# hong-chen/er3t

Measured on AMD Instinct MI355X. Metric: photons/sec, higher is better.
Workload: dtype f32; 1 GPU; les480: 480x480x100-voxel LES cloud domain (Atm_nz=116), nadir radiance, HG g=0.85 + Rayleigh, Lambert 0.03; views=1, target=radiance, local_estimate=column-table (exact for nadir), parallelism=single GPU

## Files before the change

### er3t_amd/csrc/mi3d_api.hip

```cpp
#include <hip/hip_runtime.h>

#include <cmath>
#include <cstdarg>
#include <cstdio>
#include <cstdlib>
#include <cstring>
#include <string>
#include <utility>
#include <vector>

#include "mi3d_kernels.hip"
#include "mi3d_kernel_lean.hip"
#include "mi3d_kernel_rays.hip"
#include "mi3d_kernel_flux.hip"

using namespace mi3d;

#include <algorithm>

static constexpr size_t kTabLdsBudget = 24 * 1024;
constexpr int kEvSlots = 4;

namespace {

// ... 46 lines not shown

}

struct mi3d_solver {
    int device = 0;
    int num_cu = 256;
    hipStream_t stream = nullptr;
    hipStream_t own_stream = nullptr;
    bool use_own_stream = false;

    int nz = 0, np1d = 0;
    std::vector<double> zgrd;
    std::vector<float> ext1d, omg1d, apf1d, abs1d;
    int nx = 1, ny = 1, nz3 = 0, iz3l = 1, np3d = 0;
    double dx = 1.0e4, dy = 1.0e4;
    bool has_abst = false;
    int nang = 0, npf = 0;
    std::vector<float> ang, pha;
    int sfc_mtype = MI3D_SFC_LAMBERT, nxb = 0, nyb = 0;
    bool sfc_lambert_only = true;
    float sfc_param[5] = {0, 0, 0, 0, 0};
    std::vector<float> sfc2d_host;
    double src_flx = 1.0, src_qmax = 0.0, src_the = 180.0, src_phi = 0.0;
    int src_mtype = 1;
    double th_wlen = 0.0, th_ptot = 0.0, th_ms = 0.0;
    double src_fsol = -1.0, th_psol = 0.0;
    bool thermal() const { return src_mtype == 3 || src_mtype == 2; }
    std::vector<float> th_tlev;
    size_t th_ntmpa = 0, th_ntmps = 0;
    size_t th_ncell = 0;
    DevBuf<float> d_th_tlev, d_th_tmpa, d_th_tmps;
    DevBuf<double> d_th_cdf, d_th_bsum;
    DevBuf<DevThermal> d_th;
    bool dirty_thermal = false;
    int nview = 0, nxr = 1, nyr = 1;
    double view_the[MI3D_MAX_VIEW], view_phi[MI3D_MAX_VIEW], view_zloc[MI3D_MAX_VIEW], zref = 0.0;
    int rad_kind = 2;
    double cam_psi[MI3D_MAX_VIEW], cam_xpos[MI3D_MAX_VIEW], cam_ypos[MI3D_MAX_VIEW], cam_qmax[MI3D_MAX_VIEW], cam_umax[MI3D_MAX_VIEW],
           cam_vmax[MI3D_MAX_VIEW], cam_apsize[MI3D_MAX_VIEW];
    DevBuf<CamRec> d_cams;
    int cam_mpmap = 1, cam_mrproj = 0;
    DevBuf<double> d_camdir, d_zgrd;
    bool dirty_camdir = true;
    bool camdir_ok = false;
    int target = MI3D_TARGET_FLUX, solver = MI3D_SOLVER_3D, column_le = 1, counting = 0;
    double wmin = 0.2, wfac = 1.0, le_tau1 = 0.0, le_cmin = 0.0;
    std::vector<LayerRec> lay_host;
    std::vector<double> dir_level;
    int kdir = 0;
    DevBuf<double> d_dir_level;

    DevBuf<float> d_abst, d_extp, d_omgp, d_apfp;
    DevBuf<LayerRec> d_lay;
    DevBuf<ViewRec> d_views;
    DevBuf<DevCold> d_cold;
    DevBuf<float> d_bt1d, d_dz, d_bmin, d_bmax;
    DevBuf<float4> d_vrec;
    DevBuf<float> d_bext3;
    double z_cloud = -1.0;
    int tally_window = 1;
    unsigned vcol_f4 = 0, vrow_f4 = 0;
    int vpad_col = 0, vpad_row = 0;
    DevBuf<float> d_tcol0, d_tmu, d_tp, d_tcdf, d_sfc2d;
    DevBuf<uint16_t> d_tmuidx, d_tcdfidx;
    int nmarch = 0, n_step3d = 0, col0 = 0;
    int tab3d_lo = 1 << 30, tab3d_hi = -1;
    bool hg3d = true;
    int tab_lo = 0, tab_n = 0;
    DevBuf<int> d_tabrange;
    DevBuf<float2> d_csca;
    DevBuf<tally_t> d_rad_own, d_flux_own;
    DevBuf<tally_t> d_rad_acc;
    int rad_row_pad = -1;
    int rad_spread = -1;
    tally_t *rad_ext = nullptr, *flux_ext = nullptr;
    DevBuf<double> d_heat_own;
    double *heat_ext = nullptr;
    int heat_estimator = 0;
    size_t heat_elems() const { return (size_t)nz * nx * ny; }
    double *heat_ptr() { return heat_ext ? heat_ext : d_heat_own.p; }
    DevBuf<unsigned long long> d_counters, d_next;
    DevBuf<uint32_t> d_hist;
    DevBuf<uint16_t> d_tile;
    struct PreSet {
        DevBuf<uint32_t> order, cursor;
        DevBuf<float4> entry;
        hipEvent_t done = nullptr, loop = nullptr; bool used = false;
        void release() { order.release(); entry.release(); }
    };
    PreSet pre[2];
    hipStream_t pre_stream = nullptr;
    hipEvent_t pre_main = nullptr;
    bool pre_main_used = false;
    uint64_t pre_no = 0;
    int pre_last = 0;
    int overlap_pre = 1;
    int cam_images = -1;
    bool cam_warned = false;
    bool general_warned = false;
    int entry_records = 1;
    struct EvSet {
        DevBuf<float4> events;
        DevBuf<unsigned long long> evctr, hvlist;
        hipEvent_t emit = nullptr, rays = nullptr; bool used = false;
        void release() { events.release(); hvlist.release(); }
    };
    EvSet ev[2];
    DevCold cold_host2;
    hipStream_t rays_stream = nullptr;
    int overlap_rays = 0;
    int rays_wg = 0, emit_wg = 0;
    double ev_per_photon = 0.0;
    int n_xcd = 8;
    unsigned long long *h_evctr = nullptr;
    struct EvSlot { hipEvent_t done = nullptr; uint64_t nb = 0, cap = 0; unsigned epoch = 0; bool busy = false, cleared = false; };
    EvSlot ev_slot[kEvSlots];
    unsigned ev_epoch = 0;
    int ev_cap_log2 = 28;
    struct PendingSum { bool on = false; TallyList TL; double *flux = nullptr; unsigned nflux = 0; double *heat = nullptr; unsigned nheat = 0; int split = 1; };
    struct TlSet {
        DevBuf<uint2> rec, binned;
        DevBuf<uint32_t> words;
        DevBuf<unsigned long long> cursor;
        DevBuf<float4> runs;
        hipEvent_t filled = nullptr, sorted = nullptr, scattered = nullptr; bool used = false;
        PendingSum pend;
        void release() { rec.release(); binned.release(); words.release(); runs.release(); }
    };
    TlSet tl[2];
    DevBuf<unsigned long long> d_tl_stats;
    hipStream_t tl_stream = nullptr;
    unsigned runs_unread = 0;
    bool tl_unjoined = false;
    uint64_t tl_launch_no = 0;
    int overlap_sort = 1;
    int tl_split = 4;
    double tl_per_photon = 0.0;
    double tl_total_pp = 0.0, tl_runs_pp = 0.0;
    int tally_runs = 1;
    int tl_cap_log2 = 31;
    int tally_lists = 1;
    int lds_max = 65536;
    unsigned long long *h_tlctr = nullptr;
    DevBuf<char> d_tldesc;
    char *h_tldesc = nullptr;
    hipEvent_t tldesc_ev[64] = {};
    bool tldesc_used[64] = {};
    struct TlSlot { hipEvent_t done = nullptr; uint64_t nb = 0, cap = 0, bcap = 0, rcap = 0; bool busy = false; };
    TlSlot tl_slot[kEvSlots];
    int kernel_choice = 0;
    int tile_cols = -1;
    uint64_t batch = (uint64_t)1 << 30;
    DevCold cold_host;

    bool dirty_grid = true, dirty_phase = true, dirty_sfc = true, dirty_tally = true, dirty_views = true;
    bool have_1d = false;

    DevBuf<float> d_run_own[2], d_stat_out;
    DevBuf<float> d_get_out;
    DevBuf<double> d_get_add;
    float *run_ext[2] = {nullptr, nullptr};
    DevBuf<double> d_sum[2], d_sumsq[2];
    DevBuf<float> d_factor[2];
    bool stats_on = false, stats_joined = false;
    hipEvent_t stats_ev = nullptr;
    int stats_nrun = 0;
    double analytic_share = 1.0;
    float *run_ptr(int w) { return run_ext[w] ? run_ext[w] : d_run_own[w].p; }
    size_t stat_elems(int w) const { return w == 0 ? (size_t)nview * nxr * nyr : flux_elems(); }

    std::vector<std::pair<hipEvent_t, hipEvent_t>> pending;
    double kernel_ms = 0.0;
    uint64_t launches = 0;
    std::string last_kernel;

    size_t rad_elems() const { return (size_t)(nview > 0 ? nview : 1) * nxr * nyr; }
    size_t flux_elems() const { return (size_t)3 * (nz + 1) * nx * ny; }
    tally_t *rad_ptr() { return rad_ext ? rad_ext : d_rad_own.p; }
    tally_t *flux_ptr() { return flux_ext ? flux_ext : d_flux_own.p; }
};

namespace {

// ... 382 lines not shown
    hipLaunchKernelGGL(k_scan_top, dim3(1), dim3(1024), 0, h->stream, h->d_th_bsum.p, (unsigned long)nblk);
    HIPCHK(hipGetLastError());
    hipLaunchKernelGGL(k_scan_add, dim3((unsigned)nblk), dim3(256), 0, h->stream, h->d_th_cdf.p, (unsigned long)ncell, (const double *)h->d_th_bsum.p);
    HIPCHK(hipGetLastError());
    HIPCHK(hipEventRecord(e1, h->stream));
    double ptot = 0.0;
    HIPCHK(hipMemcpyAsync(&ptot, h->d_th_cdf.p + (ncell - 1), sizeof(double), hipMemcpyDeviceToHost, h->stream));
    HIPCHK(hipStreamSynchronize(h->stream));
    float ms = 0.0f;
    HIPCHK(hipEventElapsedTime(&ms, e0, e1));
    (void)hipEventDestroy(e0); (void)hipEventDestroy(e1);
    h->th_ms = ms;
    if (!(ptot >= 0.0) || !std::isfinite(ptot)) return fail(MI3D_EINVAL, "thermal source: total emitted power %g", ptot);
    h->th_ptot = ptot;
    h->th_ncell = ncell;
    h->th_psol = 0.0;
    if (h->src_mtype == 2)
        h->th_psol = h->src_fsol * std::fabs(std::cos(h->src_the * 3.14159265358979323846 / 180.0)) * (h->dx * h->nx) * (h->dy * h->ny);
    DevThermal T;
    T.cdf = h->d_th_cdf.p; T.ptot = ptot; T.psol = h->th_psol; T.ncell = (unsigned)ncell; T.nvox = (unsigned)nvox;
    T.nxb = sfc2d ? h->nxb : 1; T.nyb = sfc2d ? h->nyb : 1;
    if ((rc = h->d_th.upload(&T, 1))) return rc;
    return MI3D_OK;
}

constexpr double kCamDirMaxCells = 1048576.0;
int build_camdir(mi3d_solver *h) {
    const size_t n = (size_t)h->nview * h->nxr * h->nyr;
    HIPCHK(sync_streams(h));
    int rc;
    if ((rc = h->d_camdir.alloc(n)) || (rc = h->d_zgrd.upload(h->zgrd.data(), h->zgrd.size()))) return rc;
    HIPCHK(hipMemsetAsync(h->d_camdir.p, 0, n * sizeof(double), h->stream));
    h->camdir_ok = true;
    if (h->src_mtype == 1) {
        const double pi = 3.14159265358979323846;
        const double th = h->src_the * pi / 180.0, ph = h->src_phi * pi / 180.0;
        const int k3lo = h->nz3 > 0 ? h->iz3l - 1 : 0;
        if (h->nz3 > 0) {
            const double h3 = h->zgrd[k3lo + h->nz3] - h->zgrd[k3lo], sz = -std::cos(th);
            const double cells = h->nz3 + 2.0 + h3 / sz * (std::fabs(std::sin(th) * std::cos(ph)) / h->dx + std::fabs(std::sin(th) * std::sin(ph)) / h->dy);
            if (!(cells <= kCamDirMaxCells)) { h->camdir_ok = false; return MI3D_OK; }
        }
        hipLaunchKernelGGL(k_cam_direct, dim3((unsigned)((h->nview + 63) / 64)), dim3(64), 0, h->stream, h->nview, h->nxr, h->nyr,
                           (const CamRec *)h->d_cams.p, (const ViewRec *)h->d_views.p, (const double *)h->d_zgrd.p, (const LayerRec *)h->d_lay.p,
                           h->nz, h->nx, h->ny, h->nz3, k3lo, h->dx, h->dy, (const float *)(h->nz3 > 0 ? h->d_bext3.p : nullptr),
                           -std::sin(th) * std::cos(ph), -std::sin(th) * std::sin(ph), -std::cos(th), h->d_camdir.p);
        HIPCHK(hipGetLastError());
    }
    return MI3D_OK;
}

}

extern "C" {

int mi3d_version(void) { return MI3D_VERSION; }

const char *mi3d_last_error(void) { return g_err.c_str(); }

int mi3d_device_count(void) {
    int n = 0;
    if (hipGetDeviceCount(&n) != hipSuccess) return 0;
    return n;
}

int mi3d_create(int device, mi3d_solver **out) {
    if (!out) return fail(MI3D_EINVAL, "out is NULL");
    *out = nullptr;
    int n = 0;
    hipError_t e = hipGetDeviceCount(&n);
    if (e != hipSuccess || n <= 0)
        return fail(MI3D_EDEVICE, "no HIP device available (%s); this solver has no CPU fallback",
                    e == hipSuccess ? "device count is 0" : hipGetErrorString(e));
    if (device < 0 || device >= n) return fail(MI3D_EINVAL, "device %d out of range [0,%d)", device, n);
    HIPCHK(hipSetDevice(device));
    mi3d_solver *h = new mi3d_solver();
    h->device = device;
    hipDeviceProp_t prop;
    if (hipGetDeviceProperties(&prop, device) == hipSuccess && prop.multiProcessorCount > 0)
        h->num_cu = prop.multiProcessorCount;
    { int v = 0; if (hipDeviceGetAttribute(&v, hipDeviceAttributeMaxSharedMemoryPerBlock, device) == hipSuccess && v >= 32768) h->lds_max = v; else (void)hipGetLastError(); }
    int rc;
    if ((rc = h->d_counters.alloc(MI3D_NCOUNTER)) || (rc = h->d_next.alloc(8 * kCtrStride)) ||
        (rc = h->d_hist.alloc(kMaxTiles)) || (rc = h->pre[0].cursor.alloc(kMaxTiles))) { delete h; return rc; }
    HIPCHK(hipMemset(h->d_counters.p, 0, MI3D_NCOUNTER * sizeof(unsigned long long)));
    HIPCHK(hipMemset(h->d_next.p, 0, 8 * kCtrStride * sizeof(unsigned long long)));
    {
        DevBuf<unsigned> fl;
        unsigned host[8] = {0, 0, 0, 0, 0, 0, 0, 0};
        if (fl.alloc(8) == MI3D_OK && hipMemset(fl.p, 0, sizeof(host)) == hipSuccess) {
            hipLaunchKernelGGL(k_xcc_census, dim3(4096), dim3(64), 0, nullptr, fl.p);
            if (hipMemcpy(host, fl.p, sizeof(host), hipMemcpyDeviceToHost) == hipSuccess) {
                int n = 0;
                for (unsigned f : host) n += f ? 1 : 0;
                if (n >= 1) h->n_xcd = n;
            }
        }
        (void)hipGetLastError();
        fl.release();
    }
    if (const char *e = getenv("MI3D_TILE_COLS")) h->tile_cols = atoi(e);
    if (const char *e = getenv("MI3D_RAD_SPREAD")) h->rad_spread = atoi(e);
    if (const char *e = getenv("MI3D_RAD_ROW_PAD")) h->rad_row_pad = atoi(e);
    if (const char *e = getenv("MI3D_TALLY_WINDOW")) h->tally_window = atoi(e) ? 1 : 0;
    if (const char *e = getenv("MI3D_TALLY_LISTS")) h->tally_lists = atoi(e) ? 1 : 0;
    if (const char *e = getenv("MI3D_TALLY_RUNS")) h->tally_runs = atoi(e) ? 1 : 0;
    if (const char *e = getenv("MI3D_ENTRY_RECORDS")) h->entry_records = atoi(e) ? 1 : 0;
    if (const char *e = getenv("MI3D_OVERLAP_RAYS")) h->overlap_rays = atoi(e) ? 1 : 0;
    if (const char *e = getenv("MI3D_OVERLAP_SORT")) h->overlap_sort = std::max(0, std::min(2, atoi(e)));
    if (const char *e = getenv("MI3D_OVERLAP_PRE")) h->overlap_pre = std::max(0, std::min(2, atoi(e)));
    if (const char *e = getenv("MI3D_TL_SPLIT")) h->tl_split = std::max(1, std::min(64, atoi(e)));
    if (const char *e = getenv("MI3D_RAYS_WG")) h->rays_wg = std::max(0, std::min(8, atoi(e)));
    if (const char *e = getenv("MI3D_EMIT_WG")) h->emit_wg = std::max(0, std::min(8, atoi(e)));
    if (const char *e = getenv("MI3D_VPAD_COL")) h->vpad_col = std::max(0, atoi(e));
    if (const char *e = getenv("MI3D_VPAD_ROW")) h->vpad_row = std::max(0, atoi(e));
    if (const char *e = getenv("MI3D_KERNEL")) h->kernel_choice = std::strcmp(e, "generic") == 0 ? 1 : 0;
    if (const char *e = getenv("MI3D_EVCAP_LOG2")) { const int b = atoi(e); if (b >= 12 && b <= 28) h->ev_cap_log2 = b; }
    if (const char *e = getenv("MI3D_BATCH_LOG2")) { const int b = atoi(e); if (b >= 8 && b <= 30) h->batch = (uint64_t)1 << b; }
    *out = h;
    return MI3D_OK;
}

int mi3d_destroy(mi3d_solver *h) {
    if (!h) return MI3D_OK;
    (void)hipSetDevice(h->device);
    (void)hipDeviceSynchronize();
    auto destroy_event = [](hipEvent_t e) { if (e) (void)hipEventDestroy(e); };
    for (auto &pr : h->pending) { (void)hipEventDestroy(pr.first); (void)hipEventDestroy(pr.second); }
    destroy_event(h->stats_ev);
    for (auto &S : h->ev_slot) destroy_event(S.done);
    for (auto &S : h->tl_slot) destroy_event(S.done);
    for (hipEvent_t e : h->tldesc_ev) destroy_event(e);
    destroy_event(h->pre_main);
    for (auto &P : h->pre) { destroy_event(P.done); destroy_event(P.loop); P.release(); P.cursor.release(); }
    for (auto &E : h->ev) { destroy_event(E.emit); destroy_event(E.rays); E.release(); E.evctr.release(); }
    for (auto &T : h->tl) { destroy_event(T.filled); destroy_event(T.sorted); destroy_event(T.scattered); T.release(); T.cursor.release(); }
    for (hipStream_t st : {h->own_stream, h->rays_stream, h->tl_stream, h->pre_stream}) if (st) (void)hipStreamDestroy(st);
    for (void *p : {(void *)h->h_evctr, (void *)h->h_tlctr, (void *)h->h_tldesc}) if (p) (void)hipHostFree(p);
    h->d_abst.release(); h->d_extp.release(); h->d_omgp.release(); h->d_apfp.release();
    h->d_lay.release(); h->d_vrec.release(); h->d_bext3.release(); h->d_tcol0.release(); h->d_tmu.release(); h->d_tp.release();
    h->d_tcdf.release(); h->d_tmuidx.release(); h->d_tcdfidx.release(); h->d_sfc2d.release(); h->d_csca.release(); h->d_rad_own.release();
    h->d_flux_own.release(); h->d_heat_own.release(); h->d_counters.release(); h->d_next.release();
    h->d_rad_acc.release(); h->d_cams.release(); h->d_camdir.release(); h->d_zgrd.release();
    h->d_hist.release(); h->d_tile.release(); h->d_tldesc.release(); h->d_tl_stats.release();
    for (int w = 0; w < 2; ++w) { h->d_run_own[w].release(); h->d_sum[w].release(); h->d_sumsq[w].release(); h->d_factor[w].release(); }
    h->d_stat_out.release(); h->d_dir_level.release(); h->d_get_out.release(); h->d_get_add.release();
    h->d_th_tlev.release(); h->d_th_tmpa.release(); h->d_th_tmps.release(); h->d_th_cdf.release(); h->d_th_bsum.release(); h->d_th.release();
    h->d_views.release(); h->d_cold.release(); h->d_tabrange.release(); h->d_bt1d.release(); h->d_dz.release(); h->d_bmin.release(); h->d_bmax.release();
    delete h;
    return MI3D_OK;
}

int mi3d_set_atm1d(mi3d_solver *h, int nz, const double *zgrd, int np1d, const float *ext, const float *omg,
                   const float *apf, const float *abs) {
    int rc = check_handle(h);
    if (rc) return rc;
    if (nz < 1 || nz > kMaxLayers) return fail(MI3D_EINVAL, "Atm_nz=%d outside [1,%d]", nz, kMaxLayers);
    if (np1d < 1 || np1d > MI3D_MAX_NP1D) return fail(MI3D_EINVAL, "Atm_np1d=%d outside [1,%d]", np1d, MI3D_MAX_NP1D);
    if (!zgrd || !ext || !omg || !apf) return fail(MI3D_EINVAL, "NULL 1-D profile");
    for (int k = 0; k < nz; ++k)
        if (!(zgrd[k + 1] > zgrd[k])) return fail(MI3D_EINVAL, "Atm_zgrd0 must ascend strictly (level %d)", k + 1);
    const size_t n = (size_t)nz * np1d;
    for (size_t i = 0; i < n; ++i)
        if (!(ext[i] >= 0.0f) || !(omg[i] >= 0.0f)) return fail(MI3D_EINVAL, "negative or NaN 1-D extinction / albedo");
    if (h->nz != nz) h->dirty_tally = true;
    h->nz = nz; h->np1d = np1d;
    h->zgrd.assign(zgrd, zgrd + nz + 1);
    h->ext1d.assign(ext, ext + n); h->omg1d.assign(omg, omg + n); h->apf1d.assign(apf, apf + n);
    if (abs) h->abs1d.assign(abs, abs + nz); else h->abs1d.assign(nz, 0.0f);
    h->have_1d = true;
    h->dirty_grid = true;
    return MI3D_OK;
}

int mi3d_set_atm3d(mi3d_solver *h, int nx, int ny, int nz3, int iz3l, int np3d, double dx, double dy,
                   const float *abst, const float *extp, const float *omgp, const float *apfp) {
    int rc = check_handle(h);
    if (rc) return rc;
    if (nx < 1 || ny < 1 || nz3 < 0) return fail(MI3D_EINVAL, "bad grid %d x %d x %d", nx, ny, nz3);
    if (!(dx > 0.0) || !(dy > 0.0)) return fail(MI3D_EINVAL, "Atm_dx / Atm_dy must be positive");
    if (nz3 > 0) {
        if (np3d < 1 || np3d > MI3D_MAX_NP3D) return fail(MI3D_EINVAL, "Atm_np3d=%d outside [1,%d]", np3d, MI3D_MAX_NP3D);
        if (!extp || !omgp || !apfp) return fail(MI3D_EINVAL, "NULL 3-D array");
        if (iz3l < 1) return fail(MI3D_EINVAL, "Atm_iz3l=%d must be >= 1", iz3l);
    }
    if (h->nx != nx || h->ny != ny) h->dirty_tally = true;
    h->nx = nx; h->ny = ny; h->nz3 = nz3; h->iz3l = nz3 > 0 ? iz3l : 1; h->np3d = nz3 > 0 ? np3d : 0;
    h->dx = dx; h->dy = dy;
    h->has_abst = false;
    if (nz3 > 0) {
// ... 310 lines not shown
            h->tab3d_lo = init[0]; h->tab3d_hi = init[1]; h->hg3d = (init[2] == 0) && (init[1] < 0);
            HIPCHK(hipMemcpy(bmin.data(), h->d_bmin.p, h->nz3 * sizeof(float), hipMemcpyDeviceToHost));
            HIPCHK(hipMemcpy(bmax.data(), h->d_bmax.p, h->nz3 * sizeof(float), hipMemcpyDeviceToHost));
            double wsum = 0.0, wz = 0.0;
            for (int k3 = 0; k3 < h->nz3; ++k3) {
                uniform3d[k3] = (bmin[k3] == bmax[k3]) ? 1 : 0;
                bt3d[k3] = bmin[k3];
                const double wgt = (double)bmax[k3] - (double)bmin[k3];
                wsum += wgt; wz += wgt * 0.5 * (h->zgrd[k3lo + k3] + h->zgrd[k3lo + k3 + 1]);
            }
            h->z_cloud = wsum > 0.0 ? wz / wsum : -1.0;
        }
        std::vector<LayerRec> lay;
        if ((rc = build_layers(h, uniform3d, bt3d, lay))) return rc;
        if ((rc = h->d_lay.upload(lay.data(), lay.size()))) return rc;
        h->lay_host = lay;
        h->dirty_grid = false;
        h->dirty_thermal = true;
        h->dirty_views = true;
        ev_forget(h);
        for (auto &S : h->tl_slot) S.busy = false;
    }
    if (h->dirty_views) {
        if ((rc = build_views(h))) return rc;
        h->dirty_views = false;
        h->dirty_camdir = true;
    }
    if (h->dirty_phase) {
        if ((rc = build_tables(h))) return rc;
        h->dirty_phase = false;
    }
    if (h->npf <= 0 && needs_tables(h))
        return fail(MI3D_ESTATE, "a 1-D component selects a tabulated phase function (apf >= 1) but no table is loaded");
    if (h->dirty_sfc) {
        if (!h->sfc2d_host.empty())
            if ((rc = h->d_sfc2d.upload(h->sfc2d_host.data(), h->sfc2d_host.size()))) return rc;
        h->dirty_sfc = false;
    }
    if (h->dirty_tally) {
        if (!h->rad_ext) {
            if ((rc = h->d_rad_own.alloc(h->rad_elems()))) return rc;
            HIPCHK(hipMemsetAsync(h->d_rad_own.p, 0, h->rad_elems() * sizeof(tally_t), h->stream));
        }
        if (!h->flux_ext) {
            if ((rc = h->d_flux_own.alloc(h->flux_elems()))) return rc;
            HIPCHK(hipMemsetAsync(h->d_flux_own.p, 0, h->flux_elems() * sizeof(tally_t), h->stream));
        }
        if ((h->target & MI3D_TARGET_HEAT) && !h->heat_ext) {
            if ((rc = h->d_heat_own.alloc(h->heat_elems()))) return rc;
            HIPCHK(hipMemsetAsync(h->d_heat_own.p, 0, h->heat_elems() * sizeof(double), h->stream));
        }
        h->dirty_tally = false;
    }
    if (h->thermal() && h->dirty_thermal) {
        if ((rc = build_thermal(h))) return rc;
        h->dirty_thermal = false;
    }
    if (h->rad_kind == 1 && h->nview > 0 && h->dirty_camdir) {
        if ((rc = build_camdir(h))) return rc;
        h->dirty_camdir = false;
    }
    return MI3D_OK;
}

int mi3d_reset(mi3d_solver *h) {
    int rc = check_handle(h);
    if (rc) return rc;
    if ((rc = mi3d_prepare(h))) return rc;
    for (const auto &E : h->ev) if (E.used && E.rays) HIPCHK(hipStreamWaitEvent(h->stream, E.rays, 0));
    HIPCHK(tl_join(h));
    HIPCHK(hipMemsetAsync(h->rad_ptr(), 0, h->rad_elems() * sizeof(tally_t), h->stream));
    HIPCHK(hipMemsetAsync(h->flux_ptr(), 0, h->flux_elems() * sizeof(tally_t), h->stream));
    if ((h->target & MI3D_TARGET_HEAT) && h->heat_ptr()) HIPCHK(hipMemsetAsync(h->heat_ptr(), 0, h->heat_elems() * sizeof(double), h->stream));
    HIPCHK(hipMemsetAsync(h->d_counters.p, 0, MI3D_NCOUNTER * sizeof(unsigned long long), h->stream));
    if (h->d_rad_acc.p) HIPCHK(hipMemsetAsync(h->d_rad_acc.p, 0, h->d_rad_acc.cap * sizeof(tally_t), h->stream));
    if ((rc = drain_events(h))) return rc;
    for (auto &S : h->ev_slot) if (S.busy) S.cleared = true;
    h->kernel_ms = 0.0;
    h->launches = 0;
    return MI3D_OK;
}

static hipError_t launch_bins(mi3d_solver *h, hipStream_t st, const BinGeom &G, int ntile, uint64_t seed, uint64_t off, uint64_t nb, uint32_t *order, uint32_t *cursor) {
    hipError_t err = hipMemsetAsync(h->d_hist.p, 0, kMaxTiles * sizeof(uint32_t), st);
    if (err != hipSuccess) return err;
    const unsigned nblk = (unsigned)std::min<uint64_t>((nb + 4095) / 4096, 4096);
    hipLaunchKernelGGL(k_bin_count, dim3(nblk), dim3(256), 0, st, G, seed, off, (uint32_t)nb, h->d_tile.p, h->d_hist.p);
    hipLaunchKernelGGL(k_bin_scan, dim3(1), dim3(256), 0, st, ntile, h->d_hist.p, cursor);
    const uint32_t slab = (uint32_t)((nb + nblk - 1) / nblk);
    hipLaunchKernelGGL(k_bin_scatter, dim3(nblk), dim3(256), 0, st, ntile, (uint32_t)nb, slab, h->d_tile.p, cursor, order);
    return hipGetLastError();
}

static hipError_t launch_entry(mi3d_solver *h, hipStream_t st, const DevScene &S, uint64_t nb, uint64_t seed, uint64_t off, const uint32_t *order, float4 *entry) {
    const DevCold &C = h->cold_host;
    EntryArgs A;
    A.lay = C.lay;
    A.Lx = C.Lx; A.Ly = C.Ly; A.dx = S.dx; A.dy = S.dy; A.inv_dx = C.inv_dx; A.inv_dy = C.inv_dy; A.inv_nx = C.inv_nx; A.inv_ny = C.inv_ny;
    A.sdx = C.sdx; A.sdy = C.sdy; A.sdz = C.sdz; A.cos_cone = C.cos_cone;
    A.nx = S.nx; A.ny = S.ny; A.nz = S.nz; A.solver = S.solver; A.target = S.target; A.kdir = S.kdir;
    hipLaunchKernelGGL(k_entry, dim3((unsigned)((nb + 255) / 256)), dim3(256), 0, st, A, nb, seed, off, order, entry);
    return hipGetLastError();
}

static hipError_t launch_lean(mi3d_solver *h, hipStream_t st, const DevScene &S, bool emit, int mix, int nt, unsigned grid, size_t lds, uint64_t nb, uint64_t seed, uint64_t off) {
    const int v = (h->counting ? 4 : 0) + (h->solver == MI3D_SOLVER_P3D ? 2 : 0) + (emit ? 1 : 0);
#define MI3D_LEAN_LAUNCH(C, P, M)                                                                                                        \
    do {                                                                                                                                 \
        if (mix == 3 && nt == 512) {                                                                                                     \
            if (lds > 65536) (void)hipFuncSetAttribute(reinterpret_cast<const void *>(k_transport_lean<C, P, 0, 3, 512>), hipFuncAttributeMaxDynamicSharedMemorySize, (int)lds); \
            hipLaunchKernelGGL((k_transport_lean<C, P, 0, 3, 512>), dim3(grid), dim3(512), lds, st, S, nb, seed, off);                    \
        } else if (mix == 3) {                                                                                                           \
            if (lds > 65536) (void)hipFuncSetAttribute(reinterpret_cast<const void *>(k_transport_lean<C, P, 0, 3>), hipFuncAttributeMaxDynamicSharedMemorySize, (int)lds); \
            hipLaunchKernelGGL((k_transport_lean<C, P, 0, 3>), dim3(grid), dim3(256), lds, st, S, nb, seed, off);                         \
        } else if (mix == 2 && nt == 512 && (M) == 0) {                                                                                  \
            if (lds > 65536) (void)hipFuncSetAttribute(reinterpret_cast<const void *>(k_transport_lean<C, P, 0, 2, 512>), hipFuncAttributeMaxDynamicSharedMemorySize, (int)lds); \
            hipLaunchKernelGGL((k_transport_lean<C, P, 0, 2, 512>), dim3(grid), dim3(512), lds, st, S, nb, seed, off);                    \
        } else if (mix == 2) {                                                                                                           \
            if (lds > 65536) (void)hipFuncSetAttribute(reinterpret_cast<const void *>(k_transport_lean<C, P, M, 2>), hipFuncAttributeMaxDynamicSharedMemorySize, (int)lds); \
            hipLaunchKernelGGL((k_transport_lean<C, P, M, 2>), dim3(grid), dim3(256), lds, st, S, nb, seed, off);                         \
        } else if (mix == 1) hipLaunchKernelGGL((k_transport_lean<C, P, M, 1>), dim3(grid), dim3(256), lds, st, S, nb, seed, off);        \
        else hipLaunchKernelGGL((k_transport_lean<C, P, M, 0>), dim3(grid), dim3(256), lds, st, S, nb, seed, off);                        \
    } while (0)
    switch (v) {
        case 0: MI3D_LEAN_LAUNCH(false, false, 0); break;
        case 1: MI3D_LEAN_LAUNCH(false, false, 2); break;
        case 2: MI3D_LEAN_LAUNCH(false, true, 0); break;
        case 3: MI3D_LEAN_LAUNCH(false, true, 2); break;
        case 4: MI3D_LEAN_LAUNCH(true, false, 0); break;
        case 5: MI3D_LEAN_LAUNCH(true, false, 2); break;
        case 6: MI3D_LEAN_LAUNCH(true, true, 0); break;
        default: MI3D_LEAN_LAUNCH(true, true, 2); break;
    }
#undef MI3D_LEAN_LAUNCH
    return hipGetLastError();
}

static hipError_t launch_rays(mi3d_solver *h, hipStream_t st, const DevScene &S, bool heavy, size_t lds, uint64_t seed) {
    if (h->rad_kind == 1) {
        const unsigned gridc = (unsigned)h->num_cu * 4u;
        if (h->src_mtype == 3) {
            if (lds > 65536) {
                (void)hipFuncSetAttribute(reinterpret_cast<const void *>(k_rays<true, false, false, true, false, true>), hipFuncAttributeMaxDynamicSharedMemorySize, (int)lds);
                (void)hipFuncSetAttribute(reinterpret_cast<const void *>(k_rays<false, false, false, true, false, true>), hipFuncAttributeMaxDynamicSharedMemorySize, (int)lds);
            }
            if (h->counting) hipLaunchKernelGGL((k_rays<true, false, false, true, false, true>), dim3(gridc), dim3(256), lds, st, S, seed);
            else hipLaunchKernelGGL((k_rays<false, false, false, true, false, true>), dim3(gridc), dim3(256), lds, st, S, seed);
            return hipGetLastError();
        }
        if (lds > 65536) {
            (void)hipFuncSetAttribute(reinterpret_cast<const void *>(k_rays<true, false, false, true>), hipFuncAttributeMaxDynamicSharedMemorySize, (int)lds);
            (void)hipFuncSetAttribute(reinterpret_cast<const void *>(k_rays<false, false, false, true>), hipFuncAttributeMaxDynamicSharedMemorySize, (int)lds);
        }
        if (h->counting) hipLaunchKernelGGL((k_rays<true, false, false, true>), dim3(gridc), dim3(256), lds, st, S, seed);
        else hipLaunchKernelGGL((k_rays<false, false, false, true>), dim3(gridc), dim3(256), lds, st, S, seed);
        return hipGetLastError();
    }
    const unsigned grid = (unsigned)h->num_cu * (unsigned)((h->rays_wg > 0 && !heavy) ? std::min(h->rays_wg, MI3D_RAYS_WAVES(h->counting != 0, heavy)) : MI3D_RAYS_WAVES(h->counting != 0, heavy));
    const bool p3d = h->solver == MI3D_SOLVER_P3D;
    const bool plain = (S.target & kTargetPlainPhase) != 0 && !heavy;
#define MI3D_LAUNCH_RAYS(C, P, X)                                                                                                    \
    do {                                                                                                                             \
        if (plain) {                                                                                                                 \
            if (lds > 65536) (void)hipFuncSetAttribute(reinterpret_cast<const void *>(k_rays<C, P, false, false, true>), hipFuncAttributeMaxDynamicSharedMemorySize, (int)lds); \
            hipLaunchKernelGGL((k_rays<C, P, false, false, true>), dim3(grid), dim3(256), lds, st, S, seed);                          \
        } else {                                                                                                                     \
            if (lds > 65536) (void)hipFuncSetAttribute(reinterpret_cast<const void *>(k_rays<C, P, X, false, false>), hipFuncAttributeMaxDynamicSharedMemorySize, (int)lds); \
            hipLaunchKernelGGL((k_rays<C, P, X, false, false>), dim3(grid), dim3(256), lds, st, S, seed);                             \
        }                                                                                                                            \
    } while (0)
    switch ((h->counting ? 4 : 0) | (p3d ? 2 : 0) | (heavy ? 1 : 0)) {
        case 0: MI3D_LAUNCH_RAYS(false, false, false); break;
        case 1: MI3D_LAUNCH_RAYS(false, false, true); break;
        case 2: MI3D_LAUNCH_RAYS(false, true, false); break;
        case 3: MI3D_LAUNCH_RAYS(false, true, true); break;
        case 4: MI3D_LAUNCH_RAYS(true, false, false); break;
        case 5: MI3D_LAUNCH_RAYS(true, false, true); break;
        case 6: MI3D_LAUNCH_RAYS(true, true, false); break;
        default: MI3D_LAUNCH_RAYS(true, true, true); break;
    }
#undef MI3D_LAUNCH_RAYS
    return hipGetLastError();
}

#ifndef MI3D_BLOCKS_PER_CU
#define MI3D_BLOCKS_PER_CU(MARCH, COUNT) MI3D_WAVES(MARCH, COUNT)
#endif

static hipError_t launch_general(mi3d_solver *h, const DevScene &S, bool march, bool flux, unsigned grid, uint64_t nb, uint64_t seed, uint64_t off, bool emit = false) {
    const int tb = 256;
    const size_t lds = (size_t)h->nz * sizeof(LayerRec) + MI3D_MAX_VIEW * sizeof(ViewRec) + sizeof(DevCold) + (size_t)9 * tb * sizeof(float) +
                       (size_t)(h->tab_n > 0 ? (1 + 2 * h->tab_n) * h->nang * sizeof(float) : 0);
    const int src = h->src_mtype == 3 ? 1 : h->src_mtype == 2 ? 2 : 0;
    const DevThermal *th = src ? h->d_th.p : nullptr;
    if (emit) {
        if (h->counting) hipLaunchKernelGGL((k_transport<true, 2, false, false, 1>), dim3(grid), dim3(tb), lds, h->stream, S, nb, seed, off, th);
        else hipLaunchKernelGGL((k_transport<false, 2, false, false, 1>), dim3(grid), dim3(tb), lds, h->stream, S, nb, seed, off, th);
        return hipGetLastError();
    }
#define MI3D_LAUNCH_T(C, M, F, T)                                                                                                      \
    do { if (h->solver == MI3D_SOLVER_P3D) hipLaunchKernelGGL((k_transport<C, M, F, true, T>), dim3(grid), dim3(tb), lds, h->stream, S, nb, seed, off, th); \
         else hipLaunchKernelGGL((k_transport<C, M, F, false, T>), dim3(grid), dim3(tb), lds, h->stream, S, nb, seed, off, th); } while (0)
#define MI3D_LAUNCH(C, M, F) do { if (src == 2) MI3D_LAUNCH_T(C, M, F, 2); else if (src == 1) MI3D_LAUNCH_T(C, M, F, 1); else MI3D_LAUNCH_T(C, M, F, 0); } while (0)
    switch ((h->counting ? 4 : 0) | (march ? 2 : 0) | (flux ? 1 : 0)) {
// ... 347 lines not shown
        if (have > 0 && (double)have >= (double)c) c = have;
        else if (have > 0 && (double)have >= 0.7 * (double)c && (double)have * item_bytes >= 1.6e10) c = have;
        else if (c > have && have > 0) c = std::max<uint64_t>(c, have + have / 4);
        c = std::min<uint64_t>(c, lim);
        c = std::max<uint64_t>(c, std::min<uint64_t>(have, lim));
        return c / chunk * chunk;
    };
    const mi3d_solver::TlSet &S0 = h->tl[0];
    const uint64_t want_cap = cap_of(r.dpp, kTlChunk, S0.rec.cap, 8.0 * nset);
    const uint64_t want_bcap = cap_of(r.tpp, kTlChunk, S0.binned.cap, 8.0 * nset);
    const uint64_t want_rcap = runs ? std::max<uint64_t>(cap_of(r.rpp, kRunChunk, S0.runs.cap / 2, 32.0 * nset), 64 * kRunChunk) : 0;
    if (want_cap < 64 * kTlChunk) return 0;
    T.cap = (unsigned)want_cap; T.bcap = (unsigned)want_bcap; T.run_cap = (unsigned)want_rcap;
    T.nwave = (int)waves;
    T.wcap = (int)std::max<size_t>(64, 4 * (size_t)(want_cap / kTlChunk) / waves);
    T.run_wcap = runs ? (int)std::max<size_t>(64, 4 * (size_t)(want_rcap / kRunChunk) / waves) : 0;
    const size_t nrow = (size_t)tl_nrow(T);
    const size_t nwords = (size_t)(want_cap / kTlChunk) + waves * T.wcap + waves + 2 * nrow * T.nbins + 2 * (size_t)T.nbins + 1 +
                          (runs ? (size_t)(want_rcap / kRunChunk) + waves * T.run_wcap + waves : 0);
    bool moves = false;
    for (int q = 0; q < nset; ++q) moves = moves || want_cap > h->tl[q].rec.cap || want_bcap > h->tl[q].binned.cap || nwords > h->tl[q].words.cap || 2 * want_rcap > h->tl[q].runs.cap;
    if (moves && sync_streams(h) != hipSuccess) { (void)hipGetLastError(); return 0; }
    int rc = MI3D_OK;
    for (int q = 0; q < nset && !rc; ++q) {
        mi3d_solver::TlSet &S = h->tl[q];
        rc = S.rec.alloc(want_cap);
        if (!rc) rc = S.binned.alloc(want_bcap);
        if (!rc) rc = S.words.alloc(nwords);
        if (!rc) rc = S.cursor.alloc(kCtrStride);
        if (!rc && q == 0) rc = h->d_tl_stats.alloc(64 * 4);
        if (!rc && runs) rc = S.runs.alloc(2 * want_rcap);
    }
    if (!rc && !h->h_tlctr && hipHostMalloc((void **)&h->h_tlctr, (size_t)4 * kEvSlots * sizeof(unsigned long long)) != hipSuccess) rc = MI3D_EDEVICE;
    if (rc) {
        (void)hipGetLastError();
        for (auto &S : h->tl) S.release();
        fprintf(stderr, "Warning [mi3d_run]: no device memory for the tally-record lists of this flux job (%.1f GB free); an atomic per level crossing instead (same results, slower).\n", (double)free_b / 1.0e9);
        return 0;
    }
    tl_compact_hist(h, T);
    for (int q = 0; q < 2; ++q) { TL[q] = T; tl_lay_out(TL[q], h->tl[q < nset ? q : 0]); }
    return want_cap;
}

static uint64_t size_ev_lists(mi3d_solver *h, uint64_t nphoton, bool two_sets) {
    const double per_rec = (double)kEvBlockF4 * 16.0 / 64.0 + (h->sfc_lambert_only ? 0.0 : 8.0);
    size_t free_b = free_bytes((size_t)8 << 30);
    for (const auto &E : h->ev) free_b += E.events.cap * sizeof(float4) + E.hvlist.cap * sizeof(unsigned long long);
    const int nset = two_sets ? 2 : 1;
    const uint64_t cap_mem = (uint64_t)(0.25 * (double)free_b / (8.0 * per_rec * nset));
    const uint64_t cap_max = (uint64_t)1 << h->ev_cap_log2;
    uint64_t want_cap = std::min<uint64_t>(cap_max, 64 * nphoton + 65536);
    if (h->ev_per_photon > 0.0)
        want_cap = std::min<uint64_t>(want_cap, std::max<uint64_t>((uint64_t)(4.0 * h->ev_per_photon * (double)nphoton / h->n_xcd), 65536));
    else want_cap = std::min<uint64_t>(want_cap, (uint64_t)1 << 22);
    want_cap = std::max<uint64_t>(want_cap, std::min<uint64_t>(h->ev[0].events.cap / ((size_t)8 * kEvBlockF4) * 64, cap_max));
    want_cap = std::min<uint64_t>(want_cap, cap_mem);
    want_cap &= ~(uint64_t)63;
    int r = MI3D_OK;
    for (;;) {
        r = want_cap < 65536 ? fail(MI3D_EDEVICE, "no memory for event lists") : MI3D_OK;
        for (int q = 0; q < nset && !r; ++q) {
            mi3d_solver::EvSet &E = h->ev[q];
            r = E.events.alloc((size_t)8 * ev_list_f4(want_cap));
            if (!r) r = E.evctr.alloc(kCtrWords * kCtrStride);
            if (!r && !h->sfc_lambert_only) r = E.hvlist.alloc((size_t)8 * want_cap);
        }
        if (!r && !h->h_evctr && hipHostMalloc((void **)&h->h_evctr, (size_t)kEvSlots * 9 * kCtrStride * sizeof(unsigned long long)) != hipSuccess) r = MI3D_EDEVICE;
        if (!r || want_cap < 65536) break;
        (void)hipGetLastError();
        for (auto &E : h->ev) E.release();
        want_cap = (want_cap / 2) & ~(uint64_t)63;
    }
    if (r) {
        (void)hipGetLastError();
        fprintf(stderr, "Warning [mi3d_run]: no device memory for the event lists of the marched views (%.1f GB free); the general kernel marches them inside its photon loop (same results, slower).\n", (double)free_b / 1.0e9);
        return 0;
    }
    h->cold_host.ev_list = h->ev[0].events.p; h->cold_host.ev_ctr = h->ev[0].evctr.p; h->cold_host.ev_cap = (int)want_cap;
    h->cold_host.hv_list = h->sfc_lambert_only ? nullptr : h->ev[0].hvlist.p;
    return want_cap;
}

static bool use_entry_records(mi3d_solver *h, const RunPlan &plan, uint64_t nphoton) {
#if MI3D_LEAN_FAST
    if ((h->target & MI3D_TARGET_HEAT) && h->heat_estimator == 1) return false;
    if (plan.loop == Loop::General || plan.thermal || !h->entry_records || h->nx >= 65536 || h->ny >= 65536 || h->nz >= 32768) return false;
    DevBuf<float4> &E = h->pre[0].entry;
    const size_t need = entry_f4((size_t)std::min<uint64_t>(nphoton, h->batch));
    size_t free_b = free_bytes((size_t)8 << 30);
    free_b += E.cap * sizeof(float4);
    if (need > E.cap && need * sizeof(float4) > free_b / 2) return false;
    if (E.alloc(need) == MI3D_OK) { h->cold_host.entry = E.p; return true; }
    (void)hipGetLastError();
#endif
    return false;
}

static bool pre_second_set(mi3d_solver *h, const RunPlan &plan, bool use_entry, bool two_sets, uint64_t nphoton) {
    mi3d_solver::PreSet &P0 = h->pre[0], &P1 = h->pre[1];
    bool two = h->overlap_pre && !two_sets && (plan.sorted || use_entry) && (plan.loop == Loop::Flux || plan.loop == Loop::ColumnRays) &&
               (h->overlap_pre > 1 || nphoton >= ((uint64_t)1 << 22) || h->runs_unread > 0);
    if (two && !h->pre_stream && hipStreamCreateWithFlags(&h->pre_stream, hipStreamNonBlocking) != hipSuccess) { (void)hipGetLastError(); two = false; }
    for (auto &S : h->pre) two = two && new_event(S.done) && new_event(S.loop);
    if (two && plan.sorted && (P1.order.alloc(P0.order.cap) != MI3D_OK || P1.cursor.alloc(kMaxTiles) != MI3D_OK)) { (void)hipGetLastError(); two = false; }
    if (two && use_entry && P1.entry.cap < P0.entry.cap) {
        const size_t free_b = free_bytes(0) + P1.entry.cap * sizeof(float4);
        if (P0.entry.cap * sizeof(float4) > free_b / 2 || P1.entry.alloc(P0.entry.cap) != MI3D_OK) { (void)hipGetLastError(); two = false; }
    }
    if (!two && (P1.entry.cap * sizeof(float4) + P1.order.cap * sizeof(uint32_t)) > ((size_t)256 << 20)) P1.release();
    return two;
}

static void set_tally_window(mi3d_solver *h, const RunPlan &plan) {
    DevCold &C = h->cold_host;
    C.tile_end = nullptr; C.win_tc = 0; C.win_ntx = 0; C.win_ntile = 0; C.win_off = 0u;
    if (!(plan.loop == Loop::Column || plan.loop == Loop::ColumnRays) || !window_wanted(h) || !plan.sorted || h->nx >= 32768 || h->ny >= 32768 ||
        h->nx < kWin || h->ny < kWin || !(h->z_cloud >= 0.0) || !(C.sdz < 0.0f))
        return;
    const double ztoa = h->zgrd[h->nz];
    const double way = h->solver == MI3D_SOLVER_IPA ? 0.0 : (ztoa - h->z_cloud) / std::fabs((double)C.sdz);
    const int tcols = plan.G.tcols;
    const int margin = (kWin - std::min(tcols, kWin)) / 2 - std::max(0, tcols - kWin) / 2;
    auto wrap = [](long v, int n) { v %= n; if (v < 0) v += n; return (unsigned)v; };
    const unsigned ox = wrap(std::lround(C.sdx * way / h->dx) - margin, h->nx);
    const unsigned oy = wrap(std::lround(C.sdy * way / h->dy) - margin, h->ny);
    C.tile_end = h->pre[0].cursor.p;
    C.win_tc = tcols; C.win_ntx = plan.G.ntx; C.win_ntile = plan.ntile;
    C.win_off = ox | (oy << 16);
}

static int rad_acc_image(mi3d_solver *h, const RunPlan &plan, DevScene &S, int &rad_row) {
    rad_row = 0;
    const int row = h->rad_row_pad >= 0 ? h->nxr + h->rad_row_pad : 32 * (((h->nxr + 31) / 32) | 1);
    const size_t acc_elems = (size_t)h->nview * h->nyr * row;
    const bool few_pixels = plan.thermal && h->rad_kind == 1 && (size_t)h->nview * h->nyr * h->nxr <= 1024;
    const bool spread = (h->target & MI3D_TARGET_RADIANCE) && h->nview > 0 && h->rad_spread != 0 && !(h->rad_spread < 0 && plan.loop == Loop::ColumnRays && !few_pixels) &&
                        (double)acc_elems * kRadLine * sizeof(tally_t) <= 1.0e9 && (double)acc_elems * kRadLine < 2147483647.0;
    if (!spread) return MI3D_OK;
    const size_t need = acc_elems * kRadLine;
    if (h->d_rad_acc.cap < need || !h->d_rad_acc.p) {
        int rc = h->d_rad_acc.alloc(need);
        if (rc) return rc;
        HIPCHK(hipMemsetAsync(h->d_rad_acc.p, 0, need * sizeof(tally_t), h->stream));
    }
    S.rad = h->d_rad_acc.p; S.rad_stride = kRadLine; S.rad_row = row;
    rad_row = row;
    return MI3D_OK;
}

static int launch_photons(mi3d_solver *h, const RunPlan &plan, uint64_t ev_cap, const TallyList &TL, bool tl_two, uint64_t nphoton, uint64_t done, uint64_t &per) {
    const uint64_t left = nphoton - done;
    int rc;
    if (plan.loop == Loop::ColumnRays) {
        if ((rc = ev_collect(h, false))) return rc;
        const uint64_t room = photons_that_fit(ev_cap, h->ev_per_photon, h->n_xcd);
        const uint64_t want_n = std::max<uint64_t>(std::min<uint64_t>(room, h->batch), 64);
        const uint64_t nl = (left + want_n - 1) / want_n;
        per = (left + nl - 1) / nl;
    }
    if (TL.cap) {
        if ((rc = tl_collect(h, false))) return rc;
        const uint64_t waves = (uint64_t)h->num_cu * MI3D_FLUX_WAVES(h->counting != 0) * 4;
        auto room_of = [waves](uint64_t cap_, uint64_t chunk, double pp_) -> uint64_t {
            return (uint64_t)((double)(cap_ > 2 * waves * chunk ? cap_ - waves * chunk : cap_ / 2) / pp_);
        };
        const TlRates r = tl_rates(h, TL.run_cap != 0);
        uint64_t room = std::min(room_of(TL.cap, kTlChunk, r.dpp), room_of(TL.bcap, kTlChunk, r.tpp));
        if (TL.run_cap) room = std::min(room, room_of(TL.run_cap, kRunChunk, r.rpp));
        const uint64_t want_n = std::max<uint64_t>(std::min<uint64_t>(room, h->batch), 4096);
        uint64_t nl = (left + want_n - 1) / want_n;
        if (tl_two && done == 0) nl = std::max<uint64_t>(nl, std::min<uint64_t>((uint64_t)h->tl_split, nphoton >> 23));
        else if (tl_two) nl = std::max<uint64_t>(nl, std::min<uint64_t>((left + per - 1) / std::max<uint64_t>(per, 1), (uint64_t)h->tl_split));
        nl = std::max<uint64_t>(nl, 1);
        per = (left + nl - 1) / nl;
    }
    return MI3D_OK;
}

static hipError_t launch_column(mi3d_solver *h, const RunPlan &plan, const DevScene &Sl, int set, bool two_sets, hipStream_t rs, unsigned grid, uint64_t nb, uint64_t seed, uint64_t off) {
    const bool split = plan.loop == Loop::ColumnRays;
    mi3d_solver::EvSet &E = h->ev[set];
    const size_t lds_col = (size_t)(h->nz + 2) * sizeof(LayerRec) + MI3D_MAX_VIEW * sizeof(ViewRec) + sizeof(DevCold);
    const int emit_wg = h->counting ? 4 : (h->emit_wg > 0 ? std::min(h->emit_wg, MI3D_LEAN_EMIT_GRID) : MI3D_LEAN_EMIT_GRID);
    const unsigned gridp = split ? (unsigned)std::min<uint64_t>((nb + 255) / 256, (uint64_t)h->num_cu * emit_wg) : grid;
    DevScene Sx = Sl;
    if (set) Sx.cold = h->d_cold.p + 1;
    hipError_t err = hipSuccess;
    if (two_sets && E.used) err = hipStreamWaitEvent(h->stream, E.rays, 0);
    if (err == hipSuccess && split) err = hipMemsetAsync(E.evctr.p, 0, kCtrWords * kCtrStride * sizeof(unsigned long long), h->stream);
    if (err == hipSuccess && plan.thermal) err = launch_general(h, Sx, false, false, gridp, nb, seed, off, true);
    else if (err == hipSuccess) {
        const size_t lds_lean = lds_col + (h->cold_host.tile_end ? kWinLds : 0) + plan.lds_tab;
        const bool wide = plan.mix >= 2 && !split && !h->counting && lds_lean * 3 <= (size_t)160 * 1024 && lds_lean * 6 > (size_t)160 * 1024;
        unsigned gridw = wide ? (unsigned)std::min<uint64_t>((nb + 511) / 512, (uint64_t)h->num_cu * 3) : gridp;
        if (plan.mix >= 2 && !wide && !split && !h->counting) gridw = std::min<unsigned>(gridw, (unsigned)h->num_cu * (unsigned)std::max<size_t>(1, std::min<size_t>(MI3D_GEN_NARROW_WAVES, ((size_t)160 * 1024) / lds_lean)));
        err = launch_lean(h, h->stream, Sx, split, plan.mix_lean, wide ? 512 : 256, gridw, lds_lean, nb, seed, off);
    }
    if (err != hipSuccess || !split) return err;
    if (two_sets) {
        err = hipEventRecord(E.emit, h->stream);
        if (err == hipSuccess) err = hipStreamWaitEvent(rs, E.emit, 0);
    }
    const bool plain_scene = (Sl.target & kTargetPlainPhase) != 0 && h->rad_kind != 1;
    if (err == hipSuccess) err = launch_rays(h, rs, Sx, false, lds_col + rays_lds_extra(h->nz, h->rad_kind == 1) + (plain_scene ? 0 : plan.lds_tab), seed);
    if (err == hipSuccess && !h->sfc_lambert_only && h->rad_kind != 1)
        err = launch_rays(h, rs, Sx, true, lds_col + rays_lds_extra(h->nz) + plan.lds_tab, seed);
    return err;
}

static int flux_lists(mi3d_solver *h, const RunPlan &plan, uint64_t nphoton, TallyList TL[2], bool &tl_two, size_t &lds_fl) {
    int rc;
    if ((rc = h->d_tldesc.alloc((size_t)64 * sizeof(TallyList)))) return rc;
    if (!h->h_tldesc && hipHostMalloc((void **)&h->h_tldesc, (size_t)64 * sizeof(TallyList)) != hipSuccess) return fail(MI3D_EDEVICE, "no pinned memory for the tally-list descriptions");
    tl_two = h->overlap_sort != 0 && (h->overlap_sort == 2 || nphoton >= ((uint64_t)1 << 25) || h->runs_unread > 0);
    if (tl_two && !h->tl_stream && hipStreamCreateWithFlags(&h->tl_stream, hipStreamNonBlocking) != hipSuccess) { (void)hipGetLastError(); tl_two = false; }
    for (auto &T : h->tl) tl_two = tl_two && new_event(T.filled) && new_event(T.sorted) && new_event(T.scattered);
    const bool tl_pilot = !(h->tl_total_pp > 0.0) && nphoton > ((uint64_t)1 << 21);
    lds_fl = (size_t)(h->nz + 2) * sizeof(LayerRec) + sizeof(DevCold);
    if (h->tally_lists && nphoton >= 4096 && size_tally_lists(h, tl_pilot ? (uint64_t)1 << 21 : std::min<uint64_t>(nphoton, h->batch), tl_two ? 2 : 1, TL))
        lds_fl += TL[0].hist_wg ? ((size_t)TL[0].ncb + 3) / 4 * 16 : (size_t)TL[0].nbins * 16;
    lds_fl += (size_t)4 * 128 * sizeof(float4) + (size_t)4 * kTlStage * sizeof(uint2);
    lds_fl += plan.lds_tab;
    if (!TL[0].cap) tl_two = false;
    if (!tl_two && TL[0].cap) HIPCHK(tl_join(h));
    return MI3D_OK;
}

static int event_lists(mi3d_solver *h, RunPlan &plan, uint64_t nphoton, uint64_t &ev_cap, bool &two_sets) {
    if (plan.loop == Loop::ColumnRays) {
        two_sets = h->overlap_rays != 0;
        if (two_sets && !h->rays_stream && hipStreamCreateWithFlags(&h->rays_stream, hipStreamNonBlocking) != hipSuccess) { (void)hipGetLastError(); two_sets = false; }
        for (auto &E : h->ev) two_sets = two_sets && new_event(E.emit) && new_event(E.rays);
        if (!(ev_cap = size_ev_lists(h, nphoton, two_sets))) {
            for (auto &E : h->ev) E.release();
            plan.loop = Loop::General; plan.why = "no device memory for its event lists"; two_sets = false;
            if (h->rad_kind == 1) {
                if (h->cam_images > 0) return fail(MI3D_EDEVICE, "no device memory for the event lists of a camera job with cam_images=%d (the general kernel serves the nearest image only)", h->cam_images);
                return cam_fallback(h, plan.why);
            }
        }
    } else if (h->ev[0].events.p) {
        HIPCHK(sync_streams(h));
        for (auto &E : h->ev) E.release();
    }
    return MI3D_OK;
}

static hipError_t launch_pre(mi3d_solver *h, const RunPlan &plan, int pset, bool pre_two, bool pre_track, bool use_entry, const DevScene &S, uint64_t nb, uint64_t seed, uint64_t off) {
    mi3d_solver::PreSet &PS = h->pre[pset];
    hipStream_t const ps = pre_two ? h->pre_stream : h->stream;
    hipError_t eb = hipSuccess;
    if (pre_two && PS.used) eb = hipStreamWaitEvent(ps, PS.loop, 0);
    if (eb == hipSuccess && pre_two && h->pre_main_used) { eb = hipStreamWaitEvent(ps, h->pre_main, 0); h->pre_main_used = false; }
    if (eb == hipSuccess && plan.sorted) eb = launch_bins(h, ps, plan.G, plan.ntile, seed, off, nb, PS.order.p, PS.cursor.p);
    if (eb == hipSuccess && use_entry)
        eb = launch_entry(h, ps, S, nb, seed, off, plan.sorted ? (const uint32_t *)PS.order.p : (const uint32_t *)nullptr, PS.entry.p);
    if (eb == hipSuccess && pre_two) eb = hipEventRecord(PS.done, ps);
    if (eb == hipSuccess && pre_track && !pre_two) {
        if (!h->pre_main) eb = hipEventCreateWithFlags(&h->pre_main, hipEventDisableTiming);
        if (eb == hipSuccess) { eb = hipEventRecord(h->pre_main, h->stream); h->pre_main_used = true; }
    }
    if (eb == hipSuccess && pre_two) eb = hipStreamWaitEvent(h->stream, PS.done, 0);
    return eb;
}

int mi3d_run(mi3d_solver *h, uint64_t nphoton, uint64_t seed, uint64_t photon_offset) {
    int rc = check_handle(h);
    if (rc) return rc;
    if ((rc = mi3d_prepare(h))) return rc;
    if ((h->target & MI3D_TARGET_RADIANCE) && h->nview == 0)
        return fail(MI3D_ESTATE, "radiance requested but no view is set (mi3d_set_views)");
    if ((h->target & MI3D_TARGET_RADIANCE) && h->rad_kind == 1 && h->solver != MI3D_SOLVER_3D)
        return fail(MI3D_EUNSUP, "cameras (Rad_mrkind=1) need the 3-D solver");
    const bool thermal = h->thermal();
    if (h->src_mtype == 2 && (h->target & MI3D_TARGET_RADIANCE) && h->rad_kind == 1)
        return fail(MI3D_EUNSUP, "solar+thermal source (Src_mtype=2): all-sky cameras (Rad_mrkind=1) are not supported");
    if (nphoton == 0) return MI3D_OK;
    if (thermal && !(h->th_ptot + h->th_psol > 0.0)) {
        h->last_kernel = h->src_mtype == 2 ? "k_transport [solar+thermal: nothing emits, no sunlight]" : "k_transport [thermal: nothing emits]";
        return MI3D_OK;
    }
    {
        const double lim = 2147483647.0;
        const double nvox = (double)h->nx * h->ny * (h->nz3 + 1) * (h->np3d > 0 ? h->np3d : 1);
        if (nvox > lim || (double)h->flux_elems() > lim || (double)h->rad_elems() > lim || (double)h->heat_elems() > lim)
            return fail(MI3D_EUNSUP, "grid too large for the 32-bit table indices of the transport kernel");
    }
    DevScene S;
    if ((rc = fill_scene(h, S))) return rc;
    RunPlan plan = plan_run(h, nphoton);
    if (plan.sorted) {
        const size_t cap = (size_t)std::min<uint64_t>(nphoton, h->batch);
        if ((rc = h->pre[0].order.alloc(cap)) || (rc = h->d_tile.alloc(cap))) return rc;
    }
    h->cold_host.order = plan.sorted ? h->pre[0].order.p : nullptr;

    TallyList TL[2] = {};
    bool tl_two = false, two_sets = false;
    size_t lds_fl = 0;
    uint64_t ev_cap = 0;
    if (plan.loop == Loop::Flux && (rc = flux_lists(h, plan, nphoton, TL, tl_two, lds_fl))) return rc;
    if (h->rad_kind == 1 && plan.loop != Loop::ColumnRays && (rc = cam_fallback(h, plan.why))) return rc;
    if ((rc = event_lists(h, plan, nphoton, ev_cap, two_sets))) return rc;
    name_route(h, plan, TL[0].cap != 0, nphoton);
    const uint64_t cap = (uint64_t)h->num_cu * (plan.loop == Loop::Flux ? MI3D_FLUX_WAVES(h->counting != 0)
                                                : plan.loop == Loop::General ? MI3D_BLOCKS_PER_CU(plan.march, h->counting != 0)
                                                                             : MI3D_LEAN_WAVES(h->counting != 0, plan.march));
    const bool use_entry = use_entry_records(h, plan, nphoton);
    const bool pre_two = pre_second_set(h, plan, use_entry, two_sets, nphoton);
    const bool pre_track = h->overlap_pre && (plan.sorted || use_entry);
    h->runs_unread++;
    set_tally_window(h, plan);
    int rad_row = 0;
    if ((rc = rad_acc_image(h, plan, S, rad_row))) return rc;
    h->cold_host.cam_images = (unsigned)(plan.loop == Loop::ColumnRays ? (h->cam_images < 0 ? 2 : h->cam_images) : 0);
    HIPCHK(upload_cold(h, two_sets, pre_two));

    hipEvent_t run_e0 = nullptr;
    struct RunGuard { hipEvent_t &e; mi3d_solver *h; ~RunGuard() { if (e) { (void)hipEventDestroy(e); e = nullptr; (void)sync_streams(h); } } } run_guard{run_e0, h};
    const bool run_timed = two_sets || tl_two;
    if (run_timed) { HIPCHK(hipEventCreate(&run_e0)); HIPCHK(hipEventRecord(run_e0, h->stream)); }
    uint64_t ilaunch = 0;
    const uint64_t nlaunch = (nphoton + h->batch - 1) / h->batch;
    uint64_t per = (nphoton + nlaunch - 1) / nlaunch;
    for (uint64_t done = 0; done < nphoton; done += per) {
        if ((rc = launch_photons(h, plan, ev_cap, TL[0], tl_two, nphoton, done, per))) return rc;
        const uint64_t nb = std::min<uint64_t>(per, nphoton - done), off = photon_offset + done;
        if (h->pending.size() >= 64 && (rc = drain_events(h))) return rc;
        HIPCHK(hipMemsetAsync(h->d_next.p, 0, 8 * kCtrStride * sizeof(unsigned long long), h->stream));
        const int pset = pre_two ? (int)(h->pre_no & 1) : 0;
        mi3d_solver::PreSet &PS = h->pre[pset];
        const hipError_t eb = launch_pre(h, plan, pset, pre_two, pre_track, use_entry, S, nb, seed, off);
        if (eb != hipSuccess) { (void)sync_streams(h); return fail(MI3D_EDEVICE, "photon order / entry records: %s", hipGetErrorString(eb)); }
        DevScene Sl = S;
        if (pset) Sl.cold = h->d_cold.p + 1;
        const uint64_t want = (nb + 255) / 256;
        const unsigned grid = (unsigned)(want < cap ? want : cap);
        hipEvent_t e0 = nullptr, e1 = nullptr;
        hipError_t err = run_timed ? hipSuccess : hipEventCreate(&e0);
        if (err == hipSuccess && !run_timed && (err = hipEventCreate(&e1)) == hipSuccess) err = hipEventRecord(e0, h->stream);
        const int set = two_sets ? (int)(ilaunch & 1) : 0;
        const int tset = tl_two ? (int)(h->tl_launch_no & 1) : 0;
        hipStream_t const rs = two_sets ? h->rays_stream : h->stream;
        if (err == hipSuccess && plan.loop == Loop::Flux) {
            err = launch_flux(h, tset, tl_two, Sl, TL[tset], plan.mix, grid, lds_fl, nb, seed, off);
            if (err == hipSuccess && tl_two) { err = hipEventRecord(h->tl[tset].sorted, h->tl_stream); h->tl[tset].used = true; h->tl_unjoined = true; }
        } else if (err == hipSuccess && plan.loop == Loop::General) err = launch_general(h, Sl, plan.march, plan.flux, grid, nb, seed, off);
        else if (err == hipSuccess) err = launch_column(h, plan, Sl, set, two_sets, rs, grid, nb, seed, off);
        if (err == hipSuccess && !run_timed) err = hipEventRecord(e1, h->stream);
        h->pre_last = pset;
        if (err == hipSuccess && (pre_two || pre_track)) {
            if (!PS.loop) err = hipEventCreateWithFlags(&PS.loop, hipEventDisableTiming);
            if (err == hipSuccess) err = hipEventRecord(PS.loop, h->stream);
            PS.used = true;
            if (pre_two) h->pre_no++;
        }
        if (err != hipSuccess) {
            if (e0) (void)hipEventDestroy(e0);
            if (e1) (void)hipEventDestroy(e1);
            (void)sync_streams(h);
            return fail(MI3D_EDEVICE, "transport launch failed: %s", hipGetErrorString(err));
        }
        if (!run_timed) h->pending.emplace_back(e0, e1);
        h->launches++; ilaunch++;
        if (TL[0].cap) {
            const bool first = !(h->tl_total_pp > 0.0);
            if ((rc = tl_note(h, TL[0].cap, TL[0].bcap, TL[0].run_cap, nb, h->d_tl_stats.p + 4 * ((h->launches - 1) % 64), tl_two ? h->tl_stream : h->stream))) return rc;
            h->tl_launch_no++;
            if (first && done + nb < nphoton) {
                if ((rc = tl_collect(h, true))) return rc;
                HIPCHK(sync_streams(h));
                if (!size_tally_lists(h, std::min<uint64_t>(nphoton - done - nb, h->batch), tl_two ? 2 : 1, TL)) return fail(MI3D_EDEVICE, "no device memory to grow the tally-record lists after the pilot launch");
            }
        }
        if (plan.loop == Loop::ColumnRays) {
            mi3d_solver::EvSet &E = h->ev[set];
            rc = ev_note(h, ev_cap, nb, rs, E.evctr.p);
            if (!rc && two_sets) {
                if (hipEventRecord(E.rays, rs) != hipSuccess) rc = fail(MI3D_EDEVICE, "event record failed");
                E.used = true;
            }
            if (rc) { (void)sync_streams(h); return rc; }
            if (!(h->ev_per_photon > 0.0)) {
                if ((rc = ev_collect(h, true))) return rc;
                if (done + nb < nphoton) {
                    HIPCHK(sync_streams(h));
                    if (!(ev_cap = size_ev_lists(h, nphoton, two_sets))) return fail(MI3D_EDEVICE, "no device memory to grow the event lists of the marched views after the pilot launch");
                    HIPCHK(upload_cold(h, two_sets, pre_two));
                }
            }
        }
    }
    const bool tl_lazy = h->overlap_sort == 2 && tl_two && !two_sets && !h->flux_ext && !h->heat_ext && !h->rad_ext && (h->stream == nullptr || h->stream == h->own_stream);
    if (run_timed) {
        if (tl_two && !tl_lazy) HIPCHK(tl_join(h));
        for (const auto &E : h->ev) if (two_sets && E.used) HIPCHK(hipStreamWaitEvent(h->stream, E.rays, 0));
        hipEvent_t run_e1 = nullptr;
        HIPCHK(hipEventCreate(&run_e1)); HIPCHK(hipEventRecord(run_e1, tl_two && tl_lazy ? h->tl_stream : h->stream));
        h->pending.emplace_back(run_e0, run_e1);
        run_e0 = nullptr;
    }
    if (plan.loop == Loop::ColumnRays && (rc = ev_collect(h, false))) { (void)sync_streams(h); return rc; }
    if (TL[0].cap && (rc = tl_collect(h, false))) return rc;
    if (rad_row) {
        const int n = (int)h->rad_elems();
        hipLaunchKernelGGL(k_fold_rad, dim3((unsigned)((n + 255) / 256)), dim3(256), 0, h->stream, h->d_rad_acc.p, h->rad_ptr(), kRadLine, n, h->nxr, rad_row);
        HIPCHK(hipGetLastError());
    }
    return MI3D_OK;
}

int mi3d_sync(mi3d_solver *h) {
    int rc = check_handle(h);
    if (rc) return rc;
    HIPCHK(sync_main(h));
    return ev_settle(h);
}

int mi3d_set_kernel(mi3d_solver *h, int choice) {
    int rc = check_handle(h);
    if (rc) return rc;
    if (choice < 0 || choice > 1) return fail(MI3D_EINVAL, "kernel choice %d (0: the lean kernels where they apply, 1: always the general one; choice 2, the lean loop with the rays of marched views inside it, was retired in round 5)", choice);
    HIPCHK(tl_join(h));
    h->kernel_choice = choice;
    return MI3D_OK;
}

int mi3d_set_tuning(mi3d_solver *h, const char *key, int value) {
    int rc = check_handle(h);
    if (rc) return rc;
    if (!key) return fail(MI3D_EINVAL, "NULL key");
    const std::string k(key);
    if (k == "tile_cols") { if (value < -1 || value > 4096) return fail(MI3D_EINVAL, "tile_cols=%d", value); h->tile_cols = value; }
    else if (k == "batch_log2") { if (value < 8 || value > 30) return fail(MI3D_EINVAL, "batch_log2=%d outside [8,30]", value); h->batch = (uint64_t)1 << value; }
    else if (k == "evcap_log2") {
        if (value < 10 || value > 28) return fail(MI3D_EINVAL, "evcap_log2=%d outside [10,28]", value);
        HIPCHK(sync_streams(h));
        h->ev_cap_log2 = value; ev_forget(h);
        for (auto &E : h->ev) E.release();
    }
    else if (k == "rad_spread") h->rad_spread = value < 0 ? -1 : (value ? 1 : 0);
    else if (k == "tally_window") h->tally_window = value ? 1 : 0;
    else if (k == "rad_row_pad") { if (value < -1 || value > 4096) return fail(MI3D_EINVAL, "rad_row_pad=%d outside [-1,4096]", value); h->rad_row_pad = value; }
    else if (k == "tlcap_log2") {
        if (value < 16 || value > 31) return fail(MI3D_EINVAL, "tlcap_log2=%d outside [16,31]", value);
        HIPCHK(sync_main(h));
        h->tl_cap_log2 = value; h->tl_per_photon = 0.0; h->tl_total_pp = 0.0; h->tl_runs_pp = 0.0;
        for (auto &S : h->tl_slot) S.busy = false;
        for (auto &T : h->tl) T.release();
    }
    else if (k == "vpad_col" || k == "vpad_row") {
        if (value < 0 || value > 4096) return fail(MI3D_EINVAL, "%s=%d outside [0,4096]", key, value);
        (k == "vpad_col" ? h->vpad_col : h->vpad_row) = value;
        h->dirty_grid = true;
    }
    else if (k == "overlap_rays") { HIPCHK(sync_streams(h)); h->overlap_rays = value ? 1 : 0; }
    else if (k == "overlap_pre") { if (value < 0 || value > 2) return fail(MI3D_EINVAL, "overlap_pre=%d outside [0,2]", value); HIPCHK(sync_streams(h)); h->overlap_pre = value; if (!value) { h->pre[1].release(); h->pre_last = 0; } }
    else if (k == "overlap_sort") { if (value < 0 || value > 2) return fail(MI3D_EINVAL, "overlap_sort=%d outside [0,2]", value); HIPCHK(sync_streams(h)); h->overlap_sort = value; if (!value) h->tl[1].release(); }
    else if (k == "tl_split") { if (value < 1 || value > 64) return fail(MI3D_EINVAL, "tl_split=%d outside [1,64]", value); h->tl_split = value; }
    else if (k == "rays_wg" || k == "emit_wg") { if (value < 0 || value > 8) return fail(MI3D_EINVAL, "%s=%d outside [0,8]", key, value); (k == "rays_wg" ? h->rays_wg : h->emit_wg) = value; }
    else if (k == "cam_images") { if (value < -1 || value > 8) return fail(MI3D_EINVAL, "cam_images=%d outside [-1,8]", value); h->cam_images = value; }
    else if (k == "entry_records") { HIPCHK(sync_main(h)); h->entry_records = value ? 1 : 0; if (!value) h->pre[0].entry.release(); }
    else if (k == "tally_runs") { HIPCHK(sync_main(h)); h->tally_runs = value ? 1 : 0; h->tl_per_photon = 0.0; h->tl_total_pp = 0.0; h->tl_runs_pp = 0.0; if (!value) for (auto &T : h->tl) T.runs.release(); }
    else if (k == "tally_lists") { HIPCHK(sync_main(h)); h->tally_lists = value ? 1 : 0; if (!value) for (auto &T : h->tl) T.release(); }
    else if (k == "own_stream") {
        HIPCHK(sync_main(h));
        const bool was_default = (h->stream == nullptr) || (h->stream == h->own_stream);
        if (value && !h->own_stream && hipStreamCreateWithFlags(&h->own_stream, hipStreamNonBlocking) != hipSuccess)
            return fail(MI3D_EDEVICE, "cannot create a stream");
        h->use_own_stream = value != 0;
        if (was_default) h->stream = h->use_own_stream ? h->own_stream : nullptr;
    }
    else return fail(MI3D_EINVAL, "unknown tuning key '%s'", key);
    return MI3D_OK;
}

const char *mi3d_last_kernel(mi3d_solver *h) { return h ? h->last_kernel.c_str() : ""; }

int mi3d_get_timing(mi3d_solver *h, double *kernel_ms, uint64_t *launches) {
    int rc = check_handle(h);
    if (rc) return rc;
    if ((rc = drain_events(h))) return rc;
    if (kernel_ms) *kernel_ms = h->kernel_ms;
    if (launches) *launches = h->launches;
    return MI3D_OK;
}

int mi3d_get_radiance(mi3d_solver *h, uint64_t nphoton_total, float *out) {
    int rc = check_handle(h);
    if (rc) return rc;
    if (!out || nphoton_total == 0) return fail(MI3D_EINVAL, "bad arguments to mi3d_get_radiance");
    if (!h->rad_ptr()) return fail(MI3D_ESTATE, "no radiance tally (nothing has run)");
    HIPCHK(sync_main(h));
    if ((rc = ev_settle(h))) return rc;
    const size_t n = (size_t)h->nview * h->nxr * h->nyr;
    const double amp = src_amp(h);
    const double fac = h->rad_kind == 1 ? amp * (h->dx * h->nx) * (h->dy * h->ny) / (double)nphoton_total
                                        : amp * (double)h->nxr * (double)h->nyr / (double)nphoton_total;
    if (n == 0) return MI3D_OK;
    if ((rc = h->d_get_out.alloc(n))) return rc;
    hipLaunchKernelGGL(k_get_field, dim3((unsigned)((n + 255) / 256)), dim3(256), 0, h->stream, (const tally_t *)h->rad_ptr(), h->d_get_out.p, fac,
                       1u, 1u, -1L, (const double *)nullptr, n);
    HIPCHK(hipGetLastError());
    HIPCHK(hipMemcpyAsync(out, h->d_get_out.p, n * sizeof(float), hipMemcpyDeviceToHost, h->stream));
    HIPCHK(hipStreamSynchronize(h->stream));
    return MI3D_OK;
}

int mi3d_get_flux(mi3d_solver *h, uint64_t nphoton_total, float *out) {
    int rc = check_handle(h);
    if (rc) return rc;
    if (!out || nphoton_total == 0) return fail(MI3D_EINVAL, "bad arguments to mi3d_get_flux");
    if (!h->flux_ptr()) return fail(MI3D_ESTATE, "no flux tally (nothing has run)");
    HIPCHK(sync_main(h));
    const size_t n = h->flux_elems();
    const double amp = src_amp(h);
    const double fac = amp * (double)h->nx * (double)h->ny / (double)nphoton_total;
    const double *add = nullptr;
    if (!h->dir_level.empty()) {
        std::vector<double> a(h->dir_level);
        for (double &x : a) x = amp * x;
        if ((rc = h->d_get_add.upload(a.data(), a.size()))) return rc;
        add = h->d_get_add.p;
    }
    if (n == 0) return MI3D_OK;
    if ((rc = h->d_get_out.alloc(n))) return rc;
    hipLaunchKernelGGL(k_get_field, dim3((unsigned)((n + 255) / 256)), dim3(256), 0, h->stream, h->flux_ptr(), h->d_get_out.p, fac,
                       (unsigned)((size_t)h->nx * h->ny), (unsigned)(h->nz + 1), (long)(n / 3), add, n);
    HIPCHK(hipGetLastError());
    HIPCHK(hipMemcpyAsync(out, h->d_get_out.p, n * sizeof(float), hipMemcpyDeviceToHost, h->stream));
    HIPCHK(hipStreamSynchronize(h->stream));
    return MI3D_OK;
}

int mi3d_get_direct_levels(mi3d_solver *h, double *out) {
    int rc = check_handle(h);
    if (rc) return rc;
    if (!out) return fail(MI3D_EINVAL, "out is NULL");
    if ((int)h->dir_level.size() != h->nz + 1) return fail(MI3D_ESTATE, "no job has run on this handle since its grid was set");
    const double amp = src_amp(h);
    for (int L = 0; L <= h->nz; ++L) out[L] = amp * h->dir_level[L];
    return MI3D_OK;
}

int mi3d_get_camera_direct(mi3d_solver *h, double *out) {
// ... 171 lines not shown
                           h->d_sum[w].p, h->d_sumsq[w].p, (int)n);
        HIPCHK(hipGetLastError());
    }
    h->stats_nrun++;
    return stats_mark(h);
}

int mi3d_stats_join(mi3d_solver *h, mi3d_solver *owner) {
    int rc = check_handle(h);
    if (rc) return rc;
    if (!owner || owner == h || !owner->stats_on || owner->stats_joined) return fail(MI3D_ESTATE, "mi3d_stats_join: the owner has not begun statistics of its own");
    if (owner->device != h->device) return fail(MI3D_EINVAL, "mi3d_stats_join: the two handles are on different devices");
    if ((rc = mi3d_prepare(h))) return rc;
    if (h->target != owner->target) return fail(MI3D_EINVAL, "mi3d_stats_join: the two handles have different targets");
    for (int w = 0; w < 2; ++w) {
        h->run_ext[w] = nullptr;
        if (!(h->target & (w == 0 ? MI3D_TARGET_RADIANCE : MI3D_TARGET_FLUX))) continue;
        if (h->stat_elems(w) != owner->stat_elems(w)) return fail(MI3D_EINVAL, "mi3d_stats_join: the two scenes have different result shapes");
        h->run_ext[w] = owner->run_ptr(w);
    }
    h->stats_on = true;
    h->stats_joined = true;
    h->stats_nrun = 0;
    return MI3D_OK;
}

int mi3d_stats_chain(mi3d_solver *h, mi3d_solver *after) {
    int rc = check_handle(h);
    if (rc) return rc;
    if (!after || after == h) return MI3D_OK;
    if (after->device != h->device) return fail(MI3D_EINVAL, "mi3d_stats_chain: the two handles are on different devices");
    if (after->stats_ev) HIPCHK(hipStreamWaitEvent(h->stream, after->stats_ev, 0));
    return MI3D_OK;
}

int mi3d_stats_get(mi3d_solver *h, int which, float *mean, float *sdev, int *nrun) {
    int rc = check_handle(h);
    if (rc) return rc;
    if (!h->stats_on) return fail(MI3D_ESTATE, "mi3d_stats_begin has not been called");
    if (which != MI3D_TARGET_RADIANCE && which != MI3D_TARGET_FLUX) return fail(MI3D_EINVAL, "which=%d", which);
    if (nrun) *nrun = h->stats_nrun;
    if (!mean && !sdev) return MI3D_OK;
    if (!(h->target & which)) return fail(MI3D_ESTATE, "no statistics of that kind were gathered");
    if (h->stats_nrun == 0) return fail(MI3D_ESTATE, "no run has been closed (mi3d_stats_end_run)");
    const int w = which == MI3D_TARGET_RADIANCE ? 0 : 1;
    const size_t n = h->stat_elems(w);
    if ((rc = h->d_stat_out.alloc(2 * n))) return rc;
    hipLaunchKernelGGL(k_stats_final, dim3((unsigned)((n + 255) / 256)), dim3(256), 0, h->stream, h->d_sum[w].p,
                       h->d_sumsq[w].p, h->d_stat_out.p, h->d_stat_out.p + n, 1.0 / (double)h->stats_nrun, (int)n);
    HIPCHK(hipGetLastError());
    HIPCHK(sync_main(h));
    if ((rc = ev_settle(h))) return rc;
    if (mean) HIPCHK(hipMemcpy(mean, h->d_stat_out.p, n * sizeof(float), hipMemcpyDeviceToHost));
    if (sdev) HIPCHK(hipMemcpy(sdev, h->d_stat_out.p + n, n * sizeof(float), hipMemcpyDeviceToHost));
    return MI3D_OK;
}

int mi3d_debug_philox(mi3d_solver *h, uint64_t seed, uint64_t id0, uint32_t draw, int n, uint32_t *out) {
    int rc = check_handle(h);
    if (rc) return rc;
    if (n <= 0 || !out) return fail(MI3D_EINVAL, "bad arguments to mi3d_debug_philox");
    DevBuf<uint32_t> d;
    if ((rc = d.alloc((size_t)4 * n))) return rc;
    hipLaunchKernelGGL(k_philox, dim3((n + 255) / 256), dim3(256), 0, h->stream, seed, id0, draw, n, d.p);
    HIPCHK(hipGetLastError());
    HIPCHK(sync_main(h));
    HIPCHK(hipMemcpy(out, d.p, (size_t)4 * n * sizeof(uint32_t), hipMemcpyDeviceToHost));
    d.release();
    return MI3D_OK;
}

int mi3d_debug_order(mi3d_solver *h, uint64_t n, uint32_t *order_out, uint32_t *tile_end_out, int ntile_max) {
    int rc = check_handle(h);
    if (rc) return rc;
    if (n == 0 || !order_out) return fail(MI3D_EINVAL, "bad arguments to mi3d_debug_order");
    if (!h->pre[0].order.p || h->pre[0].order.cap < n) return fail(MI3D_ESTATE, "no photon order of that length (the last launch ran in id order, or was shorter)");
    HIPCHK(sync_main(h));
    HIPCHK(hipMemcpy(order_out, h->pre[h->pre_last].order.p, (size_t)n * sizeof(uint32_t), hipMemcpyDeviceToHost));
    if (tile_end_out && ntile_max > 0)
        HIPCHK(hipMemcpy(tile_end_out, h->pre[h->pre_last].cursor.p, (size_t)std::min(ntile_max, kMaxTiles) * sizeof(uint32_t), hipMemcpyDeviceToHost));
    return MI3D_OK;
}

int mi3d_debug_thermal(mi3d_solver *h, double *ptot, double *cdf_out, uint64_t n) {
    int rc = check_handle(h);
    if (rc) return rc;
    if (!h->thermal()) return fail(MI3D_ESTATE, "mi3d_debug_thermal: the job is not thermal (Src_mtype=%d)", h->src_mtype);
    if (h->dirty_thermal || !h->d_th_cdf.p) return fail(MI3D_ESTATE, "mi3d_debug_thermal: the thermal source is not built (call mi3d_prepare)");
    if (cdf_out && n != h->th_ncell)
        return fail(MI3D_EINVAL, "mi3d_debug_thermal: the CDF has %zu cells, not %llu", h->th_ncell, (unsigned long long)n);
    HIPCHK(sync_main(h));
    if (ptot) *ptot = h->th_ptot;
    if (cdf_out) HIPCHK(hipMemcpy(cdf_out, h->d_th_cdf.p, (size_t)n * sizeof(double), hipMemcpyDeviceToHost));
    return MI3D_OK;
}

static_assert(MI3D_TAB_IDX_N == kTabIdxN, "include/mi3d.h states the length of a bucket index");

int mi3d_debug_phase_tables(mi3d_solver *h, int nang, int npf, float *mu, float *p, float *cdf, uint16_t *mu_idx, uint16_t *cdf_idx) {
    int rc = check_handle(h);
    if (rc) return rc;
    if (h->npf <= 0 || h->dirty_phase || !h->d_tmu.p) return fail(MI3D_ESTATE, "mi3d_debug_phase_tables: no phase table is built (mi3d_set_phase, mi3d_prepare)");
    if (nang != h->nang || npf != h->npf) return fail(MI3D_EINVAL, "mi3d_debug_phase_tables: the tables are %d x %d, not %d x %d", h->npf, h->nang, npf, nang);
    HIPCHK(sync_main(h));
    const size_t n = (size_t)nang, nt = n * (size_t)npf;
    if (mu) HIPCHK(hipMemcpy(mu, h->d_tmu.p, n * sizeof(float), hipMemcpyDeviceToHost));
    if (p) HIPCHK(hipMemcpy(p, h->d_tp.p, nt * sizeof(float), hipMemcpyDeviceToHost));
    if (cdf) HIPCHK(hipMemcpy(cdf, h->d_tcdf.p, nt * sizeof(float), hipMemcpyDeviceToHost));
    if (mu_idx) HIPCHK(hipMemcpy(mu_idx, h->d_tmuidx.p, (size_t)kTabIdxN * sizeof(uint16_t), hipMemcpyDeviceToHost));
    if (cdf_idx) HIPCHK(hipMemcpy(cdf_idx, h->d_tcdfidx.p, (size_t)npf * kTabIdxN * sizeof(uint16_t), hipMemcpyDeviceToHost));
    return MI3D_OK;
}

int mi3d_debug_phase(mi3d_solver *h, int path, int tab_lo, int tab_n, int n, const float *apf, const float *x, const float *usel,
                     float *p_out, float *mu_out) {
    int rc = check_handle(h);
    if (rc) return rc;
    if (path < 0 || path > 3 || n <= 0 || !apf || !x || !usel || !p_out || !mu_out) return fail(MI3D_EINVAL, "bad arguments to mi3d_debug_phase");
    const bool tables = h->npf > 0;
    if (tables && (h->dirty_phase || !h->d_tmu.p)) return fail(MI3D_ESTATE, "mi3d_debug_phase: the phase tables are not built (call mi3d_prepare)");
    const bool staged = tables && (path == 1 || path == 2);
    size_t lds = sizeof(DevCold);
    if (staged) {
        if (tab_lo < 0 || tab_n < 1 || tab_n > h->npf - tab_lo)
            return fail(MI3D_EINVAL, "mi3d_debug_phase: tables %d .. %d are not among the %d loaded", tab_lo, tab_lo + tab_n - 1, h->npf);
        lds += lean_tab_floats(h->nang, tab_n) * sizeof(float);
        if (lds > 64 * 1024) return fail(MI3D_EINVAL, "mi3d_debug_phase: %d tables of %d angles do not fit the LDS (%zu bytes)", tab_n, h->nang, lds);
    }
    for (int i = 0; i < n; ++i) {
        if (path == 3 && !(apf[i] < 1.0f)) return fail(MI3D_EINVAL, "mi3d_debug_phase: path 3 takes analytic selectors only (apf[%d] = %g)", i, (double)apf[i]);
        if (staged && apf[i] >= 1.0f) {
            const float t = apf[i] - 1.0f;
            int i0 = (int)std::floor(t), i1 = t > (float)i0 ? i0 + 1 : i0;
            if (i0 >= h->npf - 1) i0 = i1 = h->npf - 1;
            if (i0 < tab_lo || i1 > tab_lo + tab_n - 1)
                return fail(MI3D_EINVAL, "mi3d_debug_phase: apf[%d] = %g refers to a table outside the staged %d .. %d", i, (double)apf[i], tab_lo, tab_lo + tab_n - 1);
        }
    }
    DevCold C;
    memset(&C, 0, sizeof(C));
    if (tables) {
        C.nang = h->nang; C.npf = h->npf; C.tmu = h->d_tmu.p; C.tp = h->d_tp.p; C.tcdf = h->d_tcdf.p;
        C.tmu_idx = h->d_tmuidx.p; C.tcdf_idx = h->d_tcdfidx.p;
        if (staged) { C.tab_lo = tab_lo; C.tab_n = tab_n; }
    }
    DevBuf<DevCold> d_cold;
    DevBuf<float> d_in, d_out;
    const size_t m = (size_t)n;
    auto done = [&](int code) { d_cold.release(); d_in.release(); d_out.release(); return code; };
    if ((rc = d_cold.upload(&C, 1)) || (rc = d_in.alloc(3 * m)) || (rc = d_out.alloc(2 * m))) return done(rc);
    if (hipMemcpy(d_in.p, apf, m * sizeof(float), hipMemcpyHostToDevice) != hipSuccess || hipMemcpy(d_in.p + m, x, m * sizeof(float), hipMemcpyHostToDevice) != hipSuccess ||
        hipMemcpy(d_in.p + 2 * m, usel, m * sizeof(float), hipMemcpyHostToDevice) != hipSuccess)
        return done(fail(MI3D_EDEVICE, "mi3d_debug_phase: copy to the device failed"));
    const unsigned nblk = (unsigned)std::min<size_t>((m + 255) / 256, 1024);
    hipLaunchKernelGGL(k_debug_phase, dim3(nblk), dim3(256), lds, h->stream, d_cold.p, path, n, d_in.p, d_in.p + m, d_in.p + 2 * m, d_out.p, d_out.p + m);
    hipError_t e = hipGetLastError();
    if (e == hipSuccess) e = sync_main(h);
    if (e == hipSuccess) e = hipMemcpy(p_out, d_out.p, m * sizeof(float), hipMemcpyDeviceToHost);
    if (e == hipSuccess) e = hipMemcpy(mu_out, d_out.p + m, m * sizeof(float), hipMemcpyDeviceToHost);
    if (e != hipSuccess) return done(fail(MI3D_EDEVICE, "mi3d_debug_phase: %s", hipGetErrorString(e)));
    return done(MI3D_OK);
}

}
```

### er3t_amd/csrc/mi3d_device.h

```cpp
#pragma once

#include <hip/hip_runtime.h>
#include <stdint.h>

#include "../../include/mi3d.h"
#include "mi3d_diag.h"

namespace mi3d {

constexpr float kPi = 3.14159265358979323846f;
constexpr int kLayStride = 16;
constexpr int kMaxLayers = 512;
constexpr float kTauCut = 16.0f;

constexpr int kTargetPlainPhase = 0x100;
constexpr int kTargetRayleigh1d = 0x200;
constexpr int kTargetHeatPath = 0x400;
constexpr int kLayIn3d = 1;
constexpr int kLayStep3d = 2;

struct LayerRec {
    float dz;
    float bt;
    float zlo;
    int flags;
    float ks1d[MI3D_MAX_NP1D];
    float apf1d[MI3D_MAX_NP1D];
    float tabove;
    float tauz;
    int run_lo, run_hi;
};
static_assert(sizeof(LayerRec) == kLayStride * sizeof(float), "LayerRec layout");

struct ViewRec {
    float vx, vy, vz;
    float zs;
    int column;
    int roulette;
    float zreg;
    int point;
};
static_assert(sizeof(ViewRec) == 32, "ViewRec layout");

struct CamRec {
    float cx, cy, cz;
    float r2min;
    float zx, zy, zz;
    float cos_half;
    float xx, xy, xz;
    float inv_du;
    float yx, yy, yz;
    float inv_dv;
};
static_assert(sizeof(CamRec) == 64, "CamRec layout");
constexpr int kCamPoint = 1, kCamRect = 2, kCamCos = 4, kCamWrap = 8;

struct DevCold {
    float ztoa, zref, inv_Lx, inv_Ly;
    int nang, npf;
    const float *tmu, *tp, *tcdf;
    int tab_lo, tab_n;
    int sfc_mtype, nxb, nyb;
    float sfc_p0, sfc_p1, sfc_p2, sfc_sx, sfc_sy;
    const float *sfc2d;
    const LayerRec *lay;
    const ViewRec *views;
    unsigned long long *counters;
    float Lx, Ly;
    float inv_nx, inv_ny;
    float inv_dx, inv_dy;
    float sdx, sdy, sdz, cos_cone;
    const float2 *csca;
    const float *tcol0;
    unsigned long long *next_photon;
    float le_tau1;
    float sfc_p3;
    const uint32_t *order;
    float sfc_p4;
    int ev_cap;
    const CamRec *cams;
    float4 *ev_list;
    unsigned long long *ev_ctr;
    unsigned long long *hv_list;
    double *heat;
    float le_cmin;
    unsigned cam_images;
    const float4 *entry;
    const uint32_t *tile_end;
    int win_tc, win_ntx;
    int win_ntile;
    unsigned win_off;
    const uint16_t *tmu_idx;
    const uint16_t *tcdf_idx;
};
static_assert(sizeof(DevCold) == 304, "DevCold is staged in LDS as 19 float4");
constexpr int kTabNB = 512;
constexpr int kTabIdxN = kTabNB + 2;
__host__ __device__ inline int tab_bucket_mu(float mu) { const int b = (int)(fmaf(mu, 0.5f, 0.5f) * (float)kTabNB); return b < 0 ? 0 : (b > kTabNB - 1 ? kTabNB - 1 : b); }
__host__ __device__ inline int tab_bucket_u(float u) { const int b = (int)(u * (float)kTabNB); return b < 0 ? 0 : (b > kTabNB - 1 ? kTabNB - 1 : b); }
constexpr int kWin = 64;
constexpr int kEntryF4 = 3;
__host__ __device__ inline size_t entry_f4(size_t n) { return ((n + 63) / 64) * 64 * (size_t)kEntryF4; }
__host__ __device__ inline unsigned entry_index(unsigned pos) { return (pos >> 6) * (64u * (unsigned)kEntryF4) + (pos & 63u); }
constexpr int kEvStride = 64;
constexpr int kEvBlockF4 = 3 * 64 + 16;
__host__ __device__ inline size_t ev_list_f4(size_t cap) { return (cap / 64) * kEvBlockF4; }
__host__ __device__ inline unsigned ev_index(unsigned slot) { return (slot >> 6) * (unsigned)kEvBlockF4 + (slot & 63u); }
__host__ __device__ inline unsigned ev_word(unsigned slot) { return ((slot >> 6) * (unsigned)kEvBlockF4 + 192u) * 4u + (slot & 63u); }
constexpr unsigned kEvBlock = 512;
constexpr unsigned kCtrCursor = 9, kCtrHeavyFill = 17, kCtrHeavyCursor = 25, kCtrWords = 33;
constexpr int kCtrStride = 16;
constexpr int kColdF4 = sizeof(DevCold) / 16;

typedef double tally_t;
constexpr int kRadLine = 16;

struct DevScene {
    int nz, k3lo, nx, ny, nz3, np1d, np3d;
    int kdir;
    float dx, dy;
    float pix_sx, pix_sy;
    unsigned vcol_f4, vrow_f4;
    const float *bext3;
    const float4 *vrec;
    int nview, nmarch, nxr, nyr;
    int col0;
    int target, solver;
    float wmin, wfac;
    int rad_row;
    int rad_stride;
    tally_t *rad;
    tally_t *flux;
    const DevCold *cold;
};

typedef float vf4_t __attribute__((ext_vector_type(4)));
typedef unsigned vu2_t __attribute__((ext_vector_type(2)));
__device__ inline float4 nt_load(const float4 *p) { const vf4_t v = __builtin_nontemporal_load(reinterpret_cast<const vf4_t *>(p)); return make_float4(v.x, v.y, v.z, v.w); }
__device__ inline void nt_store(float4 *p, const float4 v) { __builtin_nontemporal_store((vf4_t){v.x, v.y, v.z, v.w}, reinterpret_cast<vf4_t *>(p)); }
__device__ inline uint2 nt_load(const uint2 *p) { const vu2_t v = __builtin_nontemporal_load(reinterpret_cast<const vu2_t *>(p)); return make_uint2(v.x, v.y); }
__device__ inline void nt_store(uint2 *p, const uint2 v) { __builtin_nontemporal_store((vu2_t){v.x, v.y}, reinterpret_cast<vu2_t *>(p)); }
#define MI3D_GLOBAL_AS __attribute__((address_space(1)))
template <class T> __device__ __forceinline__ const T *sgpr_ptr(const T *p) {
    const unsigned long long v = (unsigned long long)p;
    return reinterpret_cast<const T *>(((unsigned long long)(unsigned)__builtin_amdgcn_readfirstlane((int)(v >> 32)) << 32) | (unsigned)__builtin_amdgcn_readfirstlane((int)v));
}
__device__ __forceinline__ uint32_t glb_load_u32(const void *ubase, const unsigned byte_off) {
    return *reinterpret_cast<const MI3D_GLOBAL_AS uint32_t *>((const MI3D_GLOBAL_AS char *)ubase + byte_off);
}
template <bool NTL> __device__ __forceinline__ float4 glb_load_f4(const void *ubase, const unsigned byte_off) {
    const MI3D_GLOBAL_AS vf4_t *p = reinterpret_cast<const MI3D_GLOBAL_AS vf4_t *>((const MI3D_GLOBAL_AS char *)ubase + byte_off);
    const vf4_t v = NTL ? __builtin_nontemporal_load(p) : *p;
    return make_float4(v.x, v.y, v.z, v.w);
}
#ifndef MI3D_ENTRY_NT_LOAD
#define MI3D_ENTRY_NT_LOAD 1
#endif
#ifndef MI3D_TL_NT
#define MI3D_TL_NT 9
#endif

__device__ inline float frcp(float x) { return __builtin_amdgcn_rcpf(x); }
__device__ inline float fsqrt(float x) { return __builtin_amdgcn_sqrtf(x); }
__device__ inline float frsq(float x) { return __builtin_amdgcn_rsqf(x); }

__device__ inline uint32_t xor3_key(uint32_t a, uint32_t b, uint32_t k) {
    uint32_t r;
    asm("v_bitop3_b32 %0, %1, %2, %3 bitop3:0x96" : "=v"(r) : "v"(a), "v"(b), "s"(k));
    return r;
}

__device__ inline void philox4x32_10(uint32_t c0, uint32_t c1, uint32_t c2, uint32_t c3,
                                     uint32_t k0, uint32_t k1, uint32_t out[4]) {
#pragma unroll
    for (int r = 0; r < 10; ++r) {
        const uint64_t p0 = (uint64_t)0xD2511F53u * c0;
        const uint64_t p1 = (uint64_t)0xCD9E8D57u * c2;
        const uint32_t n0 = xor3_key((uint32_t)(p1 >> 32), c1, k0);
        const uint32_t n1 = (uint32_t)p1;
        const uint32_t n2 = xor3_key((uint32_t)(p0 >> 32), c3, k1);
        const uint32_t n3 = (uint32_t)p0;
        c0 = n0; c1 = n1; c2 = n2; c3 = n3;
        k0 += 0x9E3779B9u;
        k1 += 0xBB67AE85u;
    }
    out[0] = c0; out[1] = c1; out[2] = c2; out[3] = c3;
// ... 459 lines not shown
```

### er3t_amd/csrc/mi3d_kernel_lean.hip

```cpp
#include "mi3d_device.h"
#include "mi3d_diag.h"

namespace mi3d {

#ifndef MI3D_LEAN_THRESH
#define MI3D_LEAN_THRESH 16
#endif
#ifndef MI3D_LEAN_PASS
#define MI3D_LEAN_PASS 2
#endif
#ifndef MI3D_LEAN_EMIT4
#define MI3D_LEAN_EMIT4 1
#endif
#ifndef MI3D_LEAN_EMIT_GRID
#define MI3D_LEAN_EMIT_GRID 5
#endif
#ifndef MI3D_LEAN_FAST
#define MI3D_LEAN_FAST 1
#endif
#ifndef MI3D_LEAN_THRESH_EMIT
#define MI3D_LEAN_THRESH_EMIT 24
#endif
#ifndef MI3D_LEAN_FAST_PASS
#define MI3D_LEAN_FAST_PASS 8
#endif
#ifndef MI3D_LEAN_RARE_T
#define MI3D_LEAN_RARE_T 0
#endif
#ifndef MI3D_LEAN_WIN_EMIT
#define MI3D_LEAN_WIN_EMIT 0
#endif
#ifndef MI3D_LEAN_B4_DEFER
#define MI3D_LEAN_B4_DEFER 1
#endif
#ifndef MI3D_LEAN_PEND
#define MI3D_LEAN_PEND 1
#endif
constexpr unsigned kWinNone = 0xffffffffu;
constexpr int kWinCtl = 24;
constexpr size_t kWinLds = (size_t)kWin * kWin * sizeof(float) + kWinCtl * sizeof(unsigned);
#ifndef MI3D_LEAN_WAVES
#define MI3D_LEAN_WAVES(COUNT, MARCH) (((COUNT) || (MARCH)) ? 4 : 6)
#endif

constexpr int M_COLLU = 12;
constexpr int M_UNIFW = 13;
constexpr int M_SETUP = 14;
constexpr int M_DRAWR = 15;
constexpr int M_DRAWL = 16;
constexpr int M_ENTRY = 17;

template <bool COUNT, bool P3D, int MARCH, int MIX, int NT = 256>
#ifndef MI3D_LEAN_REG_WAVES
#define MI3D_LEAN_REG_WAVES(COUNT, MARCH) MI3D_LEAN_WAVES(COUNT, MARCH)
#endif
#ifndef MI3D_GEN_NARROW_WAVES
#define MI3D_GEN_NARROW_WAVES 6
#endif
__global__ void __launch_bounds__(NT, (MIX >= 2 && NT == 256 && MARCH == 0 && !COUNT) ? MI3D_GEN_NARROW_WAVES : MI3D_LEAN_REG_WAVES(COUNT, MARCH == 2 && MI3D_LEAN_EMIT4))
k_transport_lean(const DevScene S, const uint64_t nphoton, const uint64_t seed, const uint64_t offset) {
    static_assert(MARCH == 0 || MARCH == 2, "marched views go through event records and k_rays");
    static_assert(MIX >= 0 && MIX <= 3 && (NT == 256 || NT == 512), "builds");
    constexpr bool MIXED = (MARCH != 0), EMIT = (MARCH == 2), TWO = (MIX == 1), GEN = (MIX >= 2), RAY1 = (MIX == 3);
    constexpr unsigned NW = NT / 64;
    extern __shared__ float4 smem[];
    constexpr int kL4 = kLayStride / 4;
    const float4 *lay4 = smem + kL4;
    const LayerRec *lay = reinterpret_cast<const LayerRec *>(lay4);
    const int o_view = (S.nz + 2) * kL4;
    const ViewRec *views = reinterpret_cast<const ViewRec *>(smem + o_view);
    const DevCold *cold = reinterpret_cast<const DevCold *>(smem + o_view + MI3D_MAX_VIEW * 2);
    float *wbuf = reinterpret_cast<float *>(smem + o_view + MI3D_MAX_VIEW * 2 + kColdF4);
    unsigned *wctl = reinterpret_cast<unsigned *>(wbuf + kWin * kWin);
#define WLD(i_) __hip_atomic_load(wctl + (i_), __ATOMIC_SEQ_CST, __HIP_MEMORY_SCOPE_WORKGROUP)
#define WLDS(i_) ((unsigned)__builtin_amdgcn_readfirstlane((int)WLD(i_)))
#define WST(i_, v_) __hip_atomic_store(wctl + (i_), (unsigned)(v_), __ATOMIC_SEQ_CST, __HIP_MEMORY_SCOPE_WORKGROUP)
    const bool win_on = (!EMIT || MI3D_LEAN_WIN_EMIT) && S.cold->tile_end != nullptr;
    if (win_on) {
        for (int i = threadIdx.x; i < kWin * kWin; i += blockDim.x) wbuf[i] = 0.0f;
        if (threadIdx.x < kWinCtl) WST(threadIdx.x, (threadIdx.x < 2) ? kWinNone : 0u);
    }
    const float *ltab = nullptr;
    if (GEN && S.cold->tab_n > 0) {
        float *dst = win_on ? reinterpret_cast<float *>(wctl + kWinCtl) : wbuf;
        stage_tables(S.cold, dst);
        ltab = dst;
    }
    {
        const float4 *src = reinterpret_cast<const float4 *>(S.cold->lay);
        for (int i = threadIdx.x; i < S.nz * kL4; i += blockDim.x) smem[kL4 + i] = src[i];
        if (threadIdx.x < 2 * kL4) smem[threadIdx.x < kL4 ? threadIdx.x : (S.nz + 1) * kL4 + (threadIdx.x - kL4)] = make_float4(0.0f, 0.0f, 0.0f, 0.0f);
        const float4 *vsrc = reinterpret_cast<const float4 *>(S.cold->views);
        for (int i = threadIdx.x; i < S.nview * 2; i += blockDim.x) smem[o_view + i] = vsrc[i];
        const float4 *csrc = reinterpret_cast<const float4 *>(S.cold);
        if (threadIdx.x < kColdF4) smem[o_view + MI3D_MAX_VIEW * 2 + threadIdx.x] = csrc[threadIdx.x];
    }
    __syncthreads();

    const bool ipa_all = (S.solver == MI3D_SOLVER_IPA);
    const bool same_grid = (S.nxr == S.nx) && (S.nyr == S.ny);
    const bool plain = !GEN && (S.target & kTargetPlainPhase) != 0;
    const LeanTab T = GEN ? lean_tab(cold, ltab) : LeanTab{};
    const int np1d = (GEN && !RAY1) ? S.np1d : 1;
    const bool two3 = TWO || (GEN && !RAY1 && S.np3d > 1);
    const bool ray1 = RAY1 || (GEN && (S.target & kTargetRayleigh1d) != 0);
#define IPA_NOW() (ipa_all || (P3D && !direct))
    Counters cnt = {};
    const unsigned sx_b = S.vcol_f4 * 16u, sy_b = S.vrow_f4 * 16u;
    const char *vbase = reinterpret_cast<const char *>(S.vrec) - (long)S.k3lo * 16;
#define VREC(ix_, iy_, k_) (*reinterpret_cast<const float4 *>(vbase + ((unsigned)(iy_) * sy_b + (unsigned)(ix_) * sx_b + (unsigned)(k_) * 16u)))

    float px = 0, py = 0, pz = 0, ux = 0, uy = 0, uz = 1, iux = 1, iuy = 1, iuz = 1;
    float t = 0, tx = 0, ty = 0, tz = 0;
    int ix = 0, iy = 0, k = 0, stepx = 0, stepy = 0;
    int wrapx = 0, wrapy = 0;
    float rem = 0.0f;
    float w = 0.0f;
    float u1 = 0, u2 = 0, u3 = 0;
    uint32_t lid = 0;
#define PHOTON_ID() (offset + (uint64_t)lid)
    uint32_t draw = 0;
    int mode = M_NEED, kind = E_LAUNCH;
    bool direct = false;
    unsigned pool_next = 0, pool_left = 0;
    const unsigned xcc = __builtin_amdgcn_s_getreg((3 << 11) | 20) & 7u;
    unsigned victim = 0;
    unsigned nphot_wave = 0;
    int pend_pix = -1;
    float pend_val = 0.0f;
    const unsigned wave_w = (unsigned)__builtin_amdgcn_readfirstlane((int)(threadIdx.x >> 6));
    unsigned my_pass = 0;
    static_assert(kWin == 64, "the window's place arithmetic");
    unsigned worg = 0x80008000u, worg2 = 0x80008000u;
    const int jv_col = MIXED ? S.col0 : 0;
    typedef unsigned short us2_t __attribute__((ext_vector_type(2)));
#define RAD_TALLY(key_, val_)                                                                                                    \
    do {                                                                                                                         \
        MI3D_WIN_ANY(COUNT, cnt);                                                                                                    \
        const us2_t k2_ = __builtin_bit_cast(us2_t, (unsigned)(key_));                                                           \
        const us2_t d2_ = __builtin_elementwise_min(k2_ - __builtin_bit_cast(us2_t, worg), k2_ - __builtin_bit_cast(us2_t, worg2)); \
        const unsigned d_ = __builtin_bit_cast(unsigned, d2_);                                                                   \
        if ((d_ & ~((unsigned)(kWin - 1) * 0x10001u)) == 0u) {                                                                   \
            atomicAdd(&wbuf[(d_ >> (16 - 6)) | (d_ & (unsigned)(kWin - 1))], (val_));                                            \
            MI3D_WIN_HIT(COUNT, cnt);                                                                                                      \
        } else {                                                                                                                 \
            const int ir_ = (key_) & 0xffff, jr_ = (int)((unsigned)(key_) >> 16);                                                \
            RAD_ADD(&S.rad[(unsigned)((jv_col * S.nyr + jr_) * S.rad_row + ir_) * (unsigned)S.rad_stride], (val_));              \
        }                                                                                                                        \
    } while (0)
    auto win_flush = [&]() {
        const unsigned bo = WLD(1);
        if (bo == kWinNone) return;
        const int bx = (int)(bo & 0xffffu), by = (int)(bo >> 16);
        for (int i = threadIdx.x & 63; i < kWin * kWin; i += 64) {
            const float v = __hip_atomic_exchange(&wbuf[i], 0.0f, __ATOMIC_RELAXED, __HIP_MEMORY_SCOPE_WORKGROUP);
            if (v != 0.0f) {
                int ir = bx + (i & (kWin - 1)), jr = by + i / kWin;
                ir -= ir >= S.nxr ? S.nxr : 0; jr -= jr >= S.nyr ? S.nyr : 0;
                RAD_ADD(&S.rad[(unsigned)((jv_col * S.nyr + jr) * S.rad_row + ir) * (unsigned)S.rad_stride], v);
            }
        }
    };
    float4 rec = make_float4(0.0f, 0.0f, 0.0f, 0.0f);
    float &bt_ev = rec.x, &ev_tab = rec.y, &ev_ks0 = rec.z, &ev_apf0 = rec.w;
    float ev_ksb = 0.0f, ev_apfb = 0.0f;
    float &ev_sfc = ev_tab;
    bool emit = false;
    unsigned long long ev_lo = 0, ev_hi = 0;

#define MI3D_ENTRY_UNPACK()                                                                                          \
    do {                                                                                                             \
        const unsigned cell_ = (unsigned)ix, km_ = (unsigned)k;                                                      \
        ix = (int)(cell_ & 0xffffu); iy = (int)(cell_ >> 16);                                                        \
        k = (int)(km_ & 0xffffu);                                                                                    \
        mode = ((km_ >> 16) & 0x7fffu) == (unsigned)M_FLY ? M_SETUP : M_UNIF;                                        \
        if (COUNT && (km_ >> 31)) cnt.steps++;                  \
    } while (0)
#define MI3D_TICK(slot) MI3D_DIAG_TICK(COUNT, cnt, tick, slot)
#define MI3D_TICKC(slot, census_slot) MI3D_FPC_TICK(COUNT, cnt, tick, slot, census_slot)
    long long tick = COUNT ? clock64() : 0; (void)tick;
    unsigned pass_ctr = 0;
    for (;;) {
        if (win_on) {
            my_pass++;
            asm volatile("" ::: "memory");
            if ((threadIdx.x & 63) == 0) __hip_atomic_store(wctl + 8 + wave_w, my_pass, __ATOMIC_RELAXED, __HIP_MEMORY_SCOPE_WORKGROUP);
            asm volatile("" ::: "memory");
            const unsigned o_ = (unsigned)__builtin_amdgcn_readfirstlane((int)__hip_atomic_load(wctl, __ATOMIC_RELAXED, __HIP_MEMORY_SCOPE_WORKGROUP));
            asm volatile("" ::: "memory");
            worg = o_ == kWinNone ? 0x80008000u : o_;
            worg2 = o_ == kWinNone ? 0x80008000u : (((o_ & 0xffffu) - (unsigned)S.nxr) & 0xffffu) | (((o_ >> 16) - (unsigned)S.nyr) << 16);
        }
        MI3D_MARK("A");
        for (;;) {
            const bool flying = (mode == M_FLY);
            const int nfly = __popcll(__ballot(flying));
            if (nfly == 0) break;
            if (nfly < (EMIT ? MI3D_LEAN_THRESH_EMIT : MI3D_LEAN_THRESH) && __ballot(mode != M_FLY && mode != M_DONE) != 0ull) break;
            if (COUNT) { cnt.a_slots++; if (flying) cnt.a_lanes++; }
            if (flying) {
                const float tn = fminf(fminf(tx, ty), tz);
                const float dtau = rec.x * (tn - t);
                if (COUNT) { cnt.steps++; cnt.steps3d++; }
                MI3D_DIAG_CLEAR_STEP(COUNT, cnt, rec.z, dtau >= rem);
                if (dtau >= rem) mode = M_COLL;
                else {
                    rem -= dtau;
                    t = tn;
                    const bool zf = (tz == tn), xf = !zf && (tx == tn), yf = !zf && !xf;
                    const int cx = ix + stepx, cy = iy + stepy;
                    const int cxw = (unsigned)cx >= (unsigned)S.nx ? wrapx : cx, cyw = (unsigned)cy >= (unsigned)S.ny ? wrapy : cy;
                    ix = xf ? cxw : ix;
                    iy = yf ? cyw : iy;
                    const float txn = fmaf(S.dx, iux, tx), tyn = fmaf(S.dy, iuy, ty);
                    tx = xf ? txn : tx;
                    ty = yf ? tyn : ty;
                    if (zf) {
                        k += uz > 0.0f ? 1 : -1;
                        const float4 Ln = lay4[k * kL4];
                        tz = fmaf(Ln.x, iuz, tz);
                        if (!(__float_as_int(Ln.w) & kLayStep3d)) mode = M_UNIFW;
                    }
                    if (mode == M_FLY) rec = VREC(ix, iy, k);
                }
            }
        }

        MI3D_TICK(0);
        MI3D_MARK("BSCHED");
        if (COUNT) { cnt.b_slots++; if (mode != M_FLY && mode != M_DONE) cnt.b_lanes++; }
        bool full_ = MI3D_LEAN_FAST_PASS <= 1 || ((pass_ctr++ % (unsigned)(MI3D_LEAN_FAST_PASS)) == 0u) || __ballot(mode == M_COLL) == 0ull;
        if (MI3D_LEAN_RARE_T > 0 && !full_) full_ = __popcll(__ballot(mode != M_FLY && mode != M_DONE && mode != M_COLL)) >= MI3D_LEAN_RARE_T;
        const bool full = full_;
        MI3D_FPC(COUNT, cnt, 1, le_steps, !full && mode != M_FLY && mode != M_DONE && mode != M_COLL);
        MI3D_FPC(COUNT, cnt, 1, le_steps3d, full);

        MI3D_MARK("C");
        bool fastc = (mode == M_COLL);
        float c_kstot = 0.0f, c_ks1 = 0.0f;
        if (fastc) {
            const float4 L = lay4[k * kL4];
            const LayerRec &Lk = lay[k];
            const float ks1 = Lk.ks1d[0];
            const float ibt = frcp(rec.x);
            const float tc = fmaf(rem, ibt, t);
            const float ax = __builtin_amdgcn_fmed3f((tx - tc) * floor_abs(ux), 0.0f, S.dx);
            const float ay = __builtin_amdgcn_fmed3f((ty - tc) * floor_abs(uy), 0.0f, S.dy);
            const float az = __builtin_amdgcn_fmed3f((tz - tc) * floor_abs(uz), 0.0f, L.x);
            px = ux > 0.0f ? S.dx - ax : ax;
            py = uy > 0.0f ? S.dy - ay : ay;
            pz = uz > 0.0f ? L.x - az : az;
            if (COUNT) cnt.scatter++;
            const float ks3 = rec.z;
            float kstot = ks1 + ks3;
            if (GEN && !ray1) for (int ip = 1; ip < np1d; ++ip) kstot += Lk.ks1d[ip];
            if (two3) {
                const float2 cs = cold->csca[((unsigned)(iy * S.nx + ix) * (unsigned)S.nz3 + (unsigned)(k - S.k3lo)) * 2u + 1u];
// ... 281 lines not shown
            if (kind != E_LAUNCH) direct = false;
            if (!(w > 0.0f)) { if (COUNT) cnt.absorbed++; mode = M_NEED; }
            else {
                mode = M_DRAW;
                if (w < S.wmin) { if (COUNT) cnt.roulette++; mode = M_DRAWR; }
            }
        }

        MI3D_TICKC(4, 1);
        MI3D_MARK("B6");
        if (mode == M_DRAW || mode == M_DRAWR || mode == M_DRAWL) {
            float r0, r1, r2, r3;
            draw4_fast<!EMIT>(seed, PHOTON_ID(), draw++, r0, r1, r2, r3);
            if (mode == M_DRAW) {
                rem = -0.69314718f * __builtin_amdgcn_logf(r0);
                u1 = r1; u2 = r2; u3 = r3;
                mode = (lay[k].flags & kLayStep3d) ? M_SETUP : M_UNIF;
                MI3D_FPC(COUNT, cnt, 1, flux_tally, mode == M_UNIF);
            } else if (mode == M_DRAWR) {
                MI3D_FPC(COUNT, cnt, 1, flux_tally, r0 * S.wfac < w);
                if (r0 * S.wfac < w) { w = S.wfac; mode = M_DRAW; }
                else { if (COUNT) cnt.killed++; mode = M_NEED; }
            } else {
                float x = r0 * cold->Lx, y = r1 * cold->Ly;
                if (x >= cold->Lx) x = 0.0f;
                if (y >= cold->Ly) y = 0.0f;
                ix = min((int)(x * cold->inv_dx), S.nx - 1);
                iy = min((int)(y * cold->inv_dy), S.ny - 1);
                px = fminf(fmaxf(x - (float)ix * S.dx, 0.0f), S.dx);
                py = fminf(fmaxf(y - (float)iy * S.dy, 0.0f), S.dy);
                k = S.nz - 1;
                pz = lay[k].dz;
                ux = cold->sdx; uy = cold->sdy; uz = cold->sdz;
                u2 = 1.0f - r2 * (1.0f - cold->cos_cone);
                u3 = r3;
                w = 1.0f;
                direct = true;
                kind = E_LAUNCH;
                mode = M_FINISH;
            }
        }
        MI3D_TICKC(5, 1);

        MI3D_MARK("B4");
        MI3D_FPC(COUNT, cnt, 2, flux_tally, mode == M_NEED);
        const bool ended = mode == M_NEED && draw != 0;
        nphot_wave += (unsigned)__popcll(__ballot(ended));
        if (ended) draw = 0;
        bool took = false;
        for (;;) {
            const unsigned long long need = __ballot(mode == M_NEED);
            if (need == 0ull) break;
            if (pool_left == 0u) {
                const int leader = __ffsll((long long)need) - 1;
                bool got = false;
                while (victim < 8u) {
                    const unsigned x = (xcc + victim) & 7u;
                    const unsigned long long lo = (nphoton * x) >> 3, hi = (nphoton * (x + 1u)) >> 3;
                    const unsigned piece = (unsigned)(hi - lo);
                    unsigned long long b = 0;
                    if ((int)(threadIdx.x & 63) == leader) b = atomicAdd(cold->next_photon + x * kCtrStride, (unsigned long long)kChunk);
                    const unsigned b32 = (unsigned)__builtin_amdgcn_readlane((int)b, leader);
                    if (b32 < piece) {
                        pool_next = (unsigned)lo + b32;
                        pool_left = min(piece - b32, (unsigned)kChunk);
                        got = true;
                        break;
                    }
                    victim++;
                }
                if (!got) {
                    if (mode == M_NEED) mode = M_DONE;
                    break;
                }
            }
            const unsigned rank = __builtin_amdgcn_mbcnt_hi((unsigned)(need >> 32), __builtin_amdgcn_mbcnt_lo((unsigned)need, 0u));
            const unsigned take = min((unsigned)__popcll(need), pool_left);
            if (mode == M_NEED && rank < pool_left) {
                const uint32_t *order = sgpr_ptr(cold->order);
                const float4 *entry = sgpr_ptr(cold->entry);
                lid = order ? glb_load_u32(order + pool_next, rank * 4u) : pool_next + rank;
                if (entry) {
                    const unsigned j = (pool_next & 63u) + rank;
                    const float4 *eb = entry + (size_t)(pool_next >> 6) * (size_t)(64 * kEntryF4);
                    const unsigned eo = ((j >> 6) * (unsigned)(64 * kEntryF4) + (j & 63u)) * 16u;
                    const float4 q0 = glb_load_f4<MI3D_ENTRY_NT_LOAD != 0>(eb, eo), q1 = glb_load_f4<MI3D_ENTRY_NT_LOAD != 0>(eb, eo + 1024u), q2 = glb_load_f4<MI3D_ENTRY_NT_LOAD != 0>(eb, eo + 2048u);
                    px = q0.x; py = q0.y; pz = q0.z; rem = q0.w;
                    ux = q1.x; uy = q1.y; uz = q1.z; u1 = q1.w;
                    u2 = q2.x; u3 = q2.y;
                    ix = __float_as_int(q2.z); k = __float_as_int(q2.w);
                    mode = M_ENTRY;
                    w = 1.0f; direct = true; draw = 2;
                    kind = E_LAUNCH;
#if !MI3D_LEAN_B4_DEFER
                    MI3D_ENTRY_UNPACK();
#endif
                } else {
                    draw = 0;
                    mode = M_DRAWL;
                }
            }
            took = true;
            pool_next += take; pool_left -= take;
        }
        MI3D_TICKC(-1, 3);
        if (ended && pend_pix >= 0) { RAD_TALLY(pend_pix, pend_val); pend_pix = -1; }
        if (win_on) {
            const bool lane0 = (threadIdx.x & 63) == 0;
            if (WLDS(2) == wave_w + 1u) {
                bool clear = true;
                for (unsigned q = 0; q < NW; ++q) {
                    const unsigned c = WLDS(8 + q);
                    if (q != wave_w && !(c != WLDS(8 + NW + q) || c == kWinNone)) clear = false;
                }
                if (clear) {
                    win_flush();
                    const unsigned pos = WLDS(6);
                    const uint32_t *tend = sgpr_ptr(cold->tile_end);
                    const int ntile = __builtin_amdgcn_readfirstlane(cold->win_ntile);
                    int t = 0;
                    for (int j = 0; j < ntile; j += 64) {
                        const int q = j + (int)(threadIdx.x & 63);
                        t += __popcll(__ballot(q < ntile && tend[q] <= pos));
                    }
                    t = min(t, ntile - 1);
                    const unsigned lo = t > 0 ? tend[t - 1] : 0u, hi = tend[t];
                    const int ntx = cold->win_ntx, tc = cold->win_tc;
                    const int ty = t / ntx, tb = t - ty * ntx, tx = (ty & 1) ? ntx - 1 - tb : tb;
                    int ox = tx * tc + (int)(cold->win_off & 0xffffu), oy = ty * tc + (int)(cold->win_off >> 16);
                    while (ox >= S.nxr) ox -= S.nxr;
                    while (oy >= S.nyr) oy -= S.nyr;
                    if (lane0) {
                        WST(4, lo); WST(5, hi);
                        WST(1, (unsigned)ox | ((unsigned)oy << 16));
                        WST(0, (unsigned)ox | ((unsigned)oy << 16));
                        WST(2, 0u);
                    }
                }
            } else if (took) {
                const unsigned pos = pool_next - 1u;
                if ((pos < WLDS(4) || pos >= WLDS(5)) && WLDS(2) == 0u) {
                    unsigned won = 0u;
                    if (lane0) won = atomicCAS(wctl + 2, 0u, wave_w + 1u) == 0u ? 1u : 0u;
                    won = (unsigned)__builtin_amdgcn_readfirstlane((int)won);
                    if (won) {
                        if (lane0) {
                            WST(0, kWinNone);
                            for (unsigned q = 0; q < NW; ++q) WST(8 + NW + q, WLD(8 + q));
                            WST(6, pos);
                        }
                    }
                }
            }
        }
        if (mode == M_ENTRY) MI3D_ENTRY_UNPACK();
        MI3D_TICKC(3, 5);

        MI3D_MARK("B7");
        if (mode == M_SETUP) {
            const float4 L = lay4[k * kL4];
            iux = frcp(floor_abs(ux)); iuy = frcp(floor_abs(uy)); iuz = frcp(floor_abs(uz));
            tx = (ux > 0.0f ? S.dx - px : px) * iux;
            ty = (uy > 0.0f ? S.dy - py : py) * iuy;
            tz = (uz > 0.0f ? L.x - pz : pz) * iuz;
            t = 0.0f;
            const bool ipa = IPA_NOW();
            stepx = ipa ? 0 : (ux > 0.0f ? 1 : -1);
            stepy = ipa ? 0 : (uy > 0.0f ? 1 : -1);
            wrapx = ux > 0.0f ? 0 : S.nx - 1; wrapy = uy > 0.0f ? 0 : S.ny - 1;
            rec = VREC(ix, iy, k);
            mode = M_FLY;
        }
        MI3D_TICKC(5, 1);
        }

        MI3D_MARK("END");
        if (__ballot(mode != M_DONE) == 0ull) break;
    }
#undef MI3D_TICK
#undef MI3D_TICKC
#undef MI3D_ENTRY_UNPACK
    if (win_on) {
        unsigned nd = 0u;
        if ((threadIdx.x & 63) == 0) { WST(8 + wave_w, kWinNone); nd = atomicAdd(wctl + 3, 1u); }
        nd = (unsigned)__builtin_amdgcn_readfirstlane((int)nd);
        if (nd == NW - 1u) win_flush();
    }

    if (EMIT) {
        for (unsigned long long q = ev_lo + (threadIdx.x & 63); q < ev_hi; q += 64)
            if (q < (unsigned long long)S.cold->ev_cap) S.cold->ev_list[ev_list_f4(S.cold->ev_cap) * xcc + ev_index((unsigned)q)] = make_float4(0.0f, 0.0f, 0.0f, 0.0f);
    }
    {
        uint32_t vals[24] = {(threadIdx.x & 63) == 0 ? nphot_wave : 0u, cnt.steps, cnt.steps3d, cnt.scatter, cnt.surface, cnt.le_rays,
                             cnt.le_steps, cnt.le_steps3d, cnt.le_column, cnt.flux_tally, cnt.roulette,
                             cnt.killed, cnt.escaped, cnt.absorbed, cnt.a_lanes, cnt.a_slots, cnt.b_lanes, cnt.b_slots,
                             cnt.cyc[0], cnt.cyc[1], cnt.cyc[2], cnt.cyc[3], cnt.cyc[4], cnt.cyc[5]};
        const int ncnt = COUNT ? 24 : 1;
        for (int q = 0; q < ncnt; ++q) {
            unsigned long long v = vals[q];
            for (int off = 32; off > 0; off >>= 1) v += __shfl_down(v, off, 64);
            if ((threadIdx.x & 63) == 0 && v) atomicAdd(&S.cold->counters[q], v);
        }
    }
#undef IPA_NOW
#undef VREC
#undef PHOTON_ID
}

#ifdef MI3D_ONLY_HEADLINE
template __global__ void k_transport_lean<false, false, 0, 0>(const DevScene, const uint64_t, const uint64_t, const uint64_t);
#else
#define MI3D_LEAN_INST(C, P) template __global__ void k_transport_lean<C, P, 0, 0>(const DevScene, const uint64_t, const uint64_t, const uint64_t); \
                             template __global__ void k_transport_lean<C, P, 2, 0>(const DevScene, const uint64_t, const uint64_t, const uint64_t); \
                             template __global__ void k_transport_lean<C, P, 0, 1>(const DevScene, const uint64_t, const uint64_t, const uint64_t); \
                             template __global__ void k_transport_lean<C, P, 2, 1>(const DevScene, const uint64_t, const uint64_t, const uint64_t); \
                             template __global__ void k_transport_lean<C, P, 0, 2>(const DevScene, const uint64_t, const uint64_t, const uint64_t); \
                             template __global__ void k_transport_lean<C, P, 2, 2>(const DevScene, const uint64_t, const uint64_t, const uint64_t); \
                             template __global__ void k_transport_lean<C, P, 0, 2, 512>(const DevScene, const uint64_t, const uint64_t, const uint64_t); \
                             template __global__ void k_transport_lean<C, P, 0, 3>(const DevScene, const uint64_t, const uint64_t, const uint64_t); \
                             template __global__ void k_transport_lean<C, P, 0, 3, 512>(const DevScene, const uint64_t, const uint64_t, const uint64_t);
MI3D_LEAN_INST(false, false) MI3D_LEAN_INST(false, true) MI3D_LEAN_INST(true, false) MI3D_LEAN_INST(true, true)
#undef MI3D_LEAN_INST
#endif

struct EntryArgs {
    const LayerRec *lay;
    float Lx, Ly, dx, dy, inv_dx, inv_dy, inv_nx, inv_ny;
    float sdx, sdy, sdz, cos_cone;
    int nx, ny, nz, solver, target, kdir;
};

__global__ void __launch_bounds__(256)
k_entry(const EntryArgs A, const uint64_t nphoton, const uint64_t seed, const uint64_t offset, const uint32_t *__restrict__ order, float4 *__restrict__ entry) {
    const LayerRec *lay = A.lay;
    const bool ipa = (A.solver == MI3D_SOLVER_IPA);
    {
        const unsigned i = blockIdx.x * 256u + threadIdx.x;
        if (i >= (unsigned)nphoton) return;
        const uint64_t id = offset + (uint64_t)(order ? order[i] : i);
        float r0, r1, r2, r3;
        draw4_fast(seed, id, 0u, r0, r1, r2, r3);
        float x = r0 * A.Lx, y = r1 * A.Ly;
        if (x >= A.Lx) x = 0.0f;
        if (y >= A.Ly) y = 0.0f;
        int ix = min((int)(x * A.inv_dx), A.nx - 1);
        int iy = min((int)(y * A.inv_dy), A.ny - 1);
        float px = fminf(fmaxf(x - (float)ix * A.dx, 0.0f), A.dx);
        float py = fminf(fmaxf(y - (float)iy * A.dy, 0.0f), A.dy);
        int k = A.nz - 1;
        float pz = lay[k].dz;
        float ux = A.sdx, uy = A.sdy, uz = A.sdz;
        const float mu_cone = 1.0f - r2 * (1.0f - A.cos_cone);
        if (!(A.cos_cone >= 1.0f)) rotate_dir(ux, uy, uz, mu_cone, r3);
        draw4_fast(seed, id, 1u, r0, r1, r2, r3);
        float rem = -0.69314718f * __builtin_amdgcn_logf(r0);
        int mode = (lay[k].flags & kLayStep3d) ? M_FLY : M_UNIF;
        unsigned ran = 0u;
        if (mode == M_UNIF) {
            const bool up = uz > 0.0f;
            const LayerRec Lk = lay[k];
            const int kend = up ? Lk.run_hi : Lk.run_lo;
            const LayerRec Le = lay[kend];
            const float tv = up ? (Le.tauz + Le.bt * Le.dz - Lk.tauz) - Lk.bt * pz
                                : (Lk.tauz - Le.tauz) + Lk.bt * pz;
            const float hv = up ? (Le.zlo + Le.dz) - (Lk.zlo + pz) : (Lk.zlo + pz) - Le.zlo;
            const float iuzl = frcp(fmaxf(fabsf(uz), 1e-20f));
            const float tpath = tv * iuzl;
            const int knew = up ? kend + 1 : kend - 1;
            const bool no_tally = !(A.target & MI3D_TARGET_FLUX) || (!up && min(k, A.kdir - 1) < knew + 1);
            if (tpath < rem && knew >= 0 && knew < A.nz && no_tally) {
                rem -= tpath;
                const float s = hv * iuzl;
                px += ux * s; py += uy * s;
                k = knew;
                pz = up ? 0.0f : lay[knew].dz;
                fold_xy_raw(A.dx, A.dy, A.nx, A.ny, A.inv_dx, A.inv_dy, A.inv_nx, A.inv_ny, px, py, ix, iy, ipa);
                mode = M_FLY;
                ran = 1u;
            }
        }
        typedef float vf4 __attribute__((ext_vector_type(4)));
        vf4 *e = reinterpret_cast<vf4 *>(entry) + entry_index(i);
        __builtin_nontemporal_store((vf4){px, py, pz, rem}, e);
        __builtin_nontemporal_store((vf4){ux, uy, uz, r1}, e + 64);
        __builtin_nontemporal_store((vf4){r2, r3, __uint_as_float((unsigned)ix | ((unsigned)iy << 16)), __uint_as_float((unsigned)k | ((unsigned)mode << 16) | (ran << 31))}, e + 128);
    }
}

}
```

### er3t_amd/csrc/mi3d_kernels.hip

```cpp
#include "mi3d_device.h"
#include "mi3d_diag.h"

namespace mi3d {

__global__ void __launch_bounds__(256)
k_build_grid(int nx, int ny, int nz3, int k3lo, int np3d, const float *bt1d, const float *abst,
             const float *extp, const float *omgp, const float *apfp, float4 *vrec, float2 *csca, unsigned vcol_f4, unsigned vrow_f4, float *bext3) {
    const long nvox = (long)nx * ny * nz3;
    const long v = (long)blockIdx.x * blockDim.x + threadIdx.x;
    if (v >= nvox) return;
    const int ix = (int)(v % nx);
    const int iy = (int)((v / nx) % ny);
    const int k3 = (int)(v / ((long)nx * ny));
    float bt = bt1d[k3lo + k3];
    if (abst) bt += abst[v];
    const long o = ((long)iy * nx + ix) * nz3 + k3;
    float ks0 = 0.0f, apf0 = 0.0f;
    for (int ip = 0; ip < np3d; ++ip) {
        const float e = extp[ip * nvox + v];
        bt += e;
        float2 c = make_float2(omgp[ip * nvox + v] * e, apfp[ip * nvox + v]);
        if (!(c.x > 0.0f)) c.y = 0.0f;
        if (ip == 0) { ks0 = c.x; apf0 = c.y; }
        if (np3d > 1) csca[o * np3d + ip] = c;
// ... 187 lines not shown
__global__ void __launch_bounds__(256)
k_get_net_heating(const ThermalGrid G, const double *__restrict__ tally, double norm, double src_flx, float *__restrict__ out) {
#pragma clang fp contract(off)
    const size_t n = (size_t)G.nz * G.ny * G.nx;
    const size_t i = (size_t)blockIdx.x * blockDim.x + threadIdx.x;
    if (i >= n) return;
    const int k = (int)(i / ((size_t)G.ny * G.nx)), col = (int)(i % ((size_t)G.ny * G.nx)), iy = col / G.nx, ix = col % G.nx;
    const bool in3d = G.nz3 > 0 && k >= G.k3lo && k < G.k3lo + G.nz3;
    const double emit = src_flx * cell_emission(G, k, iy, ix, in3d).e;
    out[i] = tally ? (float)(tally[i] * norm / (double)G.lay[k].dz - emit) : (float)emit;
}

constexpr int kScanT = 256, kScanR = 8, kScanChunk = kScanT * kScanR;
__global__ void __launch_bounds__(256)
k_scan_chunk(double *a, unsigned long n, double *bsum) {
    __shared__ double s[kScanT];
    const unsigned t = threadIdx.x;
    const unsigned long base = (unsigned long)blockIdx.x * kScanChunk + (unsigned long)t * kScanR;
    double v[kScanR], run = 0.0;
#pragma unroll
    for (int r = 0; r < kScanR; ++r) { run += base + r < n ? a[base + r] : 0.0; v[r] = run; }
    s[t] = run;
    __syncthreads();
    for (unsigned off = 1; off < kScanT; off <<= 1) {
        const double x = t >= off ? s[t - off] : 0.0;
        __syncthreads();
        s[t] += x;
        __syncthreads();
    }
    const double before = t > 0 ? s[t - 1] : 0.0;
#pragma unroll
    for (int r = 0; r < kScanR; ++r) if (base + r < n) a[base + r] = v[r] + before;
    if (t == kScanT - 1) bsum[blockIdx.x] = s[kScanT - 1];
}
__global__ void __launch_bounds__(1024)
k_scan_top(double *bsum, unsigned long nb) {
    __shared__ double s[1024];
    const unsigned t = threadIdx.x;
    double carry = 0.0;
    for (unsigned long c0 = 0; c0 < nb; c0 += 1024) {
        const double x0 = c0 + t < nb ? bsum[c0 + t] : 0.0;
        s[t] = x0;
        __syncthreads();
        for (unsigned off = 1; off < 1024; off <<= 1) {
            const double x = t >= off ? s[t - off] : 0.0;
            __syncthreads();
            s[t] += x;
            __syncthreads();
        }
        if (c0 + t < nb) bsum[c0 + t] = carry + s[t] - x0;
        carry += s[1023];
        __syncthreads();
    }
}
__global__ void __launch_bounds__(256)
k_scan_add(double *a, unsigned long n, const double *bsum) {
    const double off = bsum[blockIdx.x];
    const unsigned long base = (unsigned long)blockIdx.x * kScanChunk;
    for (unsigned r = threadIdx.x; r < (unsigned)kScanChunk; r += blockDim.x)
        if (base + r < n) a[base + r] += off;
}

__device__ inline double u01_pair(uint32_t a, uint32_t b) {
    return ((double)(a >> 9) + ((double)(b >> 9) + 0.5) * (1.0 / 8388608.0)) * (1.0 / 8388608.0);
}

struct BinGeom {
    float Lx, Ly, inv_tx, inv_ty;
    int nx, ny;
    int tcols, ntx, nty;
};
constexpr int kMaxTiles = 1024;

__device__ inline int launch_tile(const BinGeom G, uint64_t seed, uint64_t id) {
    uint32_t w[4];
    philox4x32_10((uint32_t)id, (uint32_t)(id >> 32), 0u, 0u, (uint32_t)seed, (uint32_t)(seed >> 32), w);
    float x = u01(w[0]) * G.Lx, y = u01(w[1]) * G.Ly;
    if (x >= G.Lx) x = 0.0f;
    if (y >= G.Ly) y = 0.0f;
    const int tx = min((int)(x * G.inv_tx), G.ntx - 1), ty = min((int)(y * G.inv_ty), G.nty - 1);
    return ty * G.ntx + ((ty & 1) ? G.ntx - 1 - tx : tx);
}

__global__ void __launch_bounds__(256)
k_bin_count(const BinGeom G, uint64_t seed, uint64_t offset, uint32_t n, uint16_t *tile, uint32_t *hist) {
    __shared__ uint32_t lh[kMaxTiles];
    const int nt = G.ntx * G.nty;
    for (int i = threadIdx.x; i < nt; i += blockDim.x) lh[i] = 0u;
    __syncthreads();
    for (uint32_t i = blockIdx.x * blockDim.x + threadIdx.x; i < n; i += gridDim.x * blockDim.x) {
        const int t = launch_tile(G, seed, offset + i);
        tile[i] = (uint16_t)t;
        atomicAdd(&lh[t], 1u);
    }
    __syncthreads();
    for (int i = threadIdx.x; i < nt; i += blockDim.x)
        if (lh[i]) atomicAdd(&hist[i], lh[i]);
}

__global__ void __launch_bounds__(256)
k_bin_scan(int nt, const uint32_t *hist, uint32_t *cursor) {
    static_assert(kMaxTiles == 4 * 256, "four tiles per thread");
    __shared__ uint32_t s[256];
    const int t = threadIdx.x;
    uint32_t h[4], sum = 0u;
    for (int j = 0; j < 4; ++j) { h[j] = 4 * t + j < nt ? hist[4 * t + j] : 0u; sum += h[j]; }
    s[t] = sum;
    __syncthreads();
    for (int off = 1; off < 256; off <<= 1) {
        const uint32_t v = t >= off ? s[t - off] : 0u;
        __syncthreads();
        s[t] += v;
        __syncthreads();
    }
    uint32_t run = s[t] - sum;
    for (int j = 0; j < 4; ++j) { if (4 * t + j < nt) cursor[4 * t + j] = run; run += h[j]; }
}

constexpr int kScatterR = 16;
__global__ void __launch_bounds__(256)
k_bin_scatter(int nt, uint32_t n, uint32_t slab, const uint16_t *tile, uint32_t *cursor, uint32_t *order) {
    constexpr int NT = 256, CH = NT * kScatterR;
    __shared__ uint32_t lcount[kMaxTiles], lstart[kMaxTiles], gbase[kMaxTiles], part[NT / 64];
    __shared__ uint32_t sidx[CH];
    __shared__ uint16_t stile[CH];
    const unsigned tid = threadIdx.x;
    for (int i = tid; i < nt; i += NT) lcount[i] = 0u;
    __syncthreads();
    const uint32_t lo = blockIdx.x * slab, hi = min(n, lo + slab);
    for (uint32_t i = lo + tid; i < hi; i += NT) atomicAdd(&lcount[tile[i]], 1u);
    __syncthreads();
    for (int i = tid; i < nt; i += NT) gbase[i] = lcount[i] ? atomicAdd(&cursor[i], lcount[i]) : 0u;
    const int per = (nt + NT - 1) / NT;
    const int tlo = min((int)tid * per, nt), thi = min(tlo + per, nt);
    __syncthreads();
    for (uint32_t c0 = lo; c0 < hi; c0 += CH) {
        for (int i = tlo; i < thi; ++i) lcount[i] = 0u;
        __syncthreads();
        uint32_t t[kScatterR];
#pragma unroll
        for (int r = 0; r < kScatterR; ++r) {
            const uint32_t i = c0 + (uint32_t)(r * NT) + tid;
            t[r] = i < hi ? (uint32_t)tile[i] : 0xffffffffu;
            if (t[r] != 0xffffffffu) atomicAdd(&lcount[t[r]], 1u);
        }
        __syncthreads();
        uint32_t sum = 0;
        for (int i = tlo; i < thi; ++i) sum += lcount[i];
        uint32_t incl = sum;
        for (int off = 1; off < 64; off <<= 1) {
            const uint32_t x = __shfl_up(incl, off, 64);
            if ((tid & 63u) >= (unsigned)off) incl += x;
        }
        if ((tid & 63u) == 63u) part[tid >> 6] = incl;
        __syncthreads();
        uint32_t before = 0, total = 0;
        for (unsigned wv = 0; wv < (unsigned)(NT / 64); ++wv) { const uint32_t x = part[wv]; total += x; if (wv < (tid >> 6)) before += x; }
        uint32_t run = before + incl - sum;
        for (int i = tlo; i < thi; ++i) {
            const uint32_t c = lcount[i];
            lstart[i] = run; lcount[i] = run;
            run += c;
        }
        __syncthreads();
#pragma unroll
        for (int r = 0; r < kScatterR; ++r)
            if (t[r] != 0xffffffffu) {
                const uint32_t p = atomicAdd(&lcount[t[r]], 1u);
                sidx[p] = c0 + (uint32_t)(r * NT) + tid;
                stile[p] = (uint16_t)t[r];
            }
        __syncthreads();
        for (uint32_t j = tid; j < total; j += NT) {
            const uint32_t tt = stile[j];
            order[gbase[tt] + (j - lstart[tt])] = sidx[j];
        }
        __syncthreads();
        for (int i = tlo; i < thi; ++i) gbase[i] += lcount[i] - lstart[i];
    }
}

__global__ void __launch_bounds__(256)
k_fold_rad(tally_t *__restrict__ acc, tally_t *__restrict__ tally, int stride, int n, int nxr, int rad_row) {
    const int i = blockIdx.x * blockDim.x + threadIdx.x;
    if (i >= n) return;
    const size_t a = ((size_t)(i / nxr) * rad_row + (size_t)(i % nxr)) * stride;
    const tally_t v = acc[a];
    if (v != 0.0) { tally[i] += v; acc[a] = 0.0; }
}

__global__ void __launch_bounds__(256)
k_stats_add(const tally_t *__restrict__ tally, float *__restrict__ run_acc, const float *__restrict__ factor,
            double norm, int plane, int nlevel, int down_lo, const double *__restrict__ dir_level, int n,
            const double *__restrict__ add_px, double add_scale) {
#pragma clang fp contract(off)
    const int i = blockIdx.x * blockDim.x + threadIdx.x;
    if (i >= n) return;
    double t = tally[i];
    if (down_lo >= 0 && i >= down_lo && i < 2 * down_lo) t += tally[i - down_lo];
    const double a = add_px ? add_px[i] * add_scale : (dir_level && i < 2 * down_lo) ? dir_level[(i / plane) % nlevel] : 0.0;
    const float v = (float)(t * norm + a);
    const float f = factor[(i / plane) % nlevel];
    const float prod = v * f;
    run_acc[i] = run_acc[i] + prod;
}

__global__ void __launch_bounds__(256)
k_get_field(const tally_t *__restrict__ tally, float *__restrict__ out, double norm, unsigned plane, unsigned nlevel, long down_lo,
            const double *__restrict__ add, size_t n) {
#pragma clang fp contract(off)
    const size_t i = (size_t)blockIdx.x * blockDim.x + threadIdx.x;
    if (i >= n) return;
    double t = tally[i];
    const unsigned lev = (unsigned)((i / plane) % nlevel);
    if (down_lo >= 0) {
        if (i >= (size_t)down_lo && i < 2 * (size_t)down_lo) t += tally[i - (size_t)down_lo];
        const double a = (add && i < 2 * (size_t)down_lo) ? add[lev] : 0.0;
        out[i] = (float)(t * norm + a);
    } else if (add) out[i] = (float)(t * norm / add[lev]);
    else out[i] = (float)(t * norm);
}

constexpr double kCamDirTauMax = 100.0;
__global__ void __launch_bounds__(64)
k_cam_direct(int nview, int nxr, int nyr, const CamRec *__restrict__ cams, const ViewRec *__restrict__ views, const double *__restrict__ zgrd,
             const LayerRec *__restrict__ lay, int nz, int nx, int ny, int nz3, int k3lo, double dx, double dy, const float *__restrict__ bext3,
             double sx, double sy, double sz, double *__restrict__ out) {
    const int iv = blockIdx.x * blockDim.x + threadIdx.x;
    if (iv >= nview) return;
    const CamRec Cm = cams[iv];
    const float dxc = (float)sx * Cm.xx + (float)sy * Cm.xy + (float)sz * Cm.xz, dyc = (float)sx * Cm.yx + (float)sy * Cm.yy + (float)sz * Cm.yz;
    const float dzc = fminf((float)sx * Cm.zx + (float)sy * Cm.zy + (float)sz * Cm.zz, 1.0f);
    if (dzc < Cm.cos_half) return;
    int ir, jr;
    float val;
    if (!cam_pixel(Cm, views[iv].point, reinterpret_cast<const float *>(cams + nview) + iv * nxr, nxr, nyr, dxc, dyc, dzc, 1.0f, ir, jr, val)) return;
    double x = Cm.cx, y = Cm.cy, z = fmax((double)Cm.cz, zgrd[0]);
    double tau = 0.0;
    int k = 0;
    while (k < nz && zgrd[k + 1] <= z) ++k;
    for (; k < nz && tau <= kCamDirTauMax; ++k) {
        const double ztop = zgrd[k + 1];
        if (!(nz3 > 0 && k >= k3lo && k < k3lo + nz3)) {
            const double t = (ztop - z) / sz;
            tau += (double)lay[k].bt * t;
            x += sx * t; y += sy * t; z = ztop;
            continue;
        }
        long ixu = (long)floor(x / dx), iyu = (long)floor(y / dy);
        for (;;) {
            const double tz = (ztop - z) / sz;
            const double tx = sx > 0.0 ? ((double)(ixu + 1) * dx - x) / sx : sx < 0.0 ? ((double)ixu * dx - x) / sx : INFINITY;
            const double ty = sy > 0.0 ? ((double)(iyu + 1) * dy - y) / sy : sy < 0.0 ? ((double)iyu * dy - y) / sy : INFINITY;
            double t = tz;
            int axis = 2;
            if (tx < t) { t = tx; axis = 0; }
            if (ty < t) { t = ty; axis = 1; }
            t = fmax(t, 0.0);
            const long ix = ((ixu % nx) + nx) % nx, iy = ((iyu % ny) + ny) % ny;
            tau += (double)bext3[((size_t)iy * nx + ix) * nz3 + (k - k3lo)] * t;
            x += sx * t; y += sy * t; z += sz * t;
// ... 868 lines not shown
```

### er3t_amd/solver.py

```python

import ctypes as C
import os

import numpy as np

from .scene import Scene, TARGET_FLUX, TARGET_RADIANCE, TARGET_HEAT

__all__ = ['Mi3dSolver', 'load_library', 'library_path', 'COUNTER_NAMES']

MAX_VIEW = 16
NCOUNTER = 24
COUNTER_NAMES = ['photons', 'steps', 'steps3d', 'scatter', 'surface', 'le_rays', 'le_steps', 'le_steps3d',
                 'le_column', 'flux_tally', 'roulette', 'killed', 'escaped', 'absorbed',
                 'sched_a_lanes', 'sched_a_slots', 'sched_b_lanes', 'sched_b_slots',
                 'ticks_a', 'ticks_b0', 'ticks_b12', 'ticks_b34', 'ticks_b5', 'ticks_b6']

_fp  = C.POINTER(C.c_float)
_dp  = C.POINTER(C.c_double)
_u64 = C.c_uint64
_LIB = None

_SIGNATURES = [
    ('mi3d_version'            , C.c_int   , []),
    ('mi3d_last_error'         , C.c_char_p, []),
    ('mi3d_device_count'       , C.c_int   , []),
    ('mi3d_create'             , C.c_int   , [C.c_int, C.POINTER(C.c_void_p)]),
    ('mi3d_destroy'            , C.c_int   , [C.c_void_p]),
    ('mi3d_set_atm1d'          , C.c_int   , [C.c_void_p, C.c_int, _dp, C.c_int, _fp, _fp, _fp, _fp]),
    ('mi3d_set_atm3d'          , C.c_int   , [C.c_void_p, C.c_int, C.c_int, C.c_int, C.c_int, C.c_int, C.c_double, C.c_double, _fp, _fp, _fp, _fp]),
    ('mi3d_set_phase'          , C.c_int   , [C.c_void_p, C.c_int, C.c_int, _fp, _fp]),
    ('mi3d_set_surface'        , C.c_int   , [C.c_void_p, C.c_int, _fp]),
    ('mi3d_set_surface2d'      , C.c_int   , [C.c_void_p, C.c_int, C.c_int, _fp, _fp, _fp]),
    ('mi3d_set_source'         , C.c_int   , [C.c_void_p, C.c_double, C.c_double, C.c_double, C.c_double]),
    ('mi3d_set_thermal'        , C.c_int   , [C.c_void_p, C.c_int, C.c_double, C.c_int, _fp, _fp, _fp]),
    ('mi3d_set_solar_irradiance', C.c_int  , [C.c_void_p, C.c_double]),
    ('mi3d_get_source_power'   , C.c_int   , [C.c_void_p, _dp, _dp]),
    ('mi3d_set_views'          , C.c_int   , [C.c_void_p, C.c_int, _dp, _dp, _dp, C.c_double, C.c_int, C.c_int]),
    ('mi3d_set_cameras'        , C.c_int   , [C.c_void_p, C.c_int] + [_dp]*10 + [C.c_int, C.c_int]),
    ('mi3d_set_camera_map'     , C.c_int   , [C.c_void_p, C.c_int, C.c_int]),
    ('mi3d_set_options'        , C.c_int   , [C.c_void_p, C.c_int, C.c_int, C.c_double, C.c_double, C.c_int]),
    ('mi3d_set_le_roulette'    , C.c_int   , [C.c_void_p, C.c_double]),
    ('mi3d_set_le_weight_roulette', C.c_int, [C.c_void_p, C.c_double]),
    ('mi3d_set_counting'       , C.c_int   , [C.c_void_p, C.c_int]),
    ('mi3d_bind_device_buffers', C.c_int   , [C.c_void_p, C.c_void_p, C.c_void_p, C.c_void_p]),
    ('mi3d_bind_heating_buffer', C.c_int   , [C.c_void_p, C.c_void_p]),
    ('mi3d_set_heating_estimator', C.c_int , [C.c_void_p, C.c_int]),
    ('mi3d_prepare'            , C.c_int   , [C.c_void_p]),
    ('mi3d_reset'              , C.c_int   , [C.c_void_p]),
    ('mi3d_run'                , C.c_int   , [C.c_void_p, _u64, _u64, _u64]),
    ('mi3d_sync'               , C.c_int   , [C.c_void_p]),
    ('mi3d_last_kernel'        , C.c_char_p, [C.c_void_p]),
    ('mi3d_set_kernel'         , C.c_int   , [C.c_void_p, C.c_int]),
    ('mi3d_set_tuning'         , C.c_int   , [C.c_void_p, C.c_char_p, C.c_int]),
    ('mi3d_get_timing'         , C.c_int   , [C.c_void_p, _dp, C.POINTER(_u64)]),
    ('mi3d_get_radiance'       , C.c_int   , [C.c_void_p, _u64, _fp]),
    ('mi3d_get_flux'           , C.c_int   , [C.c_void_p, _u64, _fp]),
    ('mi3d_get_direct_levels'  , C.c_int   , [C.c_void_p, _dp]),
    ('mi3d_get_camera_direct'  , C.c_int   , [C.c_void_p, _dp]),
    ('mi3d_get_heating'        , C.c_int   , [C.c_void_p, _u64, _fp]),
    ('mi3d_get_emission'       , C.c_int   , [C.c_void_p, _fp]),
    ('mi3d_get_counters'       , C.c_int   , [C.c_void_p, C.POINTER(_u64)]),
    ('mi3d_stats_begin'        , C.c_int   , [C.c_void_p, C.c_void_p, C.c_void_p]),
    ('mi3d_stats_set_analytic_share', C.c_int, [C.c_void_p, C.c_double]),
    ('mi3d_stats_add'          , C.c_int   , [C.c_void_p, _u64, _fp, _fp]),
    ('mi3d_stats_join'         , C.c_int   , [C.c_void_p, C.c_void_p]),
    ('mi3d_stats_chain'        , C.c_int   , [C.c_void_p, C.c_void_p]),
    ('mi3d_stats_end_run'      , C.c_int   , [C.c_void_p, _fp, _fp]),
    ('mi3d_stats_get'          , C.c_int   , [C.c_void_p, C.c_int, _fp, _fp, C.POINTER(C.c_int)]),
    ('mi3d_debug_philox'       , C.c_int   , [C.c_void_p, _u64, _u64, C.c_uint32, C.c_int, C.POINTER(C.c_uint32)]),
    ('mi3d_debug_order'        , C.c_int   , [C.c_void_p, _u64, C.POINTER(C.c_uint32), C.POINTER(C.c_uint32), C.c_int]),
    ('mi3d_debug_thermal'      , C.c_int   , [C.c_void_p, C.POINTER(C.c_double), C.POINTER(C.c_double), _u64]),
    ('mi3d_debug_phase_tables' , C.c_int   , [C.c_void_p, C.c_int, C.c_int, _fp, _fp, _fp, C.POINTER(C.c_uint16), C.POINTER(C.c_uint16)]),
    ('mi3d_debug_phase'        , C.c_int   , [C.c_void_p, C.c_int, C.c_int, C.c_int, C.c_int, _fp, _fp, _fp, _fp, _fp]),
]

TAB_IDX_N = 514


def library_path():
    return os.environ.get('MI3D_LIBRARY') or os.path.join(os.path.dirname(os.path.abspath(__file__)), 'libmi3drt.so')


def load_library():


    global _LIB
    if _LIB is None:
        path = library_path()
        if not os.path.exists(path):
            msg = 'Error [Mi3dSolver]: Cannot find <%s>. Build it with `python -c "import __graft_entry__ as g; g.build()"`.' % path
            raise OSError(msg)
        lib = C.CDLL(path)
        for name, restype, argtypes in _SIGNATURES:
            try:
                fn = getattr(lib, name)
            except AttributeError:
                if os.environ.get('MI3D_LIBRARY'):
                    setattr(lib, name, _stale(name, path))
                    continue
                msg = 'Error [Mi3dSolver]: <%s> is stale: it lacks <%s>. Rebuild it with `make -C er3t_amd/csrc`.' % (path, name)
                raise OSError(msg)
            fn.restype  = restype
            fn.argtypes = argtypes
        _LIB = lib
    return _LIB


def _stale(name, path):
    def missing(*args):
        msg = 'Error [Mi3dSolver]: library is stale: <%s> missing from <%s>.' % (name, path)
        raise OSError(msg)
    return missing


def _ptr(a, typ=_fp):
    return None if a is None else a.ctypes.data_as(typ)


class Mi3dSolver:


    def __init__(self, device=0):
        self.lib = load_library()
        self._h  = C.c_void_p()
        self._chk(self.lib.mi3d_create(int(device), C.byref(self._h)))
        self.device = device
        self.scene  = None

    def _chk(self, rc):
        if rc != 0:
            msg = 'Error [Mi3dSolver]: %s (code %d).' % (self.lib.mi3d_last_error().decode('utf-8', 'replace'), rc)
            raise OSError(msg)

    def close(self):
        if getattr(self, '_h', None) is not None and self._h.value:
            self.lib.mi3d_destroy(self._h)
            self._h = C.c_void_p()

    def __del__(self):
        try:
            self.close()
        except Exception:
            pass

    def set_atm1d(self, zgrd, ext1d, omg1d, apf1d, abs1d):
        zgrd  = np.ascontiguousarray(zgrd, dtype=np.float64)
        ext1d = np.ascontiguousarray(np.atleast_2d(ext1d), dtype=np.float32)
        omg1d = np.ascontiguousarray(np.atleast_2d(omg1d), dtype=np.float32)
        apf1d = np.ascontiguousarray(np.atleast_2d(apf1d), dtype=np.float32)
        abs1d = np.ascontiguousarray(abs1d, dtype=np.float32)
        nz = zgrd.size - 1
        if ext1d.shape[1] != nz or omg1d.shape != ext1d.shape or apf1d.shape != ext1d.shape or abs1d.size != nz:
            raise ValueError('Error [Mi3dSolver]: 1-D profiles do not match <zgrd>.')
# ... 163 lines not shown
    def radiance(self, nphoton_total):
        out = np.zeros(self._shape_rad, dtype=np.float32)
        if out.size:
            self._chk(self.lib.mi3d_get_radiance(self._h, int(nphoton_total), _ptr(out)))
        return out

    def flux(self, nphoton_total):
        out = np.zeros(self._shape_flux, dtype=np.float32)
        self._chk(self.lib.mi3d_get_flux(self._h, int(nphoton_total), _ptr(out)))
        return out

    def direct_levels(self):
        out = np.zeros(self.scene.nz+1, dtype=np.float64)
        self._chk(self.lib.mi3d_get_direct_levels(self._h, _ptr(out, _dp)))
        return out

    def camera_direct(self):
        out = np.zeros(self._shape_rad, dtype=np.float64)
        if out.size:
            self._chk(self.lib.mi3d_get_camera_direct(self._h, _ptr(out, _dp)))
        return out

    def heating(self, nphoton_total):
        s = self.scene
        out = np.zeros((s.nz, s.ny, s.nx), dtype=np.float32)
        self._chk(self.lib.mi3d_get_heating(self._h, int(nphoton_total), _ptr(out)))
        return out

    def emission(self):
        s = self.scene
        out = np.zeros((s.nz, s.ny, s.nx), dtype=np.float32)
        self._chk(self.lib.mi3d_get_emission(self._h, _ptr(out)))
        return out

    def stats_begin(self, rad_run_ptr=None, flux_run_ptr=None):
        self._chk(self.lib.mi3d_stats_begin(self._h, C.c_void_p(rad_run_ptr or 0), C.c_void_p(flux_run_ptr or 0)))

    def stats_join(self, owner):
        self._chk(self.lib.mi3d_stats_join(self._h, owner._h))

    def stats_chain(self, after):
        self._chk(self.lib.mi3d_stats_chain(self._h, after._h))

    def stats_set_analytic_share(self, share):
        self._chk(self.lib.mi3d_stats_set_analytic_share(self._h, float(share)))

    def stats_add(self, nphoton_total, factor_rad=None, factor_flux=None):
        s = self.scene
        fr = ff = None
        if factor_rad is not None:
            fr = np.ascontiguousarray(np.broadcast_to(np.asarray(factor_rad, dtype=np.float32), (s.nview,)))
        if factor_flux is not None:
            ff = np.ascontiguousarray(np.broadcast_to(np.asarray(factor_flux, dtype=np.float32), (s.nz+1,)))
        self._chk(self.lib.mi3d_stats_add(self._h, int(nphoton_total), _ptr(fr), _ptr(ff)))

    def stats_end_run(self, keep=False):
        s = self.scene
        rad = np.zeros(self._shape_rad, dtype=np.float32) if keep and (s.target & TARGET_RADIANCE) else None
        flux = np.zeros(self._shape_flux, dtype=np.float32) if keep and (s.target & TARGET_FLUX) else None
        self._chk(self.lib.mi3d_stats_end_run(self._h, _ptr(rad), _ptr(flux)))
        out = {}
        if rad is not None:
            out['rad'] = rad
        if flux is not None:
            out['flux'] = flux
        return out

    def stats_get(self, which):
        shape = self._shape_rad if which == TARGET_RADIANCE else self._shape_flux
        mean = np.zeros(shape, dtype=np.float32); sdev = np.zeros(shape, dtype=np.float32); n = C.c_int(0)
        self._chk(self.lib.mi3d_stats_get(self._h, int(which), _ptr(mean), _ptr(sdev), C.byref(n)))
        return mean, sdev, int(n.value)

    def counters(self):
        out = np.zeros(NCOUNTER, dtype=np.uint64)
        self._chk(self.lib.mi3d_get_counters(self._h, out.ctypes.data_as(C.POINTER(_u64))))
        return dict(zip(COUNTER_NAMES, (int(v) for v in out)))

    def debug_order(self, n, ntile_max=1024):
        order = np.zeros(n, dtype=np.uint32); tend = np.zeros(ntile_max, dtype=np.uint32)
        self._chk(self.lib.mi3d_debug_order(self._h, int(n), order.ctypes.data_as(C.POINTER(C.c_uint32)), tend.ctypes.data_as(C.POINTER(C.c_uint32)), int(ntile_max)))
        return order, tend

    def debug_thermal(self, ncell):
        ptot = C.c_double(0.0); cdf = np.zeros(int(ncell), dtype=np.float64)
        self._chk(self.lib.mi3d_debug_thermal(self._h, C.byref(ptot), cdf.ctypes.data_as(C.POINTER(C.c_double)), int(ncell)))
        return float(ptot.value), cdf

    def debug_phase_tables(self, nang, npf):
        mu = np.zeros(nang, dtype=np.float32); p = np.zeros((npf, nang), dtype=np.float32); cdf = np.zeros((npf, nang), dtype=np.float32)
        mi = np.zeros(TAB_IDX_N, dtype=np.uint16); ci = np.zeros((npf, TAB_IDX_N), dtype=np.uint16)
        u16 = C.POINTER(C.c_uint16)
        self._chk(self.lib.mi3d_debug_phase_tables(self._h, int(nang), int(npf), _ptr(mu), _ptr(p), _ptr(cdf), _ptr(mi, u16), _ptr(ci, u16)))
        return mu, p, cdf, mi, ci

    def debug_phase(self, path, apf, x, usel=None, tab_lo=0, tab_n=0):
        x = np.ascontiguousarray(np.ravel(x), dtype=np.float32)
        apf = np.ascontiguousarray(np.broadcast_to(np.asarray(apf, dtype=np.float32), x.shape))
        usel = np.ascontiguousarray(np.broadcast_to(np.asarray(0.0 if usel is None else usel, dtype=np.float32), x.shape))
        p = np.zeros(x.size, dtype=np.float32); m = np.zeros(x.size, dtype=np.float32)
        self._chk(self.lib.mi3d_debug_phase(self._h, int(path), int(tab_lo), int(tab_n), x.size, _ptr(apf), _ptr(x), _ptr(usel), _ptr(p), _ptr(m)))
        return p, m

    def philox(self, seed, id0, draw, n):
        out = np.zeros((n, 4), dtype=np.uint32)
        self._chk(self.lib.mi3d_debug_philox(self._h, int(seed), int(id0), int(draw), int(n), out.ctypes.data_as(C.POINTER(C.c_uint32))))
        return out
```

### include/mi3d.h

```cpp
#ifndef MI3D_H
#define MI3D_H

#include <stdint.h>

#ifdef __cplusplus
extern "C" {
#endif

#define MI3D_VERSION 100

#define MI3D_OK 0
#define MI3D_EINVAL (-1)
#define MI3D_ESTATE (-2)
#define MI3D_EDEVICE (-3)
#define MI3D_EUNSUP (-4)

#define MI3D_MAX_NP1D 4
#define MI3D_MAX_NP3D 4
#define MI3D_MAX_VIEW 16
#define MI3D_NCOUNTER 24

#define MI3D_TARGET_FLUX 1
#define MI3D_TARGET_RADIANCE 2
#define MI3D_TARGET_HEAT 4
// ... 35 lines not shown

int mi3d_version(void);
const char *mi3d_last_error(void);

int mi3d_device_count(void);

int mi3d_create(int device, mi3d_solver **out);
int mi3d_destroy(mi3d_solver *h);

int mi3d_set_atm1d(mi3d_solver *h, int nz, const double *zgrd, int np1d, const float *ext,
                   const float *omg, const float *apf, const float *abs);

int mi3d_set_atm3d(mi3d_solver *h, int nx, int ny, int nz3, int iz3l, int np3d, double dx,
                   double dy, const float *abst, const float *extp, const float *omgp,
                   const float *apfp);

int mi3d_set_phase(mi3d_solver *h, int nang, int npf, const float *ang, const float *pha);

int mi3d_set_surface(mi3d_solver *h, int mtype, const float param[5]);

int mi3d_set_surface2d(mi3d_solver *h, int nxb, int nyb, const float *tmps, const float *jsfc,
                       const float *psfc);

int mi3d_set_source(mi3d_solver *h, double flx, double qmax_deg, double the_deg, double phi_deg);

int mi3d_set_thermal(mi3d_solver *h, int mtype, double wlen_um, int nlev, const float *tmp1d, const float *tmpa3d,
                     const float *tmps2d);

int mi3d_set_solar_irradiance(mi3d_solver *h, double fsol);
int mi3d_get_source_power(mi3d_solver *h, double *ptot, double *psol);

int mi3d_set_views(mi3d_solver *h, int nview, const double *the_deg, const double *phi_deg,
                   const double *zloc, double zref, int nxr, int nyr);

int mi3d_set_cameras(mi3d_solver *h, int ncam, const double *the_deg, const double *phi_deg, const double *psi_deg,
                     const double *xpos, const double *ypos, const double *zloc, const double *qmax_deg,
                     const double *umax_deg, const double *vmax_deg, const double *apsize, int nxr, int nyr);
int mi3d_set_camera_map(mi3d_solver *h, int mpmap, int mrproj);

int mi3d_set_options(mi3d_solver *h, int target, int solver, double wmin, double wfac, int column_le);

int mi3d_set_le_roulette(mi3d_solver *h, double tau1);
int mi3d_set_le_weight_roulette(mi3d_solver *h, double cmin);

int mi3d_set_counting(mi3d_solver *h, int on);

int mi3d_bind_device_buffers(mi3d_solver *h, void *rad_sum, void *flux_sum, void *stream);
int mi3d_bind_heating_buffer(mi3d_solver *h, void *heat_sum);

int mi3d_set_heating_estimator(mi3d_solver *h, int estimator);

int mi3d_prepare(mi3d_solver *h);

int mi3d_reset(mi3d_solver *h);

int mi3d_run(mi3d_solver *h, uint64_t nphoton, uint64_t seed, uint64_t photon_offset);

int mi3d_sync(mi3d_solver *h);
const char *mi3d_last_kernel(mi3d_solver *h);
int mi3d_set_kernel(mi3d_solver *h, int choice);
int mi3d_set_tuning(mi3d_solver *h, const char *key, int value);

int mi3d_get_timing(mi3d_solver *h, double *kernel_ms, uint64_t *launches);

int mi3d_get_radiance(mi3d_solver *h, uint64_t nphoton_total, float *out);
int mi3d_get_flux(mi3d_solver *h, uint64_t nphoton_total, float *out);
int mi3d_get_direct_levels(mi3d_solver *h, double *out);
int mi3d_get_camera_direct(mi3d_solver *h, double *out);
int mi3d_get_heating(mi3d_solver *h, uint64_t nphoton_total, float *out);
int mi3d_get_emission(mi3d_solver *h, float *out);
int mi3d_get_counters(mi3d_solver *h, uint64_t out[MI3D_NCOUNTER]);

int mi3d_stats_begin(mi3d_solver *h, void *rad_run, void *flux_run);
int mi3d_stats_join(mi3d_solver *h, mi3d_solver *owner);
int mi3d_stats_chain(mi3d_solver *h, mi3d_solver *after);
int mi3d_stats_set_analytic_share(mi3d_solver *h, double share);
int mi3d_stats_add(mi3d_solver *h, uint64_t nphoton_total, const float *factor_rad, const float *factor_flux);
int mi3d_stats_end_run(mi3d_solver *h, float *rad_run_out, float *flux_run_out);
int mi3d_stats_get(mi3d_solver *h, int which, float *mean, float *sdev, int *nrun);

int mi3d_debug_philox(mi3d_solver *h, uint64_t seed, uint64_t id0, uint32_t draw, int n,
                      uint32_t *out);
int mi3d_debug_order(mi3d_solver *h, uint64_t n, uint32_t *order_out, uint32_t *tile_end_out, int ntile_max);
int mi3d_debug_thermal(mi3d_solver *h, double *ptot, double *cdf_out, uint64_t n);
#define MI3D_TAB_IDX_N 514
int mi3d_debug_phase_tables(mi3d_solver *h, int nang, int npf, float *mu, float *p, float *cdf, uint16_t *mu_idx, uint16_t *cdf_idx);
int mi3d_debug_phase(mi3d_solver *h, int path, int tab_lo, int tab_n, int n, const float *apf, const float *x, const float *usel,
                     float *p_out, float *mu_out);

#ifdef __cplusplus
}
#endif
#endif
```

Before: 2.899 billion photons/s.

## Shrink entry records for collimated sources and rebuild photon binning without global atomics

For a collimated solar beam with no thermal source, photon entry records drop from three float4 to two. The shared direction is read from the cold scene struct and the layer thickness is re-derived in the transport kernel, which cuts entry-record write and read bandwidth. The tile binning is rewritten as a deterministic per-block histogram, a per-tile scan across blocks, and an LDS-staged scatter using per-wave counters. This replaces global atomic cursors and the separate memset. The scatter needs more dynamic LDS, and a new debug entry-dump API is added.

```diff
diff --git a/er3t_amd/csrc/mi3d_api.hip b/er3t_amd/csrc/mi3d_api.hip
--- a/er3t_amd/csrc/mi3d_api.hip
+++ b/er3t_amd/csrc/mi3d_api.hip
@@ -152,6 +152,7 @@
     DevBuf<unsigned long long> d_counters, d_next;
     DevBuf<uint32_t> d_hist;
     DevBuf<uint16_t> d_tile;
+    size_t bin_lds_set = 0;
     struct PreSet {
         DevBuf<uint32_t> order, cursor;
         DevBuf<float4> entry;
@@ -169,6 +170,9 @@
     bool cam_warned = false;
     bool general_warned = false;
     int entry_records = 1;
+    int entry_form_run = 0;
+    int entry_form_last = 0;
+    uint64_t entry_n_last = 0;
     struct EvSet {
         DevBuf<float4> events;
         DevBuf<unsigned long long> evctr, hvlist;
@@ -717,7 +721,7 @@
     { int v = 0; if (hipDeviceGetAttribute(&v, hipDeviceAttributeMaxSharedMemoryPerBlock, device) == hipSuccess && v >= 32768) h->lds_max = v; else (void)hipGetLastError(); }
     int rc;
     if ((rc = h->d_counters.alloc(MI3D_NCOUNTER)) || (rc = h->d_next.alloc(8 * kCtrStride)) ||
-        (rc = h->d_hist.alloc(kMaxTiles)) || (rc = h->pre[0].cursor.alloc(kMaxTiles))) { delete h; return rc; }
+        (rc = h->pre[0].cursor.alloc(kMaxTiles))) { delete h; return rc; }
     HIPCHK(hipMemset(h->d_counters.p, 0, MI3D_NCOUNTER * sizeof(unsigned long long)));
     HIPCHK(hipMemset(h->d_next.p, 0, 8 * kCtrStride * sizeof(unsigned long long)));
     {
@@ -740,7 +744,7 @@
     if (const char *e = getenv("MI3D_TALLY_WINDOW")) h->tally_window = atoi(e) ? 1 : 0;
     if (const char *e = getenv("MI3D_TALLY_LISTS")) h->tally_lists = atoi(e) ? 1 : 0;
     if (const char *e = getenv("MI3D_TALLY_RUNS")) h->tally_runs = atoi(e) ? 1 : 0;
-    if (const char *e = getenv("MI3D_ENTRY_RECORDS")) h->entry_records = atoi(e) ? 1 : 0;
+    if (const char *e = getenv("MI3D_ENTRY_RECORDS")) { const int v = atoi(e); h->entry_records = v == 2 ? 2 : (v ? 1 : 0); }
     if (const char *e = getenv("MI3D_OVERLAP_RAYS")) h->overlap_rays = atoi(e) ? 1 : 0;
     if (const char *e = getenv("MI3D_OVERLAP_SORT")) h->overlap_sort = std::max(0, std::min(2, atoi(e)));
     if (const char *e = getenv("MI3D_OVERLAP_PRE")) h->overlap_pre = std::max(0, std::min(2, atoi(e)));
@@ -1217,28 +1221,36 @@
 }
 
 static hipError_t launch_bins(mi3d_solver *h, hipStream_t st, const BinGeom &G, int ntile, uint64_t seed, uint64_t off, uint64_t nb, uint32_t *order, uint32_t *cursor) {
-    hipError_t err = hipMemsetAsync(h->d_hist.p, 0, kMaxTiles * sizeof(uint32_t), st);
-    if (err != hipSuccess) return err;
     const unsigned nblk = (unsigned)std::min<uint64_t>((nb + 4095) / 4096, 4096);
-    hipLaunchKernelGGL(k_bin_count, dim3(nblk), dim3(256), 0, st, G, seed, off, (uint32_t)nb, h->d_tile.p, h->d_hist.p);
-    hipLaunchKernelGGL(k_bin_scan, dim3(1), dim3(256), 0, st, ntile, h->d_hist.p, cursor);
-    const uint32_t slab = (uint32_t)((nb + nblk - 1) / nblk);
-    hipLaunchKernelGGL(k_bin_scatter, dim3(nblk), dim3(256), 0, st, ntile, (uint32_t)nb, slab, h->d_tile.p, cursor, order);
+    const uint32_t slab = (uint32_t)(((nb + nblk - 1) / nblk + 7) / 8 * 8);
+    uint32_t *bhist = h->d_hist.p, *hist = h->d_hist.p + (size_t)ntile * nblk;
+    const size_t lds = bin_scatter_lds(ntile);
+    if (lds > 65536 && lds > h->bin_lds_set) {
+        if (hipFuncSetAttribute(reinterpret_cast<const void *>(k_bin_scatter), hipFuncAttributeMaxDynamicSharedMemorySize, (int)lds) != hipSuccess) return hipGetLastError();
+        h->bin_lds_set = lds;
+    }
+    hipLaunchKernelGGL(k_bin_count, dim3(nblk), dim3(256), 0, st, G, seed, off, (uint32_t)nb, slab, h->d_tile.p, bhist);
+    hipLaunchKernelGGL(k_bin_scan, dim3((unsigned)ntile), dim3(256), 0, st, (int)nblk, bhist, hist);
+    hipLaunchKernelGGL(k_bin_scatter, dim3(nblk), dim3(256), lds, st, ntile, (uint32_t)nb, slab, h->d_tile.p, bhist, hist, cursor, order);
     return hipGetLastError();
 }
 
-static hipError_t launch_entry(mi3d_solver *h, hipStream_t st, const DevScene &S, uint64_t nb, uint64_t seed, uint64_t off, const uint32_t *order, float4 *entry) {
+static hipError_t launch_entry(mi3d_solver *h, hipStream_t st, const DevScene &S, int form, uint64_t nb, uint64_t seed, uint64_t off, const uint32_t *order, float4 *entry) {
     const DevCold &C = h->cold_host;
     EntryArgs A;
     A.lay = C.lay;
     A.Lx = C.Lx; A.Ly = C.Ly; A.dx = S.dx; A.dy = S.dy; A.inv_dx = C.inv_dx; A.inv_dy = C.inv_dy; A.inv_nx = C.inv_nx; A.inv_ny = C.inv_ny;
     A.sdx = C.sdx; A.sdy = C.sdy; A.sdz = C.sdz; A.cos_cone = C.cos_cone;
     A.nx = S.nx; A.ny = S.ny; A.nz = S.nz; A.solver = S.solver; A.target = S.target; A.kdir = S.kdir;
-    hipLaunchKernelGGL(k_entry, dim3((unsigned)((nb + 255) / 256)), dim3(256), 0, st, A, nb, seed, off, order, entry);
+    if (form == kEntryF4Short) hipLaunchKernelGGL(k_entry<kEntryF4Short>, dim3((unsigned)((nb + 255) / 256)), dim3(256), 0, st, A, nb, seed, off, order, entry);
+    else hipLaunchKernelGGL(k_entry<kEntryF4>, dim3((unsigned)((nb + 255) / 256)), dim3(256), 0, st, A, nb, seed, off, order, entry);
     return hipGetLastError();
 }
 
+static bool lean_short_build(bool emit, int mix, int nt) { return !emit && mix == 0 && nt == 256; }
+
 static hipError_t launch_lean(mi3d_solver *h, hipStream_t st, const DevScene &S, bool emit, int mix, int nt, unsigned grid, size_t lds, uint64_t nb, uint64_t seed, uint64_t off) {
+    const bool short_rec = h->entry_form_run == kEntryF4Short && lean_short_build(emit, mix, nt);
     const int v = (h->counting ? 4 : 0) + (h->solver == MI3D_SOLVER_P3D ? 2 : 0) + (emit ? 1 : 0);
 #define MI3D_LEAN_LAUNCH(C, P, M)                                                                                                        \
     do {                                                                                                                                 \
@@ -1255,6 +1267,7 @@
             if (lds > 65536) (void)hipFuncSetAttribute(reinterpret_cast<const void *>(k_transport_lean<C, P, M, 2>), hipFuncAttributeMaxDynamicSharedMemorySize, (int)lds); \
             hipLaunchKernelGGL((k_transport_lean<C, P, M, 2>), dim3(grid), dim3(256), lds, st, S, nb, seed, off);                         \
         } else if (mix == 1) hipLaunchKernelGGL((k_transport_lean<C, P, M, 1>), dim3(grid), dim3(256), lds, st, S, nb, seed, off);        \
+        else if (short_rec) hipLaunchKernelGGL((k_transport_lean<C, P, 0, 0, 256, kEntryF4Short>), dim3(grid), dim3(256), lds, st, S, nb, seed, off); \
         else hipLaunchKernelGGL((k_transport_lean<C, P, M, 0>), dim3(grid), dim3(256), lds, st, S, nb, seed, off);                        \
     } while (0)
     switch (v) {
@@ -1768,16 +1781,25 @@
     return want_cap;
 }
 
+static int entry_form(const mi3d_solver *h, const RunPlan &plan) {
+    const DevCold &C = h->cold_host;
+    const bool launch_ok = C.cos_cone >= 1.0f && C.sdz < 0.0f && !plan.thermal && !h->thermal();
+    const bool build_ok = plan.loop == Loop::Column && lean_short_build(false, plan.mix_lean, 256);
+    return (h->entry_records == 1 && launch_ok && build_ok) ? kEntryF4Short : kEntryF4;
+}
+
 static bool use_entry_records(mi3d_solver *h, const RunPlan &plan, uint64_t nphoton) {
+    h->entry_form_run = 0;
 #if MI3D_LEAN_FAST
     if ((h->target & MI3D_TARGET_HEAT) && h->heat_estimator == 1) return false;
     if (plan.loop == Loop::General || plan.thermal || !h->entry_records || h->nx >= 65536 || h->ny >= 65536 || h->nz >= 32768) return false;
     DevBuf<float4> &E = h->pre[0].entry;
-    const size_t need = entry_f4((size_t)std::min<uint64_t>(nphoton, h->batch));
+    const int form = entry_form(h, plan);
+    const size_t need = entry_f4((size_t)std::min<uint64_t>(nphoton, h->batch), form);
     size_t free_b = free_bytes((size_t)8 << 30);
     free_b += E.cap * sizeof(float4);
     if (need > E.cap && need * sizeof(float4) > free_b / 2) return false;
-    if (E.alloc(need) == MI3D_OK) { h->cold_host.entry = E.p; return true; }
+    if (E.alloc(need) == MI3D_OK) { h->cold_host.entry = E.p; h->entry_form_run = form; return true; }
     (void)hipGetLastError();
 #endif
     return false;
@@ -1941,7 +1963,7 @@
     if (eb == hipSuccess && pre_two && h->pre_main_used) { eb = hipStreamWaitEvent(ps, h->pre_main, 0); h->pre_main_used = false; }
     if (eb == hipSuccess && plan.sorted) eb = launch_bins(h, ps, plan.G, plan.ntile, seed, off, nb, PS.order.p, PS.cursor.p);
     if (eb == hipSuccess && use_entry)
-        eb = launch_entry(h, ps, S, nb, seed, off, plan.sorted ? (const uint32_t *)PS.order.p : (const uint32_t *)nullptr, PS.entry.p);
+        eb = launch_entry(h, ps, S, h->entry_form_run, nb, seed, off, plan.sorted ? (const uint32_t *)PS.order.p : (const uint32_t *)nullptr, PS.entry.p);
     if (eb == hipSuccess && pre_two) eb = hipEventRecord(PS.done, ps);
     if (eb == hipSuccess && pre_track && !pre_two) {
         if (!h->pre_main) eb = hipEventCreateWithFlags(&h->pre_main, hipEventDisableTiming);
@@ -1973,12 +1995,14 @@
         if (nvox > lim || (double)h->flux_elems() > lim || (double)h->rad_elems() > lim || (double)h->heat_elems() > lim)
             return fail(MI3D_EUNSUP, "grid too large for the 32-bit table indices of the transport kernel");
     }
+    h->entry_form_last = 0;
     DevScene S;
     if ((rc = fill_scene(h, S))) return rc;
     RunPlan plan = plan_run(h, nphoton);
     if (plan.sorted) {
         const size_t cap = (size_t)std::min<uint64_t>(nphoton, h->batch);
-        if ((rc = h->pre[0].order.alloc(cap)) || (rc = h->d_tile.alloc(cap))) return rc;
+        const size_t nblk = std::min<size_t>((cap + 4095) / 4096, 4096);
+        if ((rc = h->pre[0].order.alloc(cap)) || (rc = h->d_tile.alloc(cap)) || (rc = h->d_hist.alloc((size_t)plan.ntile * (nblk + 1)))) return rc;
     }
     h->cold_host.order = plan.sorted ? h->pre[0].order.p : nullptr;
 
@@ -2036,6 +2060,7 @@
         else if (err == hipSuccess) err = launch_column(h, plan, Sl, set, two_sets, rs, grid, nb, seed, off);
         if (err == hipSuccess && !run_timed) err = hipEventRecord(e1, h->stream);
         h->pre_last = pset;
+        h->entry_form_last = use_entry ? h->entry_form_run : 0; h->entry_n_last = nb;
         if (err == hipSuccess && (pre_two || pre_track)) {
             if (!PS.loop) err = hipEventCreateWithFlags(&PS.loop, hipEventDisableTiming);
             if (err == hipSuccess) err = hipEventRecord(PS.loop, h->stream);
@@ -2147,7 +2172,7 @@
     else if (k == "tl_split") { if (value < 1 || value > 64) return fail(MI3D_EINVAL, "tl_split=%d outside [1,64]", value); h->tl_split = value; }
     else if (k == "rays_wg" || k == "emit_wg") { if (value < 0 || value > 8) return fail(MI3D_EINVAL, "%s=%d outside [0,8]", key, value); (k == "rays_wg" ? h->rays_wg : h->emit_wg) = value; }
     else if (k == "cam_images") { if (value < -1 || value > 8) return fail(MI3D_EINVAL, "cam_images=%d outside [-1,8]", value); h->cam_images = value; }
-    else if (k == "entry_records") { HIPCHK(sync_main(h)); h->entry_records = value ? 1 : 0; if (!value) h->pre[0].entry.release(); }
+    else if (k == "entry_records") { if (value < 0 || value > 2) return fail(MI3D_EINVAL, "entry_records=%d outside [0,2]", value); HIPCHK(sync_main(h)); h->entry_records = value; if (!value) h->pre[0].entry.release(); }
     else if (k == "tally_runs") { HIPCHK(sync_main(h)); h->tally_runs = value ? 1 : 0; h->tl_per_photon = 0.0; h->tl_total_pp = 0.0; h->tl_runs_pp = 0.0; if (!value) for (auto &T : h->tl) T.runs.release(); }
     else if (k == "tally_lists") { HIPCHK(sync_main(h)); h->tally_lists = value ? 1 : 0; if (!value) for (auto &T : h->tl) T.release(); }
     else if (k == "own_stream") {
@@ -2485,6 +2510,21 @@
     return MI3D_OK;
 }
 
+int mi3d_debug_entry(mi3d_solver *h, uint64_t n, float *records_out) {
+    int rc = check_handle(h);
+    if (rc) return rc;
+    const int form = h->entry_form_last;
+    const mi3d_solver::PreSet &PS = h->pre[h->pre_last];
+    if (form == 0 || !PS.entry.p) return fail(MI3D_ESTATE, "the last launch had no entry records (mi3d_debug_entry)");
+    if (n > 0) {
+        if (!records_out) return fail(MI3D_EINVAL, "bad arguments to mi3d_debug_entry");
+        if (n > h->entry_n_last || entry_f4((size_t)n, form) > PS.entry.cap) return fail(MI3D_EINVAL, "mi3d_debug_entry: the last launch had %llu photons, not %llu", (unsigned long long)h->entry_n_last, (unsigned long long)n);
+        HIPCHK(sync_streams(h));
+        HIPCHK(hipMemcpy(records_out, PS.entry.p, entry_f4((size_t)n, form) * sizeof(float4), hipMemcpyDeviceToHost));
+    }
+    return form;
+}
+
 int mi3d_debug_thermal(mi3d_solver *h, double *ptot, double *cdf_out, uint64_t n) {
     int rc = check_handle(h);
     if (rc) return rc;
diff --git a/er3t_amd/csrc/mi3d_device.h b/er3t_amd/csrc/mi3d_device.h
--- a/er3t_amd/csrc/mi3d_device.h
+++ b/er3t_amd/csrc/mi3d_device.h
@@ -99,9 +99,9 @@
 __host__ __device__ inline int tab_bucket_mu(float mu) { const int b = (int)(fmaf(mu, 0.5f, 0.5f) * (float)kTabNB); return b < 0 ? 0 : (b > kTabNB - 1 ? kTabNB - 1 : b); }
 __host__ __device__ inline int tab_bucket_u(float u) { const int b = (int)(u * (float)kTabNB); return b < 0 ? 0 : (b > kTabNB - 1 ? kTabNB - 1 : b); }
 constexpr int kWin = 64;
-constexpr int kEntryF4 = 3;
-__host__ __device__ inline size_t entry_f4(size_t n) { return ((n + 63) / 64) * 64 * (size_t)kEntryF4; }
-__host__ __device__ inline unsigned entry_index(unsigned pos) { return (pos >> 6) * (64u * (unsigned)kEntryF4) + (pos & 63u); }
+constexpr int kEntryF4 = 3, kEntryF4Short = 2;
+__host__ __device__ inline size_t entry_f4(size_t n, int form = kEntryF4) { return ((n + 63) / 64) * 64 * (size_t)form; }
+__host__ __device__ inline unsigned entry_index(unsigned pos, int form = kEntryF4) { return (pos >> 6) * (64u * (unsigned)form) + (pos & 63u); }
 constexpr int kEvStride = 64;
 constexpr int kEvBlockF4 = 3 * 64 + 16;
 __host__ __device__ inline size_t ev_list_f4(size_t cap) { return (cap / 64) * kEvBlockF4; }
diff --git a/er3t_amd/csrc/mi3d_kernel_lean.hip b/er3t_amd/csrc/mi3d_kernel_lean.hip
--- a/er3t_amd/csrc/mi3d_kernel_lean.hip
+++ b/er3t_amd/csrc/mi3d_kernel_lean.hip
@@ -50,7 +50,7 @@
 constexpr int M_DRAWL = 16;
 constexpr int M_ENTRY = 17;
 
-template <bool COUNT, bool P3D, int MARCH, int MIX, int NT = 256>
+template <bool COUNT, bool P3D, int MARCH, int MIX, int NT = 256, int EF = kEntryF4>
 #ifndef MI3D_LEAN_REG_WAVES
 #define MI3D_LEAN_REG_WAVES(COUNT, MARCH) MI3D_LEAN_WAVES(COUNT, MARCH)
 #endif
@@ -61,6 +61,7 @@
 k_transport_lean(const DevScene S, const uint64_t nphoton, const uint64_t seed, const uint64_t offset) {
     static_assert(MARCH == 0 || MARCH == 2, "marched views go through event records and k_rays");
     static_assert(MIX >= 0 && MIX <= 3 && (NT == 256 || NT == 512), "builds");
+    static_assert(EF == kEntryF4 || (EF == kEntryF4Short && MARCH == 0), "the event-writing builds read long entry records");
     constexpr bool MIXED = (MARCH != 0), EMIT = (MARCH == 2), TWO = (MIX == 1), GEN = (MIX >= 2), RAY1 = (MIX == 3);
     constexpr unsigned NW = NT / 64;
     extern __shared__ float4 smem[];
@@ -173,6 +174,7 @@
         const unsigned cell_ = (unsigned)ix, km_ = (unsigned)k;                                                      \
         ix = (int)(cell_ & 0xffffu); iy = (int)(cell_ >> 16);                                                        \
         k = (int)(km_ & 0xffffu);                                                                                    \
+        if (EF == kEntryF4Short) pz = lay[k].dz;     \
         mode = ((km_ >> 16) & 0x7fffu) == (unsigned)M_FLY ? M_SETUP : M_UNIF;                                        \
         if (COUNT && (km_ >> 31)) cnt.steps++;                  \
     } while (0)
@@ -620,13 +622,21 @@
                 lid = order ? glb_load_u32(order + pool_next, rank * 4u) : pool_next + rank;
                 if (entry) {
                     const unsigned j = (pool_next & 63u) + rank;
-                    const float4 *eb = entry + (size_t)(pool_next >> 6) * (size_t)(64 * kEntryF4);
-                    const unsigned eo = ((j >> 6) * (unsigned)(64 * kEntryF4) + (j & 63u)) * 16u;
-                    const float4 q0 = glb_load_f4<MI3D_ENTRY_NT_LOAD != 0>(eb, eo), q1 = glb_load_f4<MI3D_ENTRY_NT_LOAD != 0>(eb, eo + 1024u), q2 = glb_load_f4<MI3D_ENTRY_NT_LOAD != 0>(eb, eo + 2048u);
-                    px = q0.x; py = q0.y; pz = q0.z; rem = q0.w;
-                    ux = q1.x; uy = q1.y; uz = q1.z; u1 = q1.w;
-                    u2 = q2.x; u3 = q2.y;
-                    ix = __float_as_int(q2.z); k = __float_as_int(q2.w);
+                    const float4 *eb = entry + (size_t)(pool_next >> 6) * (size_t)(64 * EF);
+                    const unsigned eo = ((j >> 6) * (unsigned)(64 * EF) + (j & 63u)) * 16u;
+                    if (EF == kEntryF4Short) {
+                        const float4 q0 = glb_load_f4<MI3D_ENTRY_NT_LOAD != 0>(eb, eo), q1 = glb_load_f4<MI3D_ENTRY_NT_LOAD != 0>(eb, eo + 1024u);
+                        px = q0.x; py = q0.y; rem = q0.z; u1 = q0.w;
+                        u2 = q1.x; u3 = q1.y;
+                        ix = __float_as_int(q1.z); k = __float_as_int(q1.w);
+                        ux = cold->sdx; uy = cold->sdy; uz = cold->sdz;
+                    } else {
+                        const float4 q0 = glb_load_f4<MI3D_ENTRY_NT_LOAD != 0>(eb, eo), q1 = glb_load_f4<MI3D_ENTRY_NT_LOAD != 0>(eb, eo + 1024u), q2 = glb_load_f4<MI3D_ENTRY_NT_LOAD != 0>(eb, eo + 2048u);
+                        px = q0.x; py = q0.y; pz = q0.z; rem = q0.w;
+                        ux = q1.x; uy = q1.y; uz = q1.z; u1 = q1.w;
+                        u2 = q2.x; u3 = q2.y;
+                        ix = __float_as_int(q2.z); k = __float_as_int(q2.w);
+                    }
                     mode = M_ENTRY;
                     w = 1.0f; direct = true; draw = 2;
                     kind = E_LAUNCH;
@@ -748,8 +758,10 @@
 
 #ifdef MI3D_ONLY_HEADLINE
 template __global__ void k_transport_lean<false, false, 0, 0>(const DevScene, const uint64_t, const uint64_t, const uint64_t);
+template __global__ void k_transport_lean<false, false, 0, 0, 256, kEntryF4Short>(const DevScene, const uint64_t, const uint64_t, const uint64_t);
 #else
 #define MI3D_LEAN_INST(C, P) template __global__ void k_transport_lean<C, P, 0, 0>(const DevScene, const uint64_t, const uint64_t, const uint64_t); \
+                             template __global__ void k_transport_lean<C, P, 0, 0, 256, kEntryF4Short>(const DevScene, const uint64_t, const uint64_t, const uint64_t); \
                              template __global__ void k_transport_lean<C, P, 2, 0>(const DevScene, const uint64_t, const uint64_t, const uint64_t); \
                              template __global__ void k_transport_lean<C, P, 0, 1>(const DevScene, const uint64_t, const uint64_t, const uint64_t); \
                              template __global__ void k_transport_lean<C, P, 2, 1>(const DevScene, const uint64_t, const uint64_t, const uint64_t); \
@@ -769,6 +781,7 @@
     int nx, ny, nz, solver, target, kdir;
 };
 
+template <int EF>
 __global__ void __launch_bounds__(256)
 k_entry(const EntryArgs A, const uint64_t nphoton, const uint64_t seed, const uint64_t offset, const uint32_t *__restrict__ order, float4 *__restrict__ entry) {
     const LayerRec *lay = A.lay;
@@ -790,7 +803,7 @@
         float pz = lay[k].dz;
         float ux = A.sdx, uy = A.sdy, uz = A.sdz;
         const float mu_cone = 1.0f - r2 * (1.0f - A.cos_cone);
-        if (!(A.cos_cone >= 1.0f)) rotate_dir(ux, uy, uz, mu_cone, r3);
+        if (EF != kEntryF4Short && !(A.cos_cone >= 1.0f)) rotate_dir(ux, uy, uz, mu_cone, r3);
         draw4_fast(seed, id, 1u, r0, r1, r2, r3);
         float rem = -0.69314718f * __builtin_amdgcn_logf(r0);
         int mode = (lay[k].flags & kLayStep3d) ? M_FLY : M_UNIF;
@@ -819,11 +832,19 @@
             }
         }
         typedef float vf4 __attribute__((ext_vector_type(4)));
-        vf4 *e = reinterpret_cast<vf4 *>(entry) + entry_index(i);
-        __builtin_nontemporal_store((vf4){px, py, pz, rem}, e);
-        __builtin_nontemporal_store((vf4){ux, uy, uz, r1}, e + 64);
-        __builtin_nontemporal_store((vf4){r2, r3, __uint_as_float((unsigned)ix | ((unsigned)iy << 16)), __uint_as_float((unsigned)k | ((unsigned)mode << 16) | (ran << 31))}, e + 128);
+        vf4 *e = reinterpret_cast<vf4 *>(entry) + entry_index(i, EF);
+        const float cell = __uint_as_float((unsigned)ix | ((unsigned)iy << 16)), km = __uint_as_float((unsigned)k | ((unsigned)mode << 16) | (ran << 31));
+        if (EF == kEntryF4Short) {
+            __builtin_nontemporal_store((vf4){px, py, rem, r1}, e);
+            __builtin_nontemporal_store((vf4){r2, r3, cell, km}, e + 64);
+        } else {
+            __builtin_nontemporal_store((vf4){px, py, pz, rem}, e);
+            __builtin_nontemporal_store((vf4){ux, uy, uz, r1}, e + 64);
+            __builtin_nontemporal_store((vf4){r2, r3, cell, km}, e + 128);
+        }
     }
 }
+template __global__ void k_entry<kEntryF4>(const EntryArgs, const uint64_t, const uint64_t, const uint64_t, const uint32_t *__restrict__, float4 *__restrict__);
+template __global__ void k_entry<kEntryF4Short>(const EntryArgs, const uint64_t, const uint64_t, const uint64_t, const uint32_t *__restrict__, float4 *__restrict__);
 
 }
diff --git a/er3t_amd/csrc/mi3d_kernels.hip b/er3t_amd/csrc/mi3d_kernels.hip
--- a/er3t_amd/csrc/mi3d_kernels.hip
+++ b/er3t_amd/csrc/mi3d_kernels.hip
@@ -293,101 +293,131 @@
     return ty * G.ntx + ((ty & 1) ? G.ntx - 1 - tx : tx);
 }
 
-__global__ void __launch_bounds__(256)
-k_bin_count(const BinGeom G, uint64_t seed, uint64_t offset, uint32_t n, uint16_t *tile, uint32_t *hist) {
+
+__global__ void __launch_bounds__(256)
+k_bin_count(const BinGeom G, uint64_t seed, uint64_t offset, uint32_t n, uint32_t slab, uint16_t *tile, uint32_t *bhist) {
     __shared__ uint32_t lh[kMaxTiles];
     const int nt = G.ntx * G.nty;
     for (int i = threadIdx.x; i < nt; i += blockDim.x) lh[i] = 0u;
     __syncthreads();
-    for (uint32_t i = blockIdx.x * blockDim.x + threadIdx.x; i < n; i += gridDim.x * blockDim.x) {
+    const uint32_t lo = min(n, blockIdx.x * slab), hi = min(n, lo + slab);
+    for (uint32_t i = lo + threadIdx.x; i < hi; i += blockDim.x) {
         const int t = launch_tile(G, seed, offset + i);
         tile[i] = (uint16_t)t;
         atomicAdd(&lh[t], 1u);
     }
     __syncthreads();
-    for (int i = threadIdx.x; i < nt; i += blockDim.x)
-        if (lh[i]) atomicAdd(&hist[i], lh[i]);
-}
-
-__global__ void __launch_bounds__(256)
-k_bin_scan(int nt, const uint32_t *hist, uint32_t *cursor) {
-    static_assert(kMaxTiles == 4 * 256, "four tiles per thread");
-    __shared__ uint32_t s[256];
-    const int t = threadIdx.x;
-    uint32_t h[4], sum = 0u;
-    for (int j = 0; j < 4; ++j) { h[j] = 4 * t + j < nt ? hist[4 * t + j] : 0u; sum += h[j]; }
-    s[t] = sum;
+    for (int i = threadIdx.x; i < nt; i += blockDim.x) bhist[(size_t)i * gridDim.x + blockIdx.x] = lh[i];
+}
+
+__device__ inline uint32_t block_scan_256(uint32_t sum, uint32_t *part, uint32_t *total) {
+    const unsigned tid = threadIdx.x;
+    uint32_t incl = sum;
+    for (int off = 1; off < 64; off <<= 1) {
+        const uint32_t x = __shfl_up(incl, off, 64);
+        if ((tid & 63u) >= (unsigned)off) incl += x;
+    }
     __syncthreads();
-    for (int off = 1; off < 256; off <<= 1) {
-        const uint32_t v = t >= off ? s[t - off] : 0u;
-        __syncthreads();
-        s[t] += v;
-        __syncthreads();
-    }
-    uint32_t run = s[t] - sum;
-    for (int j = 0; j < 4; ++j) { if (4 * t + j < nt) cursor[4 * t + j] = run; run += h[j]; }
-}
-
-constexpr int kScatterR = 16;
-__global__ void __launch_bounds__(256)
-k_bin_scatter(int nt, uint32_t n, uint32_t slab, const uint16_t *tile, uint32_t *cursor, uint32_t *order) {
-    constexpr int NT = 256, CH = NT * kScatterR;
-    __shared__ uint32_t lcount[kMaxTiles], lstart[kMaxTiles], gbase[kMaxTiles], part[NT / 64];
-    __shared__ uint32_t sidx[CH];
-    __shared__ uint16_t stile[CH];
+    if ((tid & 63u) == 63u) part[tid >> 6] = incl;
+    __syncthreads();
+    uint32_t before = 0, all = 0;
+    for (unsigned wv = 0; wv < 4u; ++wv) { const uint32_t x = part[wv]; all += x; if (wv < (tid >> 6)) before += x; }
+    *total = all;
+    return before + incl - sum;
+}
+
+__global__ void __launch_bounds__(256)
+k_bin_scan(int nblk, uint32_t *bhist, uint32_t *hist) {
+    __shared__ uint32_t part[4];
+    uint32_t *row = bhist + (size_t)blockIdx.x * nblk;
+    const int per = (nblk + 255) / 256;
+    const int lo = min((int)threadIdx.x * per, nblk), hi = min(lo + per, nblk);
+    uint32_t sum = 0u, total;
+    for (int i = lo; i < hi; ++i) sum += row[i];
+    uint32_t run = block_scan_256(sum, part, &total);
+    for (int i = lo; i < hi; ++i) { const uint32_t c = row[i]; row[i] = run; run += c; }
+    if (threadIdx.x == 0) hist[blockIdx.x] = total;
+}
+
+constexpr int kScatterR = 32;
+constexpr int kScatterCH = 256 * kScatterR;
+static_assert(kScatterCH <= 65536 && kScatterR % 8 == 0, "offsets into a chunk are 16 bits; groups of eight");
+__host__ __device__ inline size_t bin_scatter_lds(int nt) { return (size_t)10 * nt * sizeof(uint32_t) + (size_t)2 * kScatterCH * sizeof(uint16_t); }
+__global__ void __launch_bounds__(256)
+k_bin_scatter(int nt, uint32_t n, uint32_t slab, const uint16_t *tile, const uint32_t *bhist, const uint32_t *hist, uint32_t *cursor, uint32_t *order) {
+    constexpr int NT = 256, NW = NT / 64, CH = kScatterCH, NG = kScatterR / 8;
+    extern __shared__ uint32_t bs_lds[];
+    __shared__ uint32_t part[NW];
+    uint32_t *wcount = bs_lds, *wstart = bs_lds + NW * nt, *gbase = bs_lds + 2 * NW * nt, *gdst = gbase + nt;
+    uint16_t *soff = reinterpret_cast<uint16_t *>(gdst + nt), *stile = soff + CH;
     const unsigned tid = threadIdx.x;
-    for (int i = tid; i < nt; i += NT) lcount[i] = 0u;
-    __syncthreads();
-    const uint32_t lo = blockIdx.x * slab, hi = min(n, lo + slab);
-    for (uint32_t i = lo + tid; i < hi; i += NT) atomicAdd(&lcount[tile[i]], 1u);
-    __syncthreads();
-    for (int i = tid; i < nt; i += NT) gbase[i] = lcount[i] ? atomicAdd(&cursor[i], lcount[i]) : 0u;
+    uint32_t *mycount = wcount + (tid >> 6) * (unsigned)nt;
+    const uint32_t *mystart = wstart + (tid >> 6) * (unsigned)nt;
     const int per = (nt + NT - 1) / NT;
     const int tlo = min((int)tid * per, nt), thi = min(tlo + per, nt);
+    {
+        uint32_t sum = 0u, total;
+        for (int i = tlo; i < thi; ++i) sum += hist[i];
+        uint32_t run = block_scan_256(sum, part, &total);
+        for (int i = tlo; i < thi; ++i) {
+            gbase[i] = run + bhist[(size_t)i * gridDim.x + blockIdx.x];
+            run += hist[i];
+            if (blockIdx.x == 0) cursor[i] = run;
+            for (int wv = 0; wv < NW; ++wv) wcount[wv * nt + i] = 0u;
+        }
+    }
     __syncthreads();
+    const uint32_t lo = min(n, blockIdx.x * slab), hi = min(n, lo + slab);
     for (uint32_t c0 = lo; c0 < hi; c0 += CH) {
-        for (int i = tlo; i < thi; ++i) lcount[i] = 0u;
+        const uint32_t total = min((uint32_t)CH, hi - c0);
+        uint32_t tr[kScatterR];
+#pragma unroll
+        for (int g = 0; g < NG; ++g) {
+            const uint32_t o = (uint32_t)(g * NT * 8) + tid * 8u;
+            uint32_t w[4] = {0u, 0u, 0u, 0u};
+            if (o + 8u <= total) {
+                const uint4 q = *reinterpret_cast<const uint4 *>(tile + c0 + o);
+                w[0] = q.x; w[1] = q.y; w[2] = q.z; w[3] = q.w;
+            } else {
+                for (int r = 0; r < 8; ++r)
+                    if (o + (uint32_t)r < total) w[r >> 1] |= (uint32_t)tile[c0 + o + r] << ((r & 1) * 16);
+            }
+#pragma unroll
+            for (int r = 0; r < 8; ++r) {
+                const uint32_t t = (r & 1) ? (w[r >> 1] >> 16) : (w[r >> 1] & 0xffffu);
+                tr[g * 8 + r] = (o + (uint32_t)r < total) ? ((t << 16) | atomicAdd(&mycount[t], 1u)) : 0xffffffffu;
+            }
+        }
         __syncthreads();
-        uint32_t t[kScatterR];
-#pragma unroll
-        for (int r = 0; r < kScatterR; ++r) {
-            const uint32_t i = c0 + (uint32_t)(r * NT) + tid;
-            t[r] = i < hi ? (uint32_t)tile[i] : 0xffffffffu;
-            if (t[r] != 0xffffffffu) atomicAdd(&lcount[t[r]], 1u);
-        }
-        __syncthreads();
-        uint32_t sum = 0;
-        for (int i = tlo; i < thi; ++i) sum += lcount[i];
-        uint32_t incl = sum;
-        for (int off = 1; off < 64; off <<= 1) {
-            const uint32_t x = __shfl_up(incl, off, 64);
-            if ((tid & 63u) >= (unsigned)off) incl += x;
-        }
-        if ((tid & 63u) == 63u) part[tid >> 6] = incl;
-        __syncthreads();
-        uint32_t before = 0, total = 0;
-        for (unsigned wv = 0; wv < (unsigned)(NT / 64); ++wv) { const uint32_t x = part[wv]; total += x; if (wv < (tid >> 6)) before += x; }
-        uint32_t run = before + incl - sum;
+        uint32_t sum = 0, all;
+        for (int i = tlo; i < thi; ++i)
+            for (int wv = 0; wv < NW; ++wv) sum += wcount[wv * nt + i];
+        uint32_t run = block_scan_256(sum, part, &all);
         for (int i = tlo; i < thi; ++i) {
-            const uint32_t c = lcount[i];
-            lstart[i] = run; lcount[i] = run;
-            run += c;
+            gdst[i] = gbase[i] - run;
+            const uint32_t run0 = run;
+            for (int wv = 0; wv < NW; ++wv) {
+                const uint32_t c = wcount[wv * nt + i];
+                wstart[wv * nt + i] = run;
+                wcount[wv * nt + i] = 0u;
+                run += c;
+            }
+            gbase[i] += run - run0;
         }
         __syncthreads();
 #pragma unroll
-        for (int r = 0; r < kScatterR; ++r)
-            if (t[r] != 0xffffffffu) {
-                const uint32_t p = atomicAdd(&lcount[t[r]], 1u);
-                sidx[p] = c0 + (uint32_t)(r * NT) + tid;
-                stile[p] = (uint16_t)t[r];
+        for (int g = 0; g < NG; ++g)
+#pragma unroll
+            for (int r = 0; r < 8; ++r) {
+                const uint32_t v = tr[g * 8 + r];
+                if (v != 0xffffffffu) {
+                    const uint32_t t = v >> 16, p = mystart[t] + (v & 0xffffu);
+                    soff[p] = (uint16_t)((uint32_t)(g * NT * 8) + tid * 8u + (uint32_t)r);
+                    stile[p] = (uint16_t)t;
+                }
             }
         __syncthreads();
-        for (uint32_t j = tid; j < total; j += NT) {
-            const uint32_t tt = stile[j];
-            order[gbase[tt] + (j - lstart[tt])] = sidx[j];
-        }
-        __syncthreads();
-        for (int i = tlo; i < thi; ++i) gbase[i] += lcount[i] - lstart[i];
+        for (uint32_t j = tid; j < total; j += NT) order[gdst[stile[j]] + j] = c0 + soff[j];
     }
 }
 
diff --git a/er3t_amd/solver.py b/er3t_amd/solver.py
--- a/er3t_amd/solver.py
+++ b/er3t_amd/solver.py
@@ -69,6 +69,7 @@
     ('mi3d_stats_get'          , C.c_int   , [C.c_void_p, C.c_int, _fp, _fp, C.POINTER(C.c_int)]),
     ('mi3d_debug_philox'       , C.c_int   , [C.c_void_p, _u64, _u64, C.c_uint32, C.c_int, C.POINTER(C.c_uint32)]),
     ('mi3d_debug_order'        , C.c_int   , [C.c_void_p, _u64, C.POINTER(C.c_uint32), C.POINTER(C.c_uint32), C.c_int]),
+    ('mi3d_debug_entry'        , C.c_int   , [C.c_void_p, _u64, _fp]),
     ('mi3d_debug_thermal'      , C.c_int   , [C.c_void_p, C.POINTER(C.c_double), C.POINTER(C.c_double), _u64]),
     ('mi3d_debug_phase_tables' , C.c_int   , [C.c_void_p, C.c_int, C.c_int, _fp, _fp, _fp, C.POINTER(C.c_uint16), C.POINTER(C.c_uint16)]),
     ('mi3d_debug_phase'        , C.c_int   , [C.c_void_p, C.c_int, C.c_int, C.c_int, C.c_int, _fp, _fp, _fp, _fp, _fp]),
@@ -398,6 +399,18 @@
         self._chk(self.lib.mi3d_debug_order(self._h, int(n), order.ctypes.data_as(C.POINTER(C.c_uint32)), tend.ctypes.data_as(C.POINTER(C.c_uint32)), int(ntile_max)))
         return order, tend
 
+    def debug_entry(self, n=0):
+        form = self.lib.mi3d_debug_entry(self._h, 0, None)
+        if form < 0:
+            self._chk(form)
+        if not n:
+            return form, None
+        rec = np.zeros(((int(n) + 63)//64, form, 64, 4), dtype=np.float32)
+        rc = self.lib.mi3d_debug_entry(self._h, int(n), _ptr(rec))
+        if rc < 0:
+            self._chk(rc)
+        return form, rec
+
     def debug_thermal(self, ncell):
         ptot = C.c_double(0.0); cdf = np.zeros(int(ncell), dtype=np.float64)
         self._chk(self.lib.mi3d_debug_thermal(self._h, C.byref(ptot), cdf.ctypes.data_as(C.POINTER(C.c_double)), int(ncell)))
diff --git a/include/mi3d.h b/include/mi3d.h
--- a/include/mi3d.h
+++ b/include/mi3d.h
@@ -141,6 +141,7 @@
 int mi3d_debug_philox(mi3d_solver *h, uint64_t seed, uint64_t id0, uint32_t draw, int n,
                       uint32_t *out);
 int mi3d_debug_order(mi3d_solver *h, uint64_t n, uint32_t *order_out, uint32_t *tile_end_out, int ntile_max);
+int mi3d_debug_entry(mi3d_solver *h, uint64_t n, float *records_out);
 int mi3d_debug_thermal(mi3d_solver *h, double *ptot, double *cdf_out, uint64_t n);
 #define MI3D_TAB_IDX_N 514
 int mi3d_debug_phase_tables(mi3d_solver *h, int nang, int npf, float *mu, float *p, float *cdf, uint16_t *mu_idx, uint16_t *cdf_idx);
```

Result: faster. 2.928 billion photons/s, median of 6 (+1.0%).
